# peterhpark/neuroclear

Hardware: AMD Instinct MI355X
Metric: voxels/sec (higher is better)
Workload: dtype f32

## Files before the change

include/nc_hip.h:

```cpp
#ifndef NC_HIP_H
#define NC_HIP_H

#include <stddef.h>
#include <stdint.h>

#ifdef __cplusplus
extern "C" {
#endif

#define NC_OK 0
#define NC_ERR_SHAPE (-1)
#define NC_ERR_WS (-2)
#define NC_ERR_HIP (-3)
#define NC_ERR_ARG (-4)

const char* nc_last_error(void);
int nc_version(void);
int nc_conv_fwd_path(int C, int K, int kd, int kh, int kw, int stride, int pad);
int nc_conv_wgrad_path(int C, int K, int kd, int kh, int kw, int stride, int pad);
void nc_prof_begin(double min_flop);
int nc_prof_end(int max, int* cls, double* flop, float* ms);
int nc_prof_end2(int max, int* cls, double* flop, float* ms, double* abytes);
void nc_set_force_direct(int on);
void nc_sconv_set_cfg(int cfg);
// ... 229 lines not shown
int nc_c8_instnorm_act_bwd(const void* gh, int g_ctot, int g_c0, const void* xh, const float* mean, const float* rstd, float slope,
                           void* dxh, float* dbias , int N, int C, long S, int dtype, void* ws, size_t ws_bytes,
                           void* stream);
int nc_c8_maxpool2_fwd(const void* xh, int x_ctot, int x_c0, void* yh, int N, int C, int D, int H, int W, int dtype, void* stream);
int nc_c8_maxpool2_bwd_add(const void* dph, const void* xh, int x_ctot, int x_c0, const void* skiph, int s_ctot, int s_c0, void* dxh,
                           int N, int C, int D, int H, int W, int dtype, void* stream);
int nc_from_c8(const void* xh, int x_ctot, int x_c0, float* y, int N, int C, long S, int dtype, void* stream);
size_t nc_convT_c8_ws_bytes(int N, int C, int D, int H, int W, int K);
int nc_convT_k2s2_fwd_c8(const void* xh, const float* w, const float* bias, void* yh, int out_ctot, int out_c0, int N, int C, int D,
                         int H, int W, int K, int dtype, void* ws, size_t ws_bytes, void* stream);
int nc_convT_k2s2_dgrad_c8(const void* dyh, int dy_ctot, int dy_c0, const float* w, void* dxh, int N, int C, int D, int H, int W, int K,
                           void* ws, size_t ws_bytes, void* stream);
int nc_convT_k2s2_wgrad_c8(const void* xh, const void* dyh, int dy_ctot, int dy_c0, float* dw, float* dbias , int N,
                           int C, int D, int H, int W, int K, void* ws, size_t ws_bytes, void* stream);

int nc_unet_deconv_lp_supported(int N, int S0, int S1, int S2, int dtype);
size_t nc_unet_deconv_lp_saved_bytes(int N, int S0, int S1, int S2);
size_t nc_unet_deconv_lp_ws_bytes(int N, int S0, int S1, int S2);
int nc_unet_deconv_lp_fwd(const float* params, const float* x, float* y, void* saved, int N, int S0, int S1, int S2, int dtype,
                          void* ws, size_t ws_bytes, void* stream);
int nc_unet_deconv_lp_bwd(const float* params, const float* x, const float* y, const void* saved, const float* dy, float* dx,
                          float* dparams, int N, int S0, int S1, int S2, int dtype, void* ws, size_t ws_bytes, void* stream);
int nc_deep_linear_lp_supported(int N, int S0, int S1, int S2, int dtype);
size_t nc_deep_linear_lp_saved_bytes(int N, int S0, int S1, int S2);
size_t nc_deep_linear_lp_ws_bytes(int N, int S0, int S1, int S2);
int nc_deep_linear_lp_fwd(const float* params, const float* x, float* y, void* saved, int N, int S0, int S1, int S2, int dtype,
                          void* ws, size_t ws_bytes, void* stream, unsigned* kept);
int nc_deep_linear_lp_bwd(const float* params, const float* x, const void* saved, const float* dy, float* dx, float* dparams,
                          int N, int S0, int S1, int S2, int dtype, void* ws, size_t ws_bytes, void* stream, unsigned kept);

void nc_set_conv_split(int on);
int nc_get_conv_split(void);
void nc_set_split_terms(int terms);
int nc_get_split_terms(void);
void nc_set_p2d_terms(int mode);
int nc_get_p2d_terms(void);
void nc_set_h2_guard(int on);
int nc_get_h2_guard(void);
int nc_h2_guard_stats(unsigned long long* out4, int reset);
void nc_set_epi_stats(int on);
int nc_get_epi_stats(void);
void nc_set_s3x_w64(int on);
int nc_get_s3x_w64(void);
int nc_unet_deconv_fwd_terms(int S0, int S1, int S2);
void nc_set_c8x_mode(int mode);
int nc_get_c8x_mode(void);
int nc_conv_lp_uses_c8x(int what , int fp32_out, int N, int C, int D, int H, int W, int K, int ks);
void nc_set_s3_fusion(int on);
int nc_conv_split_supported(int what, int N, int C, int D, int H, int W, int K, int kd, int kh, int kw, int stride, int pad);
size_t nc_conv_split_ws_bytes(int N, int C, int D, int H, int W, int K, int ks);
size_t nc_s3_bytes(int N, int C, long S);
int nc_to_s3(const float* x, void* xs, int N, int C, long S, void* stream);
int nc_conv_fwd_split(const float* x, const void* xs, const float* w, const float* bias, float* y, int N, int C, int D, int H, int W,
                      int K, int ks , void* ws, size_t ws_bytes, void* stream);
int nc_conv_dgrad_split(const float* dy, const void* dys, const float* w, float* dx, int N, int C, int D, int H, int W, int K, int ks,
                        void* ws, size_t ws_bytes, void* stream);
int nc_conv_wgrad_split(const float* x, const void* xs, const float* dy, const void* dys, float* dw, int N, int C, int D, int H, int W,
                        int K, int ks, void* ws, size_t ws_bytes, void* stream);

int nc_conv2d_split_active(int what, int N, int C, int H, int W, int K, int k, int stride, int pad);

int nc_convT_k2s2_split_supported(int N, int C, int D, int H, int W, int K);
int nc_convT_k2s2_split_active(int N, int C, int D, int H, int W, int K);
size_t nc_convT_k2s2_split_ws_bytes(int N, int C, int D, int H, int W, int K);
int nc_convT_k2s2_fwd_split(const float* x, const void* xs, const float* w, const float* bias, float* y, void* ys, int ys_ctot, int ys_c0,
                            int N, int C, int D, int H, int W, int K, void* ws, size_t ws_bytes, void* stream);

size_t nc_h2_bytes(int N, int C, long S);
size_t nc_h2_cells_offset(size_t elems);
int nc_to_h2_debug(const float* x, long xstride, void* xs, int N, int C, long S, int ctot, int c0, unsigned* cell, float bound, unsigned* guard,
                   void* stream);
int nc_act_split2h_debug(const float* x, const float* mean, const float* rstd, float slope, float* y, long ystride, void* ys, int N, int C, long S,
                         int ctot, int c0, float bound, unsigned* cell, unsigned* cell2, void* stream);
int nc_act_split2h_pool_debug(const float* x, const float* mean, const float* rstd, float slope, void* ys, void* pooled, int N, int C, int D, int H,
                              int W, int ctot, int c0, float bound, unsigned* cell, void* stream);
int nc_maxpool2_h2_debug(const void* in, void* out, int N, int C, int ctot, int D, int H, int W, void* stream);
int nc_h2_to_s3_if_debug(const void* xh, void* xs, int N, int C, long S, const unsigned* cells, const unsigned* guard, void* stream);
int nc_instnorm_act_bwd_dbias_h2_debug(const float* dy, const float* w1, const float* x, const float* mean, const float* rstd, float slope, void* dxs,
                                       float* dbias, int N, int C, long S, void* ws, size_t ws_bytes, unsigned* guard, void* stream);
int nc_instnorm_act_bwd_dbias_h2_pool_debug(const float* dy, long dy_stride, const float* gp, const unsigned char* arg, const float* x, const float* mean,
                                            const float* rstd, float slope, void* dxs, float* dbias, int N, int C, int D, int H, int W, void* ws,
                                            size_t ws_bytes, unsigned* guard, void* stream);
int nc_maxpool2_fwd_arg_debug(const float* x, float* y, unsigned char* arg, int NC, int D, int H, int W, void* stream);
size_t nc_convT_k2s2_split_h2_ws_bytes(int N, int C, int D, int H, int W, int K);
int nc_convT_k2s2_fwd_split_h2_debug(const float* x, const float* w, const float* bias, float* y, void* ys, int ys_ctot, int ys_c0, int N, int C,
                                     int D, int H, int W, int K, unsigned* out_cell, void* ws, size_t ws_bytes, void* stream);
int nc_convT_k2s2_fwd_s3_debug(const float* x, const float* w, const float* bias, float* y, void* ys, int ys_ctot, int ys_c0, int N, int C, int D,
                               int H, int W, int K, void* stream);
int nc_instnorm_relu_tail_sigmoid_debug(const float* x, const float* mean, const float* rstd, const float* w1, const float* b1, const float* w2,
                                        const float* b2, float* y, int C, long S, void* stream);

size_t nc_lk_ws_bytes(int N, int D, int H, int W, int k);
int nc_lk_fwd(const float* x, const float* w, float* y, int N, int D, int H, int W, int k, void* ws, size_t ws_bytes, void* stream);
int nc_lk_dgrad(const float* dy, const float* w, float* dx, int N, int D, int H, int W, int k, void* ws, size_t ws_bytes, void* stream);
int nc_lk_wgrad(const float* x, const float* dy, float* dw, int N, int D, int H, int W, int k, void* ws, size_t ws_bytes, void* stream);

size_t nc_kgan_param_floats(int ndf, int nd);
size_t nc_kgan_saved_floats(int B, int D, int H, int W, int ndf, int nd);
size_t nc_kgan_ws_bytes(int B, int D, int H, int W, int ndf, int nd);
int nc_kgan_out_shape(int B, int D, int H, int W, int ndf, int nd, int* oD, int* oH, int* oW);
int nc_kgan_fwd(const float* params, const float* x, float* y, float* saved, int B, int D, int H, int W, int ndf, int nd, void* ws,
                size_t ws_bytes, void* stream);
int nc_kgan_bwd(const float* params, const float* x, const float* saved, const float* dy, float* dx, float* dparams, int B, int D, int H,
                int W, int ndf, int nd, void* ws, size_t ws_bytes, void* stream);

#ifdef __cplusplus
}
#endif
#endif
```

neuroclear_amd/csrc/api.hip:

```cpp
#include <cstring>
#include <vector>

#include <atomic>
#include <mutex>
#include <set>
#include <utility>

#include "common.hpp"

namespace nc {

static thread_local char g_err[512] = "";

void set_error(const char* fmt, ...) {
  va_list ap;
  va_start(ap, fmt);
  vsnprintf(g_err, sizeof(g_err), fmt, ap);
  va_end(ap);
}

int raise_dyn_lds(const void* kernel, int bytes, const char* who) {
  static std::mutex mu;
  static std::set<std::pair<const void*, int>> done;
  int dev = 0;
// ... 403 lines not shown
  if (nc_conv2d_k3_reflect_active(0, N, C, H, W, K)) {
    ProfScope ps(0, 12, d, 0, s);
    return conv_fwd_k3_reflect(x, w, bias, y, d, (char*)ws + pb, ws_bytes - pb, s);
  }
  if (int e = reflect_pad_fwd(x, (float*)ws, (long)N * C, H, W, 1, s)) return e;
  return nc_conv_fwd((const float*)ws, w, bias, y, N, C, 1, H + 2, W + 2, K, 1, 3, 3, 1, 0, (char*)ws + pb, ws_bytes - pb, stream);
}

int nc_conv2d_k3_reflect_dgrad(const float* dy, const float* w, float* dx, int N, int C, int H, int W, int K, void* ws, size_t ws_bytes,
                               void* stream) {
  ConvDims d;
  if (int e = k3r_args("conv2d_k3_reflect_dgrad", d, dy, w, dx, N, C, H, W, K, ws, ws_bytes)) return e;
  hipStream_t s = (hipStream_t)stream;
  const size_t pb = k3r_pad_bytes(N, C, H, W);
  float* dxe = (float*)ws;
  if (nc_conv2d_k3_reflect_active(1, N, C, H, W, K)) {
    ProfScope ps(1, 12, d, 0, s);
    if (int e = conv_dgrad_k3_reflect_ext(dy, w, dxe, d, (char*)ws + pb, ws_bytes - pb, s)) return e;
  } else {
    if (int e = nc_conv_dgrad(dy, w, dxe, N, C, 1, H + 2, W + 2, K, 1, 3, 3, 1, 0, (char*)ws + pb, ws_bytes - pb, stream)) return e;
  }
  return reflect_pad_bwd(dxe, dx, (long)N * C, H, W, 1, s);
}

int nc_conv2d_k3_reflect_wgrad(const float* x, const float* dy, float* dw, float* dbias, int N, int C, int H, int W, int K, void* ws,
                               size_t ws_bytes, void* stream) {
  ConvDims d;
  if (int e = k3r_args("conv2d_k3_reflect_wgrad", d, x, dy, dw, N, C, H, W, K, ws, ws_bytes)) return e;
  const size_t pb = k3r_pad_bytes(N, C, H, W);
  if (int e = reflect_pad_fwd(x, (float*)ws, (long)N * C, H, W, 1, (hipStream_t)stream)) return e;
  return nc_conv_wgrad((const float*)ws, dy, dw, dbias, N, C, 1, H + 2, W + 2, K, 1, 3, 3, 1, 0, (char*)ws + pb, ws_bytes - pb, stream);
}

int nc_conv_bwd(const float* x, const float* dy, const float* w, float* dx, float* dw, float* dbias, int N, int C, int D, int H, int W,
                int K, int kd, int kh, int kw, int stride, int pad, void* ws, size_t ws_bytes, void* stream) {
  ConvDims d;
  if (int e = conv_args("conv_bwd", d, x, dy, dw, N, C, D, H, W, K, kd, kh, kw, stride, pad)) return e;
  if (!w) { set_error("conv_bwd: null pointer"); return NC_ERR_ARG; }
  hipStream_t s = (hipStream_t)stream;
  SwitchScope switches_;
  if (dx && dgrad_path(d) == 9 && wgrad_path(d) == 9 && ws && s3_bwd_ws_bytes(d) && ws_bytes >= s3_bwd_ws_bytes(d)) {
    {
      ProfScope ps(1, 9, d, 0, s);
      if (int e = conv_bwd_s3(x, dy, w, dx, dw, d, ws, ws_bytes, s, 0)) return e;
      if (int e = conv_bwd_s3(x, dy, w, dx, dw, d, ws, ws_bytes, s, 1)) return e;
    }
    {
      ProfScope ps(2, 9, d, 0, s);
      if (int e = conv_bwd_s3(x, dy, w, dx, dw, d, ws, ws_bytes, s, 2)) return e;
    }
    if (dbias) return bias_grad(dy, dbias, d.N, d.K, (long)d.Do * d.Ho * d.Wo, ws, ws_bytes, s);
    return NC_OK;
  }
  if (dx)
    if (int e = nc_conv_dgrad(dy, w, dx, N, C, D, H, W, K, kd, kh, kw, stride, pad, ws, ws_bytes, stream)) return e;
  return nc_conv_wgrad(x, dy, dw, dbias, N, C, D, H, W, K, kd, kh, kw, stride, pad, ws, ws_bytes, stream);
}

}

namespace nc {
int conv_fwd_keep(const float* x, const float* w, const float* bias, float* y, int N, int C, int D, int H, int W, int K, int ks,
                  void* ws, size_t ws_bytes, void* stream, void* xs_keep, bool* kept, const S3xPrepared* prep) {
  ConvDims d;
  *kept = false;
  if (xs_keep && make_dims(d, N, C, D, H, W, K, ks, ks, ks, 1, ks / 2) && fwd_path(d) == 9 && wgrad_path(d) == 9) {
    if (!x || !w || !y) { set_error("conv_fwd: null pointer"); return NC_ERR_ARG; }
    ProfScope ps(0, 9, d, 0, (hipStream_t)stream);
    *kept = true;
    return conv_fwd_s3(x, nullptr, w, bias, y, d, ws, ws_bytes, (hipStream_t)stream, xs_keep, nullptr, prep);
  }
  return nc_conv_fwd(x, w, bias, y, N, C, D, H, W, K, ks, ks, ks, 1, ks / 2, ws, ws_bytes, stream);
}

bool conv_keep_supported(int N, int C, int D, int H, int W, int K, int ks) {
  ConvDims d;
  return make_dims(d, N, C, D, H, W, K, ks, ks, ks, 1, ks / 2) && fwd_path(d) == 9 && wgrad_path(d) == 9;
}
bool conv_fwd_on_split(int N, int C, int D, int H, int W, int K, int ks) {
  ConvDims d;
  return make_dims(d, N, C, D, H, W, K, ks, ks, ks, 1, ks / 2) && fwd_path(d) == 9;
}

int conv_fwd_pre(const void* xs, const float* w, const float* bias, float* y, int N, int C, int D, int H, int W, int K, int ks, void* ws,
                 size_t ws_bytes, void* stream, float* stats_part, const S3xPrepared* prep) {
  ConvDims d;
  if (!xs || !w || !y) { set_error("conv_fwd_pre: null pointer"); return NC_ERR_ARG; }
  if (!make_dims(d, N, C, D, H, W, K, ks, ks, ks, 1, ks / 2) || fwd_path(d) != 9) { set_error("conv_fwd_pre: layer not on the split-operand kernels"); return NC_ERR_SHAPE; }
  ProfScope ps(0, 9, d, 0, (hipStream_t)stream);
  if (stats_part && !(conv_layer_h2(d) && ks == 3)) { set_error("conv_fwd_pre: epilogue statistics exist for the two-term 3^3 layers only"); return NC_ERR_ARG; }
  return conv_fwd_s3(nullptr, xs, w, bias, y, d, ws, ws_bytes, (hipStream_t)stream, nullptr, stats_part, prep);
}

bool conv_bwd_pre_supported(int N, int C, int D, int H, int W, int K, int ks, bool want_dx, size_t ws_bytes) {
  ConvDims d;
  return make_dims(d, N, C, D, H, W, K, ks, ks, ks, 1, ks / 2) && wgrad_path(d) == 9 && s3_bwd_ws_bytes(d) && ws_bytes >= s3_bwd_ws_bytes(d) &&
         (!want_dx || dgrad_path(d) == 9);
}
int conv_bwd_pre(const float* x, const void* xs, const float* w, float* dx, float* dw, int N, int C, int D, int H, int W, int K, int ks,
                 void* ws, size_t ws_bytes, void* stream, bool dy_guarded, const S3xPrepared* prep) {
  ConvDims d;
  hipStream_t s = (hipStream_t)stream;
  if (!conv_bwd_pre_supported(N, C, D, H, W, K, ks, dx != nullptr, ws_bytes) || !make_dims(d, N, C, D, H, W, K, ks, ks, ks, 1, ks / 2)) {
    set_error("conv_bwd_pre: layer not on the split-operand kernels");
    return NC_ERR_SHAPE;
  }
  if ((!x && !xs) || !w || !dw || !ws) { set_error("conv_bwd_pre: null pointer"); return NC_ERR_ARG; }
  if (dx) {
    ProfScope ps(1, 9, d, 0, s);
    if (int e = conv_bwd_s3(x, nullptr, w, dx, dw, d, ws, ws_bytes, s, 1, nullptr, dy_guarded, prep)) return e;
  }
  ProfScope ps(2, 9, d, 0, s);
  return conv_bwd_s3(x, nullptr, w, dx, dw, d, ws, ws_bytes, s, 2, xs, dy_guarded);
}

int conv_bwd_keep(const float* x, const void* xs, const float* dy, const float* w, float* dx, float* dw, int N, int C, int D, int H,
                  int W, int K, int ks, void* ws, size_t ws_bytes, void* stream) {
  ConvDims d;
  hipStream_t s = (hipStream_t)stream;
  if (xs && make_dims(d, N, C, D, H, W, K, ks, ks, ks, 1, ks / 2) && wgrad_path(d) == 9 && ws && s3_bwd_ws_bytes(d) &&
      ws_bytes >= s3_bwd_ws_bytes(d) &&
      (!dx || dgrad_path(d) == 9)) {
    if (!x || !dy || !w || !dw) { set_error("conv_bwd: null pointer"); return NC_ERR_ARG; }
    {
      ProfScope ps(1, 9, d, 0, s);
      if (int e = conv_bwd_s3(x, dy, w, dx, dw, d, ws, ws_bytes, s, 0)) return e;
      if (dx)
        if (int e = conv_bwd_s3(x, dy, w, dx, dw, d, ws, ws_bytes, s, 1)) return e;
    }
    ProfScope ps(2, 9, d, 0, s);
    return conv_bwd_s3(x, dy, w, dx, dw, d, ws, ws_bytes, s, 2, xs);
  }
  return nc_conv_bwd(x, dy, w, dx, dw, nullptr, N, C, D, H, W, K, ks, ks, ks, 1, ks / 2, ws, ws_bytes, stream);
}
}
```

neuroclear_amd/csrc/c8_api.hip:

```cpp
#include "common.hpp"

namespace nc {
size_t c8_stats_ws_bytes(int N, int C, long S);
int c8_instnorm_stats(const void* x, int N, int C, long S, float eps, float* mean, float* rstd, int dt, void* ws, size_t wsb, hipStream_t s);
int c8_instnorm_apply(const void* x, const float* mean, const float* rstd, float slope, void* y, int ctot, int c0, int N, int C, long S, int dt, hipStream_t s);
int c8_instnorm_bwd(const void* g, int gctot, int gc0, const void* x, const float* mean, const float* rstd, float slope, void* dx, float* dbias, int N, int C, long S, int dt, void* ws, size_t wsb, hipStream_t s);
int c8_maxpool_fwd(const void* x, int ctot, int c0, void* y, int N, int C, int D, int H, int W, int dt, hipStream_t s);
int c8_maxpool_bwd_add(const void* dp, const void* x, int ctot, int c0, const void* skip, int sctot, int sc0, void* dx, int N, int C, int D, int H, int W, int dt, hipStream_t s);
int c8_to_f32(const void* x, int ctot, int c0, float* y, int N, int C, long S, int dt, hipStream_t s);
bool convT_h_supported(int C, int K);
size_t convT_h_ws_bytes(int N, int C, int D, int H, int W, int K);
int convT_fwd_h(const void* x, const float* w, const float* bias, void* out, int octot, int oc0, int N, int C, int D, int H, int W, int K, int dt, void* ws, size_t wsb, hipStream_t s);
int convT_dgrad_h(const void* dy, int dctot, int dc0, const float* w, void* dx, int N, int C, int D, int H, int W, int K, void* ws, size_t wsb, hipStream_t s);
int convT_wgrad_h(const void* x, const void* dy, int dctot, int dc0, float* dw, float* dbias, int N, int C, int D, int H, int W, int K, void* ws, size_t wsb, hipStream_t s);
}

using namespace nc;

static bool dt_ok(int dt) { return dt == NC_DT_F16 || dt == NC_DT_BF16; }

extern "C" {

int nc_conv_fwd_c8(const void* xh, const float* w, const float* bias, void* yh, int out_ctot, int out_c0, int N, int C, int D, int H,
                   int W, int K, int kd, int kh, int kw, int stride, int pad, int dtype, void* ws, size_t ws_bytes, void* stream) {
// ... 109 lines not shown
int nc_conv_split_supported(int what, int N, int C, int D, int H, int W, int K, int kd, int kh, int kw, int stride, int pad) {
  ConvDims d;
  if (!make_dims(d, N, C, D, H, W, K, kd, kh, kw, stride, pad)) return 0;
  return what == 0 ? s3_fwd_supported(d) : what == 1 ? s3_dgrad_supported(d) : what == 2 ? s3_wgrad_supported(d) : 0;
}

size_t nc_conv_split_ws_bytes(int N, int C, int D, int H, int W, int K, int ks) {
  ConvDims d;
  if (!make_dims(d, N, C, D, H, W, K, ks, ks, ks, 1, ks / 2)) return 0;
  const size_t a = s3_ws_bytes(d), b = s3_wgrad_ws_bytes(d);
  return a > b ? a : b;
}

size_t nc_s3_bytes(int N, int C, long S) { return (C % 8 || N < 1 || S < 1) ? 0 : s3_tensor_bytes(N, C, S); }

int nc_to_s3(const float* x, void* xs, int N, int C, long S, void* stream) {
  if (!x || !xs) { set_error("to_s3: null pointer"); return NC_ERR_ARG; }
  if (N < 1 || C < 8 || C % 8 || S < 1) { set_error("to_s3: channels must be a multiple of 8"); return NC_ERR_SHAPE; }
  return split3_to(x, xs, N, C, S, (hipStream_t)stream);
}

int nc_conv_fwd_split(const float* x, const void* xs, const float* w, const float* bias, float* y, int N, int C, int D, int H, int W,
                      int K, int ks, void* ws, size_t ws_bytes, void* stream) {
  ConvDims d;
  if ((!x && !xs) || !w || !y) { set_error("conv_fwd_split: null pointer"); return NC_ERR_ARG; }
  if (!make_dims(d, N, C, D, H, W, K, ks, ks, ks, 1, ks / 2) || !s3_fwd_supported(d)) { set_error("conv_fwd_split: shape not covered"); return NC_ERR_SHAPE; }
  ProfScope ps(0, 1, d, 1, (hipStream_t)stream);
  ForceThreeTerm f3;
  return conv_fwd_s3(x, xs, w, bias, y, d, ws, ws_bytes, (hipStream_t)stream);
}

int nc_conv_dgrad_split(const float* dy, const void* dys, const float* w, float* dx, int N, int C, int D, int H, int W, int K, int ks,
                        void* ws, size_t ws_bytes, void* stream) {
  ConvDims d;
  if ((!dy && !dys) || !w || !dx) { set_error("conv_dgrad_split: null pointer"); return NC_ERR_ARG; }
  if (!make_dims(d, N, C, D, H, W, K, ks, ks, ks, 1, ks / 2) || !s3_dgrad_supported(d)) { set_error("conv_dgrad_split: shape not covered"); return NC_ERR_SHAPE; }
  ProfScope ps(1, 1, d, 1, (hipStream_t)stream);
  ForceThreeTerm f3;
  return conv_dgrad_s3(dy, dys, w, dx, d, ws, ws_bytes, (hipStream_t)stream);
}

int nc_conv_wgrad_split(const float* x, const void* xs, const float* dy, const void* dys, float* dw, int N, int C, int D, int H, int W,
                        int K, int ks, void* ws, size_t ws_bytes, void* stream) {
  ConvDims d;
  if ((!x && !xs) || (!dy && !dys) || !dw) { set_error("conv_wgrad_split: null pointer"); return NC_ERR_ARG; }
  if (!make_dims(d, N, C, D, H, W, K, ks, ks, ks, 1, ks / 2) || !s3_wgrad_supported(d)) { set_error("conv_wgrad_split: shape not covered"); return NC_ERR_SHAPE; }
  ProfScope ps(2, 9, d, 0, (hipStream_t)stream);
  ForceThreeTerm f3;
  return conv_wgrad_s3(x, xs, dy, dys, dw, d, ws, ws_bytes, (hipStream_t)stream);
}

static size_t al256(size_t b) { return (b + 255) & ~(size_t)255; }
int nc_convT_k2s2_split_supported(int N, int C, int D, int H, int W, int K) { return convT_s3x_supported(N, C, D, H, W, K) ? 1 : 0; }
int nc_conv_lp_uses_c8x(int what, int fp32_out, int N, int C, int D, int H, int W, int K, int ks) {
  if (what == 0) return c8x_supported(N, C, D, H, W, K, ks, fp32_out != 0) ? 1 : 0;
  if (what == 1) return c8x_supported(N, K, D, H, W, C, ks, fp32_out != 0) ? 1 : 0;
  return 0;
}
int nc_convT_k2s2_split_active(int N, int C, int D, int H, int W, int K) { return nc_get_conv_split() && convT_s3x_supported(N, C, D, H, W, K) ? 1 : 0; }
size_t nc_convT_k2s2_split_ws_bytes(int N, int C, int D, int H, int W, int K) {
  if (!convT_s3x_supported(N, C, D, H, W, K)) return 0;
  return al256(convT_s3x_ws_bytes(C, K)) + al256(s3_tensor_bytes(N, C, (long)D * H * W)) + 256;
}
int nc_convT_k2s2_fwd_split(const float* x, const void* xs, const float* w, const float* bias, float* y, void* ys, int ys_ctot, int ys_c0,
                            int N, int C, int D, int H, int W, int K, void* ws, size_t ws_bytes, void* stream) {
  if ((!x && !xs) || !w || (!y && !ys) || !ws) { set_error("convT_k2s2_fwd_split: null pointer"); return NC_ERR_ARG; }
  if (!convT_s3x_supported(N, C, D, H, W, K)) { set_error("convT_k2s2_fwd_split: shape not covered"); return NC_ERR_SHAPE; }
  const size_t wb = al256(convT_s3x_ws_bytes(C, K));
  const long S = (long)D * H * W;
  if (ws_bytes < wb + (xs ? 0 : al256(s3_tensor_bytes(N, C, S)))) { set_error("convT_k2s2_fwd_split: workspace too small"); return NC_ERR_WS; }
  if (!xs) {
    void* t = (char*)ws + wb;
    if (int e = split3_to(x, t, N, C, S, (hipStream_t)stream)) return e;
    xs = t;
  }
  return convT_fwd_s3x(xs, w, bias, y, ys, ys ? ys_ctot : 8, ys ? ys_c0 : 0, N, C, D, H, W, K, ws, wb, (hipStream_t)stream);
}

}

namespace nc {
int convT_fwd_split_h2(const float* x, const float* w, const float* bias, float* y, void* ys, int ys_ctot, int ys_c0, int N, int C, int D, int H,
                       int W, int K, const unsigned* out_cell, void* ws, size_t ws_bytes, hipStream_t s) {
  if (!x || !w || !ys || !out_cell || !ws) { set_error("convT_fwd_split_h2: null pointer"); return NC_ERR_ARG; }
  if (!convT_s3x_supported(N, C, D, H, W, K)) { set_error("convT_fwd_split_h2: shape not covered"); return NC_ERR_SHAPE; }
  const size_t wb = al256(convT_s3x_ws_bytes(C, K));
  const long S = (long)D * H * W;
  const size_t ex = (size_t)N * C * S;
  if (ws_bytes < wb + h2_cells_offset(ex) + 256) { set_error("convT_fwd_split_h2: workspace too small"); return NC_ERR_WS; }
  void* t = (char*)ws + wb;
  unsigned* xc = h2_cells_of(t, ex);
  if (int e = h2_set_cell(xc, sqrtf((float)S), s)) return e;
  if (int e = split2h_into(x, (long)C * S, t, N, C, S, C, 0, xc, s)) return e;
  return convT_fwd_s3x(t, w, bias, y, ys, ys_ctot, ys_c0, N, C, D, H, W, K, ws, wb, s, out_cell, xc);
}
}
```

neuroclear_amd/csrc/common.hpp:

```cpp
#pragma once
#include <hip/hip_runtime.h>

#include <cstdarg>
#include <cstdio>

#include "../../include/nc_hip.h"
#include "switches.hpp"

namespace nc {

void set_error(const char* fmt, ...);

inline int check_launch(const char* what) {
  hipError_t e = hipGetLastError();
  if (e != hipSuccess) {
    set_error("%s: %s", what, hipGetErrorString(e));
    return NC_ERR_HIP;
  }
  return NC_OK;
}

inline long cdiv(long a, long b) { return (a + b - 1) / b; }
inline size_t align256(size_t b) { return (b + 255) & ~(size_t)255; }
inline size_t up64(size_t n) { return (n + 63) & ~(size_t)63; }
// ... 46 lines not shown
    return false;
  d.Do = (D + 2 * d.pd - kd) / d.sd + 1;
  d.Ho = (H + 2 * d.ph - kh) / d.sh + 1;
  d.Wo = (W + 2 * d.pw - kw) / d.sw + 1;
  return d.Do >= 1 && d.Ho >= 1 && d.Wo >= 1 && (D + 2 * d.pd >= kd) && (H + 2 * d.ph >= kh) && (W + 2 * d.pw >= kw);
}

int conv_fwd_direct(const float* x, const float* w, const float* b, float* y, const ConvDims& d, hipStream_t s);
int conv_dgrad_direct(const float* dy, const float* w, float* dx, const ConvDims& d, hipStream_t s);
int conv_wgrad_direct(const float* x, const float* dy, float* dw, const ConvDims& d, hipStream_t s);
int bias_grad(const float* dy, float* db, int N, int K, long S, void* ws, size_t wsb, hipStream_t s);
static constexpr size_t kBiasGradWsBytes = 64 * 1024 * sizeof(double);

bool mfma_fwd_supported(const ConvDims& d);
bool c1k3_fwd_supported(const ConvDims& d);
int conv_fwd_c1k3(const float* x, const float* w, const float* bias, float* y, const ConvDims& d, hipStream_t s, float* stats_part = nullptr);
size_t c1k3_stats_bytes(const ConvDims& d);
int c1k3_stats_finalize(const float* stats_part, const float* bias, const ConvDims& d, float eps, float* mean, float* rstd, hipStream_t s);
bool mfma_dgrad_supported(const ConvDims& d);
bool mfma_wgrad_supported(const ConvDims& d);
size_t mfma_ws_bytes(const ConvDims& d);
size_t mfma_fwd_ws_bytes(const ConvDims& d);
int conv_fwd_mfma(const float* x, const float* w, const float* b, float* y, const ConvDims& d, void* ws, size_t wsb,
                  hipStream_t s);
int conv_dgrad_mfma(const float* dy, const float* w, float* dx, const ConvDims& d, void* ws, size_t wsb,
                    hipStream_t s);
int conv_wgrad_mfma(const float* x, const float* dy, float* dw, const ConvDims& d, void* ws, size_t wsb,
                    hipStream_t s);

bool gemm_fwd_supported(const ConvDims& d);
bool gemm_dgrad_supported(const ConvDims& d);
bool gemm_wgrad_supported(const ConvDims& d);
size_t gemm_ws_bytes(const ConvDims& d);
int conv_fwd_gemm(const float* x, const float* w, const float* b, float* y, const ConvDims& d, void* ws, size_t wsb,
                  hipStream_t s);
int conv_dgrad_gemm(const float* dy, const float* w, float* dx, const ConvDims& d, void* ws, size_t wsb,
                    hipStream_t s);
int conv_wgrad_gemm(const float* x, const float* dy, float* dw, const ConvDims& d, void* ws, size_t wsb,
                    hipStream_t s);

bool sconv_fwd_supported(const ConvDims& d);
bool sconv_dgrad_supported(const ConvDims& d);
size_t sconv_ws_bytes(const ConvDims& d);
bool p2d_fwd_supported(const ConvDims& d);
bool p2d_dgrad_supported(const ConvDims& d);
size_t p2d_ws_bytes(const ConvDims& d);
int conv_fwd_p2d(const float* x, const float* w, const float* bias, float* y, const ConvDims& d, void* ws, size_t wsb, hipStream_t s);
int conv_dgrad_p2d(const float* dy, const float* w, float* dx, const ConvDims& d, void* ws, size_t wsb, hipStream_t s);
bool p2d_wgrad_supported(const ConvDims& d);
size_t p2d_wgrad_ws_bytes(const ConvDims& d);
int conv_wgrad_p2d(const float* x, const float* dy, float* dw, const ConvDims& d, void* ws, size_t wsb, hipStream_t s);
int conv_fwd_sconv(const float* x, const float* w, const float* bias, float* y, const ConvDims& d, void* ws, size_t wsb, hipStream_t s);
int conv_dgrad_sconv(const float* dy, const float* w, float* dx, const ConvDims& d, void* ws, size_t wsb, hipStream_t s);
int conv2d_k3_num_cfgs();
bool conv2d_k3_fwd_supported(const ConvDims& d);
bool conv2d_k3_dgrad_supported(const ConvDims& d);
size_t conv2d_k3_ws_bytes(const ConvDims& d);
int conv_fwd_k3(const float* x, const float* w, const float* bias, float* y, const ConvDims& d, void* ws, size_t wsb, hipStream_t s);
int conv_dgrad_k3(const float* dy, const float* w, float* dx, const ConvDims& d, void* ws, size_t wsb, hipStream_t s);
bool conv2d_k3_reflect_ok(const ConvDims& d);
int conv_fwd_k3_reflect(const float* x, const float* w, const float* bias, float* y, const ConvDims& d, void* ws, size_t wsb, hipStream_t s);
int conv_dgrad_k3_reflect_ext(const float* dy, const float* w, float* dxe, const ConvDims& d, void* ws, size_t wsb, hipStream_t s);
int reflect_pad_fwd(const float* x, float* y, long NC, int H, int W, int p, hipStream_t s);
int reflect_pad_bwd(const float* g, float* dx, long NC, int H, int W, int p, hipStream_t s);
bool sconv_wgrad_supported(const ConvDims& d);
size_t sconv_wgrad_ws_bytes(const ConvDims& d);
int conv_wgrad_sconv(const float* x, const float* dy, float* dw, const ConvDims& d, void* ws, size_t wsb, hipStream_t s);

bool pg1_supported(const ConvDims& d);
size_t pg1_ws_bytes(const ConvDims& d);
int conv_fwd_pg1(const float* x, const float* w, const float* bias, float* y, const ConvDims& d, float slope, hipStream_t s);
int conv_wgrad_pg1(const float* x, const float* g, const float* act, float slope, float* dw, float* db, const ConvDims& d,
                   void* ws, size_t wsb, hipStream_t s);
int conv_dgrad_pg1(const float* g, const float* act, float slope, const float* w, float* dx, const ConvDims& d, hipStream_t s);

bool wgrad_1x1_supported(const ConvDims& d);
size_t wgrad_1x1_ws_bytes(const ConvDims& d);
int conv_wgrad_1x1(const float* x, const float* dy, float* dw, const ConvDims& d, void* ws, size_t wsb, hipStream_t s);
bool flat_1x1_supported(const ConvDims& d);
int conv_fwd_1x1(const float* x, const float* w, const float* b, float* y, const ConvDims& d, void* ws, size_t wsb,
                 hipStream_t s);
int conv_dgrad_1x1(const float* dy, const float* w, float* dx, const ConvDims& d, void* ws, size_t wsb,
                   hipStream_t s);

size_t conv_fwd_to1_k3_ws_bytes(int N, int D, int H, int W);
int conv_fwd_to1_k3(const float* x, const float* w, float* y, int N, int C, int D, int H, int W, void* ws, size_t wsb, hipStream_t s);
bool to1_dgrad_supported(const ConvDims& d);
int conv_dgrad_to1(const float* dy, const float* w, float* dx, const ConvDims& d, hipStream_t s);
bool to1_mfma_supported(const ConvDims& d);
size_t to1_mfma_ws_bytes(const ConvDims& d);
int conv_dgrad_to1_mfma(const float* dy, const float* w, float* dx, const ConvDims& d, void* ws, size_t wsb,
                        hipStream_t s);
bool k1_fwd_supported(const ConvDims& d);
bool k1_wgrad_supported(const ConvDims& d);
int conv_fwd_k1(const float* x, const float* w, const float* b, float* y, const ConvDims& d, hipStream_t s);
int conv_wgrad_k1(const float* x, const float* dy, float* dw, const ConvDims& d, hipStream_t s);
bool c1_wgrad_supported(const ConvDims& d);
size_t c1_wgrad_ws_bytes(const ConvDims& d);
int conv_wgrad_c1(const float* x, const float* dy, float* dw, const ConvDims& d, void* ws, size_t wsb, hipStream_t s);

bool s3_fwd_supported(const ConvDims& d);
bool s3_dgrad_supported(const ConvDims& d);
size_t s3_ws_bytes(const ConvDims& d);
size_t s3_tensor_bytes(int N, int C, long S);
int split3_to(const float* x, void* xs, int N, int C, long S, hipStream_t s);
int split3_into(const float* x, long xstride, void* xs, int N, int C, long S, int ctot, int c0, hipStream_t s, const unsigned* guard = nullptr);
bool conv_layer_h2(const ConvDims& d);
void count_in_bwd_launches(int n, int which = 0);
int operand_into(const ConvDims& d, const float* x, long xstride, void* xs, int N, int C, long S, int ctot, int c0, hipStream_t s);
int act_operand(const ConvDims& d, const float* x, const float* mean, const float* rstd, float slope, float* y, long ystride, void* ys, int N, int C,
                long S, int ctot, int c0, hipStream_t s);
int act_split3(const float* x, const float* mean, const float* rstd, float slope, float* y, long ystride, void* ys, int N, int C, long S,
               int ctot, int c0, hipStream_t s);
struct S3xPrepared { const void* wp; const unsigned* wcell; };
int conv_fwd_s3(const float* x, const void* xs, const float* w, const float* b, float* y, const ConvDims& d, void* ws, size_t wsb,
                hipStream_t s, void* xs_keep = nullptr, float* stats_part = nullptr, const S3xPrepared* prep = nullptr);
int conv_dgrad_s3(const float* dy, const void* dys, const float* w, float* dx, const ConvDims& d, void* ws, size_t wsb, hipStream_t s);
size_t s3_bwd_ws_bytes(const ConvDims& d);
int conv_bwd_s3(const float* x, const float* dy, const float* w, float* dx, float* dw, const ConvDims& d, void* ws, size_t wsb,
                hipStream_t s, int phase, const void* xs = nullptr, bool dy_guarded = false, const S3xPrepared* prep = nullptr);
int conv_fwd_keep(const float* x, const float* w, const float* bias, float* y, int N, int C, int D, int H, int W, int K, int ks,
                  void* ws, size_t ws_bytes, void* stream, void* xs_keep, bool* kept, const S3xPrepared* prep = nullptr);
int conv_bwd_keep(const float* x, const void* xs, const float* dy, const float* w, float* dx, float* dw, int N, int C, int D, int H,
                  int W, int K, int ks, void* ws, size_t ws_bytes, void* stream);
bool s3x_supported(int N, int Cin, int D, int H, int W, int Kout, int KS);
size_t s3x_packed_bytes(int Cin, int Kout, int KS, int NT = 3);
int s3x_ksteps(int Cin, int KS);
constexpr int kWPrepMaxSegs = 18, kWPrepMaxBounds = 2, kWPrepBoundCell0 = kWPrepMaxSegs, kWPrepCellBytes = 256;
struct WPrepSeg { const float* w; int Cin, Kout, flip; unsigned a_bits; int b_cell; unsigned* ext_cell; };
struct WPrepBound { const float* w; const float* bias; int C, K; float in_bound; int cell; };
size_t wprep_bytes(const WPrepSeg* segs, int n);
int wprep_run(const WPrepSeg* segs, int n, const WPrepBound* bounds, int nb, void* region, S3xPrepared* out, hipStream_t s);
int s3x_pack_h2(const float* w, int Cin, int Kout, int KS, long so, long si, int flip, int split_c, const unsigned* cell_a, const unsigned* cell_b,
                unsigned* wcell, void* wp_ws, hipStream_t s);
int conv_s3x_h2(const void* xs, const unsigned* cell_a, const unsigned* cell_b, int split_c, const float* w, const float* bias, float* y, int N,
                int Cin, int D, int H, int W, int Kout, int KS, long so, long si, int flip, unsigned* wcell, void* wp_ws, hipStream_t s,
                const unsigned* guard = nullptr, float* stats_part = nullptr, const S3xPrepared* prep = nullptr);
size_t s3x_stats_bytes(int N, int D, int H, int W, int Kout, int KS);
int s3x_stats_finalize(const float* stats_part, const float* bias, int N, int D, int H, int W, int Kout, int KS, float eps, float* mean, float* rstd,
                       hipStream_t s);
bool c1k7_h2_supported(const ConvDims& d);
size_t c1k7_h2_ws_bytes(const ConvDims& d);
int conv_c1k7_h2(const float* x, const float* w, const float* bias, float* y, const ConvDims& d, void* ws, size_t wsb, hipStream_t s);
size_t c1k7_h2_dgrad_ws_bytes(const ConvDims& d);
bool dl_typed_supported(int N, int D, int H, int W);
size_t dl_typed_bytes(int N, int D, int H, int W);
const float* dl_typed_wp(const char* scratch, int N, int D, int H, int W);
float* dl_typed_dwsw(char* scratch, int N, int D, int H, int W);
int dl_typed_compose(const float* F, char* scratch, int N, int D, int H, int W, hipStream_t s);
int dl_typed_fwd_boundary(const float* act0, float* y, char* scratch, int N, int D, int H, int W, hipStream_t s);
int dl_typed_dgrad_boundary(const float* act0, const float* dy, float* g, char* scratch, int N, int D, int H, int W, hipStream_t s);
int dl_typed_p(const float* act0, const float* dy, float* Pq, char* scratch, int N, int D, int H, int W, hipStream_t s);
int conv_c1k7_h2_dgrad(const float* dy, const float* w, float* dx, const ConvDims& d, void* ws, size_t wsb, hipStream_t s);
inline size_t h2_cells_offset(size_t elems) { return (elems * 4 + 255) & ~(size_t)255; }
inline unsigned* h2_cells_of(const void* t, size_t elems) { return (unsigned*)((char*)const_cast<void*>(t) + h2_cells_offset(elems)); }
int instnorm_relu_tail_sigmoid(const float* x, const float* mean, const float* rstd, const float* w1, const float* b1, const float* w2,
                               const float* b2, float* y, int C, long S, hipStream_t s);
int instnorm_act_bwd_dbias_h2(const float* dy, const float* x, const float* mean, const float* rstd, float slope, void* dxs,
                              float* dbias, int N, int C, long S, void* ws, size_t ws_bytes, void* stream, unsigned* guard = nullptr);
int instnorm_act_bwd_dbias_h2_rank1(const float* dy1, const float* w1, const float* x, const float* mean, const float* rstd, float slope, void* dxs,
                                    float* dbias, int C, long S, void* ws, size_t ws_bytes, void* stream, unsigned* guard);
unsigned* conv_bwd_guard_words(void* ws, int N, int K, long S);
int maxpool2_h2(const void* in, void* out, int N, int C, int ctot, int D, int H, int W, hipStream_t s);
int h2_zero_cells(unsigned* cells, int n, hipStream_t s);
int h2_set_cell(unsigned* cell, float bound, hipStream_t s);
int h2_absmax(const float* x, long n, unsigned* cell, hipStream_t s, unsigned* cell2 = nullptr);
int split2h_into(const float* x, long xstride, void* xs, int N, int C, long S, int ctot, int c0, const unsigned* cell, hipStream_t s,
                 unsigned* guard = nullptr);
constexpr int kGuardLow = 0, kGuardAll = 1, kGuardFlag = 2;
constexpr unsigned kGuardDrop = 17u << 23;
constexpr unsigned long long kGuardShare = 64;
#if defined(__HIP_DEVICE_COMPILE__)
__device__ __forceinline__ bool guard_skip(const unsigned* guard, int want) {
  return guard && (int)(__builtin_nontemporal_load(guard + kGuardFlag) != 0) != want;
}
#else
__device__ bool guard_skip(const unsigned* guard, int want);
#endif
#if defined(__HIPCC__)
__device__ __forceinline__ void h2_guard_decide_one(unsigned* ga, unsigned* gb, unsigned* prior, unsigned* flag, int can_flip,
                                                    unsigned long long* stats, unsigned long long total_a) {
  unsigned f = 0;
  unsigned long long worst = 0;
  int n = 0;
  for (unsigned* g : {ga, gb}) {
    if (!g) continue;
    ++n;
    const unsigned long long lo = g[kGuardLow], all = (g == ga && total_a) ? total_a - g[kGuardAll] : g[kGuardAll];
    if (all && lo * kGuardShare > all) f = 1;
    const unsigned long long ppm = all ? lo * 1000000ull / all : 0;
    worst = ppm > worst ? ppm : worst;
  }
  unsigned F = f && can_flip ? 1u : 0u;
  if (prior && prior[kGuardFlag]) F = 1u;
  *flag = F;
  if (prior) prior[kGuardFlag] = F;
  if (stats && n) {
    __hip_atomic_fetch_add(stats + 0, (unsigned long long)n, __ATOMIC_RELAXED, __HIP_MEMORY_SCOPE_SYSTEM);
    if (f) __hip_atomic_fetch_add(stats + (can_flip ? 1 : 2), 1ull, __ATOMIC_RELAXED, __HIP_MEMORY_SCOPE_SYSTEM);
    __hip_atomic_fetch_max(stats + 3, worst, __ATOMIC_RELAXED, __HIP_MEMORY_SCOPE_SYSTEM);
  }
}
#endif
unsigned long long* h2_guard_stats_dev();
int h2_guard_read(unsigned long long* out4, int reset);
int h2_guard_zero(unsigned* g, hipStream_t s, int nwords = 8);
int h2_guard_decide(unsigned* ga, unsigned* gb, unsigned* prior, unsigned* flag, bool can_flip, hipStream_t s, unsigned long long total_a = 0);
int h2_to_s3_if(const void* xh, void* xs, int N, int C, long S, const unsigned* cells, const unsigned* guard, hipStream_t s);
int act_split2h(const float* x, const float* mean, const float* rstd, float slope, float* y, long ystride, void* ys, int N, int C, long S, int ctot,
                int c0, float bound, unsigned* cell, unsigned* cell2, hipStream_t s);
int act_split2h_pool(const float* x, const float* mean, const float* rstd, float slope, void* ys, void* pooled, int N, int C, int D, int H, int W,
                     int ctot, int c0, float bound, unsigned* cell, hipStream_t s);
int conv_s3x(const void* xs, const float* w, const float* bias, float* y, int N, int Cin, int D, int H, int W, int Kout, int KS, long so,
             long si, int flip, void* wp_ws, hipStream_t s, const unsigned* guard = nullptr);
bool conv_keep_supported(int N, int C, int D, int H, int W, int K, int ks);
bool conv_fwd_on_split(int N, int C, int D, int H, int W, int K, int ks);
int conv_fwd_pre(const void* xs, const float* w, const float* bias, float* y, int N, int C, int D, int H, int W, int K, int ks, void* ws,
                 size_t ws_bytes, void* stream, float* stats_part = nullptr, const S3xPrepared* prep = nullptr);
bool conv_bwd_pre_supported(int N, int C, int D, int H, int W, int K, int ks, bool want_dx, size_t ws_bytes);
int conv_bwd_pre(const float* x, const void* xs, const float* w, float* dx, float* dw, int N, int C, int D, int H, int W, int K, int ks,
                 void* ws, size_t ws_bytes, void* stream, bool dy_guarded = false, const S3xPrepared* prep = nullptr);
bool instnorm_bwd_h2_pool_supported(int N, int C, int D, int H, int W, unsigned* guard);
int instnorm_act_bwd_dbias_h2_pool(const float* skip, long skip_stride, const float* gp, const unsigned char* arg, const float* x, const float* mean,
                                   const float* rstd, float slope, void* dxs, float* dbias, int N, int C, int D, int H, int W, void* ws,
                                   size_t ws_bytes, void* stream, unsigned* guard);
int maxpool2_fwd_arg(const float* x, float* y, unsigned char* arg, int NC, int D, int H, int W, hipStream_t s);
bool instnorm_bwd_s3_supported(int N, int C, long S);
int instnorm_act_bwd_dbias_s3(const float* dy, const float* x, const float* mean, const float* rstd, float slope, void* dxs,
                              float* dbias, int N, int C, long S, void* ws, size_t ws_bytes, void* stream);
bool convT_fwd_s3_supported(int N, int C, int D, int H, int W, int K);
size_t c8x_packed_bytes(int Cin, int Kout, int KS);
bool c8x_supported(int N, int Cin, int D, int H, int W, int Kout, int KS, bool fp32_out);
int conv_c8x(const void* xh, const float* w, const float* bias, float* y, void* yh, int ctot, int c0, int N, int Cin, int D, int H, int W,
             int Kout, int KS, long so, long si, int flip, int diffuse, int dt, void* wp_ws, hipStream_t s);
bool convT_s3x_supported(int N, int C, int D, int H, int W, int K);
size_t convT_s3x_ws_bytes(int C, int K);
int convT_fwd_s3x(const void* xs, const float* w, const float* bias, float* y, void* ys, int ctot, int c0, int N, int C, int D, int H, int W,
                  int K, void* ws, size_t wsb, hipStream_t s, const unsigned* h2cell = nullptr, const unsigned* xcell = nullptr);
int convT_h2_bound(const float* w, const float* bias, int C, int K, float in_bound, unsigned* cell, hipStream_t s);
int convT_fwd_split_h2(const float* x, const float* w, const float* bias, float* y, void* ys, int ys_ctot, int ys_c0, int N, int C, int D, int H,
                       int W, int K, const unsigned* out_cell, void* ws, size_t ws_bytes, hipStream_t s);
int convT_fwd_s3(const float* x, const float* w, const float* bias, float* y, void* ys, int ctot, int c0, int N, int C, int D, int H,
                 int W, int K, void* stream);
bool s3_wgrad_supported(const ConvDims& d);
bool c8x_wgrad_supported(const ConvDims& d);
size_t c8x_wgrad_part_bytes(const ConvDims& d);
int conv_wgrad_c8x(const void* xh, const void* dyh, float* dw, const ConvDims& d, int dtype, void* ws, size_t wsb, hipStream_t s);
size_t s3_wgrad_ws_bytes(const ConvDims& d);
int conv_wgrad_s3(const float* x, const void* xs, const float* dy, const void* dys, float* dw, const ConvDims& d, void* ws, size_t wsb,
                  hipStream_t s);
bool s3x_k32_supported(int N, int D, int H, int W);
bool conv_fwd_h2_k32_supported(const ConvDims& d);
int conv_fwd_h2_k32_keep(const float* x, const float* w, float* y, const ConvDims& d, void* ws, size_t wsb, hipStream_t s, void* xs_keep);
bool conv_fwd_h2_c32_supported(const ConvDims& d);
size_t conv_fwd_h2_c32_ws_bytes(const ConvDims& d);
int conv_fwd_h2_c32(const float* x, const float* w, float* y, const ConvDims& d, void* ws, size_t wsb, hipStream_t s);
bool wgrad_h2_supported(const ConvDims& d);
int conv_wgrad_h2(const float* x, const void* xs, const float* dy, const void* dys, float* dw, const ConvDims& d, void* ws, size_t wsb, hipStream_t s);
bool h_fwd_supported(const ConvDims& d);
bool h_dgrad_supported(const ConvDims& d);
bool h_wgrad_supported(const ConvDims& d);
size_t h_ws_bytes(const ConvDims& d);
int to_c8(const float* x, void* xh, int N, int C, long S, int dt, hipStream_t s);
int conv_fwd_h(const float* x, const void* xh, const float* w, const float* b, float* y, const ConvDims& d, int dt,
               void* ws, size_t wsb, hipStream_t s);
int conv_dgrad_h(const float* dy, const void* dyh, const float* w, float* dx, const ConvDims& d, int dt, void* ws,
                 size_t wsb, hipStream_t s);
int conv_wgrad_h(const float* x, const void* xh, const float* dy, const void* dyh, float* dw, const ConvDims& d, int dt,
                 void* ws, size_t wsb, hipStream_t s);
int conv_fwd_h_c8(const void* xh, const float* w, const float* b, void* yh, int ctot, int c0, const ConvDims& d, int dt,
                  void* ws, size_t wsb, hipStream_t s);
int conv_fwd_h_na1(const void* xh, const float* w, float* y, const ConvDims& d, int dt, void* ws, size_t wsb, hipStream_t s);
int conv_dgrad_h_c8(const void* dyh, const float* w, void* dxh, int ctot, int c0, const ConvDims& d, int dt, void* ws,
                    size_t wsb, hipStream_t s);
size_t dl_tail_bytes();
const float* dl_tail_E(const char* tail);
const float* dl_tail_Ef(const char* tail);
float* dl_tail_q(char* tail);
int dl_tail_compose(const float* w2, const float* w3, const float* w4, const float* w5, char* tail, hipStream_t s);
int dl_tail_grads(const float* w2, const float* w3, const float* w4, const float* w5, char* tail, float* dw2, float* dw3, float* dw4, float* dw5,
                  hipStream_t s);
float* dl_tail_P(char* tail);
const float* dl_w1_fold(char* tail, const float* w1, hipStream_t s);
int dl_w1_contract(const char* tail, float* dw1, hipStream_t s);
int dl_q_from_p(char* tail, const float* w1, hipStream_t s);
const float* dl_fold_fwd64(char* tail, const float* w1, hipStream_t s);
int dl_combine27(const float* Z, float* y, int N, int D, int H, int W, int zch, hipStream_t s);
bool c1_h_supported(int D, int H, int W, int KS);
size_t c1_h_ws_bytes(int N, int D, int H, int W, int KS);
int conv_c1_fwd_h(const float* x, const float* w, const float* bias, void* yh, int ctot, int c0, int N, int D, int H, int W, int KS,
                  int dt, void* ws, size_t wsb, hipStream_t s);
int conv_c1_dgrad_h(const void* dyh, const float* w, float* dx, int N, int D, int H, int W, int KS, void* ws, size_t wsb,
                    hipStream_t s);

void h_set_weight_diffusion(int on);

bool c1_wgrad_h_supported(int N, int D, int H, int W, int KS);
size_t c1_wgrad_h_ws_bytes(int N, int D, int H, int W, int KS);
int conv_c1_wgrad_h(const float* x, const void* dyh, float* dw, int N, int D, int H, int W, int KS, void* ws, size_t wsb,
                    hipStream_t s);

static constexpr size_t kPackSlackBytes = 128 * 1024;

struct ProfScope {
  int idx;
  hipStream_t s;
  ProfScope(int op, int path, const ConvDims& d, int lp, hipStream_t stream);
  ~ProfScope();
};

}
```

neuroclear_amd/csrc/conv_1x1.hip:

```cpp
#include "common.hpp"

namespace nc {
NC_ZERO_PAGE()


typedef float f32x4 __attribute__((ext_vector_type(4)));

static constexpr int kVC = 128;
static constexpr int kPitch = 136;
static constexpr int kMaxP1 = 9;

struct W1Params {
  const float* x;
  const float* dy;
  float* slab;
  const float* zeros;
  int C, K, N;
  long S;
  int Kp, Cp;
  int npd, npx;
  long nchunks;
  long cps;
};

__global__ __launch_bounds__(512) void k_wgrad_1x1(W1Params p) {
  extern __shared__ __attribute__((aligned(16))) float lds[];
  typedef const __attribute__((address_space(1))) void* gptr_t;
  typedef __attribute__((address_space(3))) void* lptr_t;
  const int tid = threadIdx.x, lane = tid & 63;
  const int wave = __builtin_amdgcn_readfirstlane(tid >> 6);
  const int l15 = lane & 15, kq = lane >> 4;
  const int MB = p.Kp / 16, NB = p.Cp / 16, nblk = MB * NB;
  const int bufsz = (p.npd + p.npx) * 256;
  const long c0 = p.nchunks * blockIdx.x / gridDim.x, c1 = p.nchunks * (blockIdx.x + 1) / gridDim.x;

  int goff[kMaxP1], gcol[kMaxP1];
#pragma unroll
  for (int i = 0; i < kMaxP1; ++i) {
    const int j = wave + 8 * i;
    const bool isx = j >= p.npd;
    const int f = ((isx ? j - p.npd : j) * 64 + lane) * 4;
    const int row = f / kPitch, col = f - row * kPitch;
    const bool ok = col < kVC && row < (isx ? p.C : p.K);
    goff[i] = ok ? (int)(row * p.S + col) : -1;
    gcol[i] = col;
  }
  auto issue = [&](long chunk, float* buf) {
    const long n = chunk / p.cps;
    const long v0 = (chunk - n * p.cps) * kVC;
    const float* db = p.dy + n * p.K * p.S + v0;
    const float* xb = p.x + n * p.C * p.S + v0;
    const int vleft = (int)min((long)kVC, p.S - v0);
#pragma unroll
    for (int i = 0; i < kMaxP1; ++i) {
      const int j = wave + 8 * i;
      if (j < p.npd + p.npx) {
        const float* base = j >= p.npd ? xb : db;
        const float* src = (goff[i] >= 0 && gcol[i] < vleft) ? base + goff[i] : p.zeros;
        nc_dma_lds16(src, nc_lds_addr((buf + j * 256)));
      }
    }
  };

  f32x4 acc[2] = {f32x4{0.f, 0.f, 0.f, 0.f}, f32x4{0.f, 0.f, 0.f, 0.f}};
  int aoff[2], boff[2];
#pragma unroll
  for (int t = 0; t < 2; ++t) {
    const int b = wave + 8 * t;
    const int mb = b < nblk ? b / NB : 0, nb = b < nblk ? b % NB : 0;
    aoff[t] = (mb * 16 + l15) * kPitch + 4 * kq;
    boff[t] = p.npd * 256 + (nb * 16 + l15) * kPitch + 4 * kq;
  }

  if (c0 < c1) issue(c0, lds);
  for (long c = c0; c < c1; ++c) {
    const int par = (int)((c - c0) & 1);
    asm volatile("s_waitcnt vmcnt(0)" ::: "memory");
    __syncthreads();
    if (c + 1 < c1) issue(c + 1, lds + (par ^ 1) * bufsz);
    const float* buf = lds + par * bufsz;
#pragma unroll
    for (int t = 0; t < 2; ++t) {
      if (wave + 8 * t < nblk) {
#pragma unroll
        for (int q = 0; q < kVC; q += 16) {
          const f32x4 a = *reinterpret_cast<const f32x4*>(__builtin_assume_aligned(buf + aoff[t] + q, 16));
          const f32x4 b = *reinterpret_cast<const f32x4*>(__builtin_assume_aligned(buf + boff[t] + q, 16));
#pragma unroll
          for (int m = 0; m < 4; ++m) acc[t] = __builtin_amdgcn_mfma_f32_16x16x4f32(a[m], b[m], acc[t], 0, 0, 0);
        }
      }
    }
  }
  float* sl = p.slab + (long)blockIdx.x * p.Kp * p.Cp;
#pragma unroll
  for (int t = 0; t < 2; ++t) {
    const int b = wave + 8 * t;
    if (b < nblk) {
      const int mb = b / NB, nb = b % NB;
#pragma unroll
      for (int r = 0; r < 4; ++r) sl[(mb * 16 + 4 * kq + r) * p.Cp + nb * 16 + l15] = acc[t][r];
    }
  }
}

__global__ void k_wgrad_1x1_reduce(const float* __restrict__ slab, float* __restrict__ dw, int nwg, int K, int C,
                                   int Kp, int Cp) {
  const int i = blockIdx.x * (blockDim.x >> 6) + (threadIdx.x >> 6);
  if (i >= K * C) return;
  const int lane = threadIdx.x & 63;
  const int k = i / C, c = i - k * C;
  float s = 0.f;
  for (int w = lane; w < nwg; w += 64) s += slab[((long)w * Kp + k) * Cp + c];
#pragma unroll
  for (int o = 32; o > 0; o >>= 1) s += __shfl_xor(s, o, 64);
  if (lane == 0) dw[i] = s;
}

bool wgrad_1x1_supported(const ConvDims& d) {
  if (d.kd != 1 || d.kh != 1 || d.kw != 1 || d.sh != 1 || d.sw != 1 || d.ph != 0 || d.pw != 0) return false;
  if (d.K > 64 || d.C > 64) return false;
  const long S = (long)d.D * d.H * d.W;
  if (S % 4 || S < 16384 || S * 64 >= (1L << 31)) return false;
  return true;
}

static int wg1_nwg(const ConvDims& d) {
  const long S = (long)d.D * d.H * d.W;
  const long chunks = (long)d.N * ((S + kVC - 1) / kVC);
  return (int)(chunks < 256 ? chunks : 256);
}

size_t wgrad_1x1_ws_bytes(const ConvDims& d) {
  if (!wgrad_1x1_supported(d)) return 0;
  const int Kp = (d.K + 15) & ~15, Cp = (d.C + 15) & ~15;
  return (size_t)wg1_nwg(d) * Kp * Cp * sizeof(float) + 256;
}

int conv_wgrad_1x1(const float* x, const float* dy, float* dw, const ConvDims& d, void* ws, size_t wsb, hipStream_t s) {
  const size_t need = wgrad_1x1_ws_bytes(d);
  if (!need) {
    set_error("wgrad_1x1: unsupported shape");
    return NC_ERR_SHAPE;
  }
  if (!ws || wsb < need) {
    set_error("wgrad_1x1: workspace too small (%zu < %zu)", wsb, need);
    return NC_ERR_WS;
  }
  W1Params p{};
  p.x = x; p.dy = dy; p.slab = (float*)ws;
  p.zeros = nc_zero_page();
  if (!p.zeros) { set_error("wgrad_1x1: no zero page"); return NC_ERR_HIP; }
  p.C = d.C; p.K = d.K; p.N = d.N;
  p.S = (long)d.D * d.H * d.W;
  p.Kp = (d.K + 15) & ~15; p.Cp = (d.C + 15) & ~15;
  p.npd = (p.Kp * kPitch + 255) / 256; p.npx = (p.Cp * kPitch + 255) / 256;
  p.cps = (p.S + kVC - 1) / kVC;
  p.nchunks = (long)d.N * p.cps;
  const int nwg = wg1_nwg(d);
  const int lds_bytes = 2 * (p.npd + p.npx) * 256 * (int)sizeof(float);
  if (int e = raise_dyn_lds(k_wgrad_1x1, 160 * 1024, "wgrad_1x1")) return e;
  hipLaunchKernelGGL(k_wgrad_1x1, dim3(nwg), dim3(512), lds_bytes, s, p);
  if (int e = check_launch("wgrad_1x1")) return e;
  hipLaunchKernelGGL(k_wgrad_1x1_reduce, dim3((d.K * d.C + 3) / 4), dim3(256), 0, s, (const float*)ws, dw, nwg, d.K,
                     d.C, p.Kp, p.Cp);
  return check_launch("wgrad_1x1_reduce");
}

static constexpr int kPitchF = 144;
static constexpr int kPitchO = 132;
struct F1Params {
  const float* in;
  const float* w;
  const float* bias;
  float* out;
  const float* zeros;
  int M, R, N;
  int sm, sr;
  long S;
  int Rp;
  int npi;
  long nchunks, cps;
};

__global__ __launch_bounds__(512) void k_flat_1x1(F1Params p) {
  extern __shared__ __attribute__((aligned(16))) float lds[];
  typedef const __attribute__((address_space(1))) void* gptr_t;
  typedef __attribute__((address_space(3))) void* lptr_t;
  const int tid = threadIdx.x, lane = tid & 63;
  const int wave = __builtin_amdgcn_readfirstlane(tid >> 6);
  const int l15 = lane & 15, kq = lane >> 4;
  const int MB = (p.M + 15) / 16;
  const int bufsz = p.npi * 256;
  float* ost = lds + 2 * bufsz;
  const long c0 = p.nchunks * blockIdx.x / gridDim.x, c1 = p.nchunks * (blockIdx.x + 1) / gridDim.x;

  int goff[5], gcol[5];
#pragma unroll
  for (int i = 0; i < 5; ++i) {
    const int f = ((wave + 8 * i) * 64 + lane) * 4;
    const int row = f / kPitchF, col = f - row * kPitchF;
    goff[i] = (col < kVC && row < p.R) ? (int)(row * p.S + col) : -1;
    gcol[i] = col;
  }
  auto issue = [&](long chunk, float* buf) {
    const long n = chunk / p.cps;
    const long v0 = (chunk - n * p.cps) * kVC;
    const float* xb = p.in + n * p.R * p.S + v0;
    const int vleft = (int)min((long)kVC, p.S - v0);
#pragma unroll
    for (int i = 0; i < 5; ++i) {
      const int j = wave + 8 * i;
      if (j < p.npi) {
        const float* src = (goff[i] >= 0 && gcol[i] < vleft) ? xb + goff[i] : p.zeros;
        nc_dma_lds16(src, nc_lds_addr((buf + j * 256)));
      }
    }
  };
  const int wpm = MB >= 4 ? 2 : MB == 2 ? 4 : 8;
  const int mb = wave / wpm;
  const bool mb_on = mb < MB;
  float aw[16];
#pragma unroll
  for (int ks = 0; ks < 16; ++ks) {
    const int m = mb * 16 + l15, r = 4 * ks + kq;
    aw[ks] = (mb_on && m < p.M && r < p.R) ? p.w[(long)m * p.sm + (long)r * p.sr] : 0.f;
  }
  const int nks = p.Rp / 4;
  const int b_off = kq * kPitchF + l15;

  if (c0 < c1) issue(c0, lds);
  for (long c = c0; c < c1; ++c) {
    const int par = (int)((c - c0) & 1);
    asm volatile("s_waitcnt vmcnt(0)" ::: "memory");
    __syncthreads();
    if (c + 1 < c1) issue(c + 1, lds + (par ^ 1) * bufsz);
    const float* buf = lds + par * bufsz + b_off;
    if (mb_on) {
      for (int nb = wave % wpm; nb < 8; nb += wpm) {
        f32x4 acc = f32x4{0.f, 0.f, 0.f, 0.f};
#pragma unroll
        for (int ks = 0; ks < 16; ++ks)
          if (ks < nks) acc = __builtin_amdgcn_mfma_f32_16x16x4f32(aw[ks], buf[4 * ks * kPitchF + nb * 16], acc, 0, 0, 0);
#pragma unroll
        for (int rr = 0; rr < 4; ++rr) ost[(mb * 16 + 4 * kq + rr) * kPitchO + nb * 16 + l15] = acc[rr];
      }
    }
    __syncthreads();
    const long n = c / p.cps;
    const long v0 = (c - n * p.cps) * kVC;
    const int vleft = (int)min((long)kVC, p.S - v0);
    for (int m = 2 * wave + (lane >> 5); m < p.M; m += 16) {
      const int col = (lane & 31) * 4;
      if (col < vleft) {
        f32x4 v = *reinterpret_cast<const f32x4*>(__builtin_assume_aligned(ost + m * kPitchO + col, 16));
        if (p.bias) {
          const float b = p.bias[m];
          v += f32x4{b, b, b, b};
        }
        *reinterpret_cast<f32x4*>(p.out + (n * p.M + m) * p.S + v0 + col) = v;
      }
    }
  }
}

static bool flat_1x1_shape(const ConvDims& d) {
  if (d.kd != 1 || d.kh != 1 || d.kw != 1 || d.sh != 1 || d.sw != 1 || d.ph != 0 || d.pw != 0) return false;
  if (d.K > 64 || d.C > 64) return false;
  const long S = (long)d.D * d.H * d.W;
  return S % 4 == 0 && S >= 16384 && S * 64 < (1L << 31);
}
bool flat_1x1_supported(const ConvDims& d) { return flat_1x1_shape(d); }

static int launch_flat(const float* in, const float* w, const float* bias, float* out, int M, int R, int sm, int sr,
                       const ConvDims& d, void* ws, size_t wsb, hipStream_t s) {
  if (!ws || wsb < 256) {
    set_error("flat_1x1: workspace too small");
    return NC_ERR_WS;
  }
  F1Params p{};
  p.in = in; p.w = w; p.bias = bias; p.out = out; p.zeros = nc_zero_page();
  if (!p.zeros) { set_error("flat_1x1: no zero page"); return NC_ERR_HIP; }
  p.M = M; p.R = R; p.N = d.N; p.sm = sm; p.sr = sr;
  p.S = (long)d.D * d.H * d.W;
  p.Rp = (R + 3) & ~3;
  p.npi = (p.Rp * kPitchF + 255) / 256;
  p.cps = (p.S + kVC - 1) / kVC;
  p.nchunks = (long)d.N * p.cps;
  const int nwg = (int)(p.nchunks < 512 ? p.nchunks : 512);
  const int MB = (M + 15) / 16;
  const int lds_bytes = (2 * p.npi * 256 + MB * 16 * kPitchO) * (int)sizeof(float);
  if (int e = raise_dyn_lds(k_flat_1x1, 160 * 1024, "flat_1x1")) return e;
  hipLaunchKernelGGL(k_flat_1x1, dim3(nwg), dim3(512), lds_bytes, s, p);
  return check_launch("flat_1x1");
}

int conv_fwd_1x1(const float* x, const float* w, const float* b, float* y, const ConvDims& d, void* ws, size_t wsb,
                 hipStream_t s) {
  return launch_flat(x, w, b, y, d.K, d.C, d.C, 1, d, ws, wsb, s);
}
int conv_dgrad_1x1(const float* dy, const float* w, float* dx, const ConvDims& d, void* ws, size_t wsb,
                   hipStream_t s) {
  return launch_flat(dy, w, nullptr, dx, d.C, d.K, 1, d.C, d, ws, wsb, s);
}

}
```

neuroclear_amd/csrc/convt_s3.hip:

```cpp

#include "common.hpp"
#include "s3_common.hpp"
#include "w_prep.hpp"

namespace nc {
namespace {

typedef float f32x4 __attribute__((ext_vector_type(4)));
typedef __bf16 bf16x8 __attribute__((ext_vector_type(8)));
typedef _Float16 f16x8 __attribute__((ext_vector_type(8)));
typedef int i32x4 __attribute__((ext_vector_type(4)));

constexpr int kTWaves = 8;
constexpr int kTThreads = kTWaves * 64;
constexpr int kTCB = 4;

template <int NT>
__global__ void __launch_bounds__(256) k_pack_wT_s3(const float* __restrict__ w, unsigned short* __restrict__ wp, int C, int K, int QN, long total,
                                                    const unsigned* __restrict__ wcell) {
  const long i = (long)blockIdx.x * 256 + threadIdx.x;
  if (i >= total) return;
  const int j = (int)(i & 7);
  long r = i >> 3;
  const int lane = (int)(r & 63); r >>= 6;
// ... 84 lines not shown
    };
    load_b(0);
#pragma unroll 1
    for (int s = 0; s < NS; ++s) {
      i32x4 Bc[kTCB][NT];
#pragma unroll
      for (int cb = 0; cb < kTCB; ++cb)
#pragma unroll
        for (int t = 0; t < NT; ++t) Bc[cb][t] = B[cb][t];
      if (s + 1 < NS) load_b(s + 1);
      const i32x4* ws = wl + (long)s * QN * NT * 64;
#pragma unroll
      for (int q = 0; q < QN; ++q) {
        i32x4 A[NT];
#pragma unroll
        for (int t = 0; t < NT; ++t) A[t] = ws[(q * NT + t) * 64];
        constexpr int NP = NT == 3 ? 6 : 3;
        constexpr int TA[6] = {NT - 1, NT == 3 ? 1 : 0, 0, 1, 0, 0};
        constexpr int TB[6] = {0, 1, NT == 3 ? 2 : 0, 0, 1, 0};
#pragma unroll
        for (int m = 0; m < NP; ++m)
#pragma unroll
          for (int cb = 0; cb < kTCB; ++cb) {
            if constexpr (NT == 3)
              acc[q][cb] = __builtin_amdgcn_mfma_f32_16x16x32_bf16(__builtin_bit_cast(bf16x8, A[TA[m]]), __builtin_bit_cast(bf16x8, Bc[cb][TB[m]]),
                                                                   acc[q][cb], 0, 0, 0);
            else
              acc[q][cb] = __builtin_amdgcn_mfma_f32_16x16x32_f16(__builtin_bit_cast(f16x8, A[TA[m]]), __builtin_bit_cast(f16x8, Bc[cb][TB[m]]),
                                                                  acc[q][cb], 0, 0, 0);
          }
      }
    }
#pragma unroll
    for (int cb = 0; cb < kTCB; ++cb) {
      const long v = v0 + cb * 16 + m16;
      if (v >= S) continue;
      const int ix = (int)(v % p.W), iy = (int)((v / p.W) % p.H), iz = (int)(v / ((long)p.W * p.H));
#pragma unroll
      for (int q = 0; q < QN; ++q) {
        const int qq = qg * QN + q;
        const long o = ((long)(2 * iz + (qq >> 2)) * H2 + (2 * iy + ((qq >> 1) & 1))) * W2 + 2 * ix + (qq & 1);
        float val[4];
#pragma unroll
        for (int e = 0; e < 4; ++e) val[e] = NT == 2 ? acc[q][cb][e] * oscx * oscw + bb[e] : acc[q][cb][e] + bb[e];
        if (p.y) {
          float* yk = p.y + ((long)n * p.K + kg * 16 + 4 * g) * S2 + o;
#pragma unroll
          for (int e = 0; e < 4; ++e) yk[(long)e * S2] = val[e];
        }
        if (p.ys && p.h2cell) {
          unsigned short t3[4][3];
          const float sc = h2_scale(*p.h2cell);
#pragma unroll
          for (int e = 0; e < 4; ++e) h2_split(val[e] * sc, t3[e]);
          const long blk = ((long)n * p.oblocks + p.ob0 + kg * 2 + (g >> 1)) * 2;
#pragma unroll
          for (int t = 0; t < 2; ++t)
            p.ys[((blk + t) * S2 + o) * 2 + (g & 1)] = make_uint2(t3[0][t] | ((unsigned)t3[1][t] << 16), t3[2][t] | ((unsigned)t3[3][t] << 16));
        } else if (p.ys) {
          unsigned short t3[4][3];
#pragma unroll
          for (int e = 0; e < 4; ++e) s3_split(val[e], t3[e]);
          const long blk = ((long)n * p.oblocks + p.ob0 + kg * 2 + (g >> 1)) * 3;
#pragma unroll
          for (int t = 0; t < 3; ++t)
            p.ys[((blk + t) * S2 + o) * 2 + (g & 1)] = make_uint2(t3[0][t] | ((unsigned)t3[1][t] << 16), t3[2][t] | ((unsigned)t3[3][t] << 16));
        }
      }
    }
  }
}

__global__ void __launch_bounds__(256) k_convT_bound(const float* __restrict__ w, const float* __restrict__ bias, int C, int K, float in_bound,
                                                     unsigned* __restrict__ cell) {
  __shared__ float part[4][64];
  __shared__ float red[64];
  convT_bound_block(w, bias, C, K, in_bound, cell, (int)blockIdx.x, part, red);
}

int qn_for(int C) { return (C / 32) * 8 * 3 * 1024 <= 128 * 1024 ? 8 : 4; }

}

bool convT_s3x_supported(int N, int C, int D, int H, int W, int K) {
  const bool on = sw::raw(sw::CONVT_S3X) != 0;
  const long S = (long)D * H * W;
  if (!on || C % 32 || K % 16 || C > 256 || N < 1) return false;
  if ((C / 32) * qn_for(C) * 3 * 1024 > 128 * 1024) return false;
  return (long)N * K * 8 * S < (1L << 40) && S * 16 * 3 * (C / 8) < (1L << 40);
}
size_t convT_s3x_ws_bytes(int C, int K) { return (size_t)C * K * 8 * 3 * 2 + 256; }

int convT_h2_bound(const float* w, const float* bias, int C, int K, float in_bound, unsigned* cell, hipStream_t s) {
  hipLaunchKernelGGL(k_convT_bound, dim3((unsigned)cdiv((long)K * 8, 64)), dim3(256), 0, s, w, bias, C, K, in_bound, cell);
  return check_launch("convT_h2_bound");
}

int convT_fwd_s3x(const void* xs, const float* w, const float* bias, float* y, void* ys, int ctot, int c0, int N, int C, int D, int H, int W,
                  int K, void* ws, size_t wsb, hipStream_t s, const unsigned* h2cell, const unsigned* xcell) {
  if (!xs || !w || (!y && !ys) || !ws) { set_error("convT_fwd_s3x: null pointer"); return NC_ERR_ARG; }
  if (!convT_s3x_supported(N, C, D, H, W, K) || ctot % 8 || c0 % 8) { set_error("convT_fwd_s3x: shape not covered"); return NC_ERR_SHAPE; }
  if (wsb < convT_s3x_ws_bytes(C, K)) { set_error("convT_fwd_s3x: workspace too small"); return NC_ERR_WS; }
  const int QN = qn_for(C);
  const int NT = xcell ? 2 : 3;
  const long total = (long)C * K * 8 * NT;
  unsigned* wcell = (unsigned*)((char*)ws + (size_t)C * K * 8 * 3 * 2);
  if (NT == 2) {
    if (int e = h2_zero_cells(wcell, 1, s)) return e;
    if (int e = h2_absmax(w, (long)C * K * 8, wcell, s)) return e;
    hipLaunchKernelGGL(k_pack_wT_s3<2>, dim3((unsigned)cdiv(total, 256)), dim3(256), 0, s, w, (unsigned short*)ws, C, K, QN, total, (const unsigned*)wcell);
  } else {
    hipLaunchKernelGGL(k_pack_wT_s3<3>, dim3((unsigned)cdiv(total, 256)), dim3(256), 0, s, w, (unsigned short*)ws, C, K, QN, total, (const unsigned*)nullptr);
  }
  if (int e = check_launch("pack_wT_s3")) return e;
  const long S = (long)D * H * W;
  TParams3 p{};
  p.xs = (const uint4*)xs; p.wp = (const uint4*)ws; p.bias = bias; p.y = y; p.ys = (uint2*)ys;
  p.N = N; p.C = C; p.K = K; p.D = D; p.H = H; p.W = W;
  p.oblocks = ctot / 8; p.ob0 = c0 / 8; p.h2cell = ys ? h2cell : nullptr; p.xcell = xcell; p.wcell = wcell;
  p.ngroups = (K / 16) * (8 / QN);
  p.ntiles = (long)N * cdiv(S, 512);
  int per_xcd = 32 / p.ngroups;
  if (per_xcd < 1) per_xcd = 1;
  const unsigned grid = (unsigned)(8 * p.ngroups * per_xcd);
  const size_t lds = (size_t)(C / 32) * QN * NT * 1024;
  auto launch = [&](auto kern) -> int {
    if (int e = raise_dyn_lds(kern, 160 * 1024, "convT_fwd_s3x")) return e;
    hipLaunchKernelGGL(kern, dim3(grid), dim3(kTThreads), lds, s, p);
    return check_launch("convT_s3");
  };
  if (NT == 2) return QN == 8 ? launch(k_convT_s3<8, 2>) : launch(k_convT_s3<4, 2>);
  return QN == 8 ? launch(k_convT_s3<8, 3>) : launch(k_convT_s3<4, 3>);
}

}
```

neuroclear_amd/csrc/gen_nets.hip:

```cpp


#include "common.hpp"
#include "unet_desc.hpp"

using namespace nc;

namespace {

size_t s3_floats(size_t elems) { return up64((elems * 6 + 3) / 4); }

constexpr int kLeanBit0 = 10;
constexpr int kLeanBlocks[5] = {1, 3, 5, 6, 8};
int lean_index(int consumer) {
  for (int j = 0; j < 5; ++j) if (kLeanBlocks[j] == consumer) return j;
  return -1;
}

constexpr unsigned kKeptWPrep = 1u << 15;
constexpr unsigned kKeptPoolArg = 1u << 26;
void wprep_segs(WPrepSeg (&sg)[18]) {
  for (int i = 1; i < 10; ++i) {
    sg[2 * (i - 1)] = WPrepSeg{nullptr, kUB[i].C, kUB[i].K, 0, 0u, -1, nullptr};
    sg[2 * (i - 1) + 1] = WPrepSeg{nullptr, kUB[i].K, kUB[i].C, 1, 0u, -1, nullptr};
  }
}
unsigned f32_bits(float f) { unsigned b; __builtin_memcpy(&b, &f, 4); return b; }


struct UPlan {
  int N, d[3][3];
  long S[3];
  size_t a1, cat1, p1, a2, cat2, p2, b1, b2, b3, e2a, e2b, e1, t1, raw[10], mean[10], rstd[10], saved;
  size_t xs3[10];
  size_t wprep;
  size_t parg[2];
  size_t G1, G2, G3, H1, H2, H3, Q1, Q2, s1, s2, T, grads;
  size_t conv_ws, in_ws, convT_ws;
};

bool u_plan(UPlan& p, int N, int S0, int S1, int S2) {
  if (N < 1 || !u_edges_ok(S0, S1, S2)) return false;
  p = UPlan{};
  p.N = N;
  u_level_dims(S0, S1, S2, p.d, p.S);
  const size_t n = (size_t)N, S = (size_t)p.S[0], Sh = (size_t)p.S[1], Sq = (size_t)p.S[2];
  size_t off = 0;
  auto take = [&](size_t k) { size_t r = off; off += up64(k); return r; };
  p.a1 = take(n * 64 * S); p.cat1 = take(n * 128 * S); p.p1 = take(n * 64 * Sh); p.a2 = take(n * 128 * Sh);
  p.cat2 = take(n * 256 * Sh); p.p2 = take(n * 128 * Sq); p.b1 = take(n * 256 * Sq); p.b2 = take(n * 256 * Sq);
  p.b3 = take(n * 256 * Sq); p.e2a = take(n * 128 * Sh); p.e2b = take(n * 128 * Sh); p.e1 = take(n * 64 * S);
  p.t1 = take(n * S);
  for (int i = 0; i < 10; ++i) {
    p.raw[i] = take(n * kUB[i].K * (size_t)p.S[kUB[i].lvl]);
    p.mean[i] = take(n * kUB[i].K);
    p.rstd[i] = take(n * kUB[i].K);
  }
  for (int i = 1; i < 10; ++i) { p.xs3[i] = off; off += s3_floats(n * kUB[i].C * (size_t)p.S[kUB[i].lvl]); }
  {
    WPrepSeg sg[18];
    wprep_segs(sg);
    p.wprep = off;
    off += up64((wprep_bytes(sg, 18) + 3) / 4);
  }
  p.parg[0] = off; off += up64((n * 64 * Sh + 3) / 4);
  p.parg[1] = off; off += up64((n * 128 * Sq + 3) / 4);
  p.saved = off;
  off = 0;
  p.G1 = take(n * 64 * S); p.G2 = take(n * 64 * S); p.G3 = take(n * 128 * S);
  p.H1 = take(n * 128 * Sh); p.H2 = take(n * 128 * Sh); p.H3 = take(n * 256 * Sh);
  p.Q1 = take(n * 256 * Sq); p.Q2 = take(n * 256 * Sq); p.s1 = take(n * S); p.s2 = take(n * S);
  p.T = take(n * 64 * S);
  p.grads = off;
  auto upd = [&](int C, int K, int l, int k) {
    const size_t b = nc_conv_ws_bytes(N, C, p.d[l][0], p.d[l][1], p.d[l][2], K, k, k, k, 1, k / 2);
    if (b > p.conv_ws) p.conv_ws = b;
  };
  for (int i = 0; i < 10; ++i) upd(kUB[i].C, kUB[i].K, kUB[i].lvl, 3);
  upd(64, 1, 0, 1); upd(1, 1, 0, 1);
  p.in_ws = nc_instnorm_bwd_dbias_ws_bytes(N * 256, (long)S);
  for (int i = 1; i < 10; ++i) {
    const size_t b = s3x_stats_bytes(N, p.d[kUB[i].lvl][0], p.d[kUB[i].lvl][1], p.d[kUB[i].lvl][2], kUB[i].K, 3);
    if (b > p.in_ws) p.in_ws = b;
  }
  p.convT_ws = nc_convT_ws_bytes(N, 256, p.d[2][0], p.d[2][1], p.d[2][2], 128);
  const size_t c2 = nc_convT_ws_bytes(N, 128, p.d[1][0], p.d[1][1], p.d[1][2], 64);
  if (c2 > p.convT_ws) p.convT_ws = c2;
  return true;
}

int gather_half(const float* src, float* dst, int N, int Ctot, int c0, int C, long S, hipStream_t s) {
  if (hipMemcpy2DAsync(dst, (size_t)C * S * 4, src + (size_t)c0 * S, (size_t)Ctot * S * 4, (size_t)C * S * 4, N,
                       hipMemcpyDeviceToDevice, s) != hipSuccess) {
    set_error("gather_half: hipMemcpy2DAsync failed");
// ... 9 lines not shown
}

extern "C" {

size_t nc_unet_deconv_param_floats(void) { return u_offsets().total; }

int nc_unet_wprep_layout(int N, int S0, int S1, int S2, int block, int form, size_t* pack_off, size_t* pack_bytes, size_t* cell_off,
                         size_t* bound_off) {
  UPlan p;
  if (!u_plan(p, N, S0, S1, S2) || block < 1 || block > 9 || form < 0 || form > 1) { set_error("unet_wprep_layout: bad argument"); return NC_ERR_ARG; }
  WPrepSeg sg[18];
  wprep_segs(sg);
  const int k = 2 * (block - 1) + form;
  size_t off = kWPrepCellBytes;
  for (int j = 0; j < k; ++j) off += s3x_packed_bytes(sg[j].Cin, sg[j].Kout, 3, 2);
  if (pack_off) *pack_off = p.wprep * 4 + off;
  if (pack_bytes) *pack_bytes = s3x_packed_bytes(sg[k].Cin, sg[k].Kout, 3, 2);
  if (cell_off) *cell_off = p.wprep * 4 + (size_t)k * 4;
  if (bound_off) *bound_off = block == 7 ? p.wprep * 4 + (size_t)kWPrepBoundCell0 * 4 : block == 9 ? p.wprep * 4 + (size_t)(kWPrepBoundCell0 + 1) * 4 : 0;
  return NC_OK;
}
int nc_s3x_pack_h2_debug(const float* w, int C, int K, int form, const unsigned* cell_a, const unsigned* cell_b, void* wp, unsigned* wcell,
                         void* stream) {
  if (!w || !cell_a || !cell_b || !wp || !wcell || C % 64 || K % 64) { set_error("s3x_pack_h2_debug: bad argument"); return NC_ERR_ARG; }
  if (form) return s3x_pack_h2(w, K, C, 3, 27, (long)C * 27, 1, K, cell_a, cell_a, wcell, wp, (hipStream_t)stream);
  return s3x_pack_h2(w, C, K, 3, (long)C * 27, 27, 0, C / 2, cell_a, cell_b, wcell, wp, (hipStream_t)stream);
}
int nc_convT_h2_bound_debug(const float* w, const float* bias, int C, int K, float in_bound, unsigned* cell, void* stream) {
  if (!w || !cell) { set_error("convT_h2_bound_debug: null pointer"); return NC_ERR_ARG; }
  NC_TRY(h2_zero_cells(cell, 1, (hipStream_t)stream));
  return convT_h2_bound(w, bias, C, K, in_bound, cell, (hipStream_t)stream);
}

size_t nc_unet_deconv_saved_floats(int N, int S0, int S1, int S2) {
  UPlan p;
  return u_plan(p, N, S0, S1, S2) ? p.saved : 0;
}

size_t nc_unet_deconv_train_ws_bytes(int N, int S0, int S1, int S2) {
  UPlan p;
  return u_plan(p, N, S0, S1, S2) ? u_ws_bytes(p, true) : 0;
}

int nc_unet_deconv_train_fwd(const float* params, const float* x, float* y, float* saved, int N, int S0, int S1, int S2,
                             void* ws, size_t ws_bytes, void* stream, unsigned* kept) {
  NetworkScope net_scope;
  if (!params || !x || !y || !saved) { set_error("unet_deconv_train_fwd: null pointer"); return NC_ERR_ARG; }
  UPlan p;
  if (!u_plan(p, N, S0, S1, S2)) {
    set_error("unet_deconv_train_fwd: every edge must be a positive multiple of 4 (got %d,%d,%d)", S0, S1, S2);
    return NC_ERR_SHAPE;
  }
  if (!ws || ws_bytes < u_ws_bytes(p, false)) { set_error("unet_deconv_train_fwd: workspace too small"); return NC_ERR_WS; }
  const UOff o = u_offsets();
  void* cws = ws;
  void* iws = (char*)ws + align256(p.conv_ws);
  float* V = saved;
  const float* P = params;
  if (kept) *kept = 0;
  hipStream_t hs = (hipStream_t)stream;
  const bool fuse_on = sw::raw(sw::S3_TRAIN_FUSE) != 0;
  const bool lean = sw::raw(sw::UNET_LEAN) != 0;
  bool use[10], pre[10], h2l[10];
  ConvDims cd[10];
  for (int i = 0; i < 10; ++i) {
    const UBlock& b = kUB[i];
    const int* d = p.d[b.lvl];
    use[i] = fuse_on && i >= 1 && conv_keep_supported(N, b.C, d[0], d[1], d[2], b.K, 3);
    pre[i] = false;
    h2l[i] = make_dims(cd[i], N, b.C, d[0], d[1], d[2], b.K, 3, 3, 3, 1, 1) && use[i] && conv_layer_h2(cd[i]);
  }
  const long S = p.S[0], Sh = p.S[1], Sq = p.S[2];
  const int *d0 = p.d[0], *d1 = p.d[1], *d2 = p.d[2];
  const bool ct2 = nc_convT_k2s2_split_active(1, 256, d2[0], d2[1], d2[2], 128) &&
                   p.conv_ws >= nc_convT_k2s2_split_ws_bytes(1, 256, d2[0], d2[1], d2[2], 128);
  const bool ct_h2 = sw::raw(sw::CONVT_H2) != 0;
  const bool ct2h = ct2 && h2l[7] && ct_h2;
  const bool ct1 = nc_convT_k2s2_split_active(1, 128, d1[0], d1[1], d1[2], 64) &&
                   p.conv_ws >= nc_convT_k2s2_split_ws_bytes(1, 128, d1[0], d1[1], d1[2], 64);
  const bool ct1h = ct1 && h2l[9] && ct_h2;
  unsigned* cell7 = h2_cells_of(V + p.xs3[7], (size_t)N * 256 * Sh) + 1;
  unsigned* cell9 = h2_cells_of(V + p.xs3[9], (size_t)N * 128 * S) + 1;
  unsigned kept_mask = 0;
  S3xPrepared prep[18] = {};
  bool bound7 = false, bound9 = false;
  if (sw::raw(sw::UNET_WPREP)) {
    WPrepSeg sg[18];
    wprep_segs(sg);
    WPrepBound wb[2];
    int nb = 0, any = 0;
    for (int i = 1; i < 10; ++i) {
      if (!h2l[i]) continue;
      WPrepSeg& f = sg[2 * (i - 1)];
      f.a_bits = f32_bits(sqrtf((float)p.S[kUB[i].lvl]));
      f.w = P + o.w[i];
      if (i == 7 || i == 9) {
        if (i == 7 ? ct2h : ct1h) {
          f.b_cell = kWPrepBoundCell0 + nb;
          f.ext_cell = i == 7 ? cell7 : cell9;
          wb[nb++] = i == 7 ? WPrepBound{P + o.w[10], P + o.b[10], 256, 128, sqrtf((float)Sq), 0}
                            : WPrepBound{P + o.w[11], P + o.b[11], 128, 64, sqrtf((float)Sh), 0};
          (i == 7 ? bound7 : bound9) = true;
        } else {
          f.w = nullptr;
        }
      }
      sg[2 * (i - 1) + 1].w = P + o.w[i];
      any = 1;
    }
    if (any) {
      NC_TRY(wprep_run(sg, 18, wb, nb, V + p.wprep, prep, hs));
      kept_mask |= kKeptWPrep;
    }
  }
  auto prep_of = [&](int seg) -> const S3xPrepared* { return prep[seg].wp ? &prep[seg] : nullptr; };
  auto block = [&](int i, const float* in, float* out, size_t out_stride, int to, int to_ctot) -> int {
    const UBlock& b = kUB[i];
    const int* d = p.d[b.lvl];
    const long S = p.S[b.lvl];
    const bool epi = pre[i] && h2l[i] && sw::raw(sw::EPI_STATS) == 2 && s3x_stats_bytes(N, d[0], d[1], d[2], b.K, 3) && s3x_stats_bytes(N, d[0], d[1], d[2], b.K, 3) <= p.in_ws;
    if (pre[i]) {
      NC_TRY(conv_fwd_pre(V + p.xs3[i], P + o.w[i], P + o.b[i], V + p.raw[i], N, b.C, d[0], d[1], d[2], b.K, 3, cws, p.conv_ws, stream,
                          epi ? (float*)iws : nullptr, i >= 1 ? prep_of(2 * (i - 1)) : nullptr));
      kept_mask |= 1u << i;
      if (h2l[i]) kept_mask |= 1u << (16 + i);
    } else {
      bool kept1 = false;
      NC_TRY(conv_fwd_keep(in, P + o.w[i], P + o.b[i], V + p.raw[i], N, b.C, d[0], d[1], d[2], b.K, 3, cws, p.conv_ws, stream,
                           i >= 1 ? (void*)(V + p.xs3[i]) : nullptr, &kept1, i >= 1 ? prep_of(2 * (i - 1)) : nullptr));
      if (kept1) kept_mask |= 1u << i;
      if (kept1 && i >= 1 && conv_layer_h2(cd[i])) kept_mask |= 1u << (16 + i);
    }
    if (epi) NC_TRY(s3x_stats_finalize((const float*)iws, P + o.b[i], N, d[0], d[1], d[2], b.K, 3, 1e-5f, V + p.mean[i], V + p.rstd[i], hs));
    else NC_TRY(nc_instnorm_stats(V + p.raw[i], N * b.K, S, 1e-5f, V + p.mean[i], V + p.rstd[i], iws, p.in_ws, stream));
    if (to >= 0 && use[to]) {
      const int lj = lean && h2l[to] && to_ctot == b.K ? lean_index(to) : -1;
      if (lj >= 0) { out = nullptr; kept_mask |= 1u << (kLeanBit0 + lj); }
      NC_TRY(act_operand(cd[to], V + p.raw[i], V + p.mean[i], V + p.rstd[i], 0.f, out, (long)out_stride, V + p.xs3[to], N, b.K, S, to_ctot, 0, hs));
      if (to_ctot == b.K) pre[to] = true;
      return NC_OK;
    }
    if (out_stride == (size_t)b.K * S || N == 1)
      return nc_instnorm_act_fwd(V + p.raw[i], V + p.mean[i], V + p.rstd[i], 0.f, out, N * b.K, S, stream);
    for (int n = 0; n < N; ++n)
      NC_TRY(nc_instnorm_act_fwd(V + p.raw[i] + (size_t)n * b.K * S, V + p.mean[i] + n * b.K, V + p.rstd[i] + n * b.K, 0.f,
                                 out + n * out_stride, b.K, S, stream));
    return NC_OK;
  };
  NC_TRY(block(0, x, V + p.a1, (size_t)64 * S, 1, 64));
  NC_TRY(block(1, V + p.a1, V + p.cat1, (size_t)128 * S, 9, 128));
  const bool pool_arg = sw::get(sw::IN_BWD_FOLD) != 0;
  if (pool_arg) kept_mask |= kKeptPoolArg;
  for (int n = 0; n < N; ++n) {
    if (pool_arg)
      NC_TRY(maxpool2_fwd_arg(V + p.cat1 + (size_t)n * 128 * S, V + p.p1 + (size_t)n * 64 * Sh, (unsigned char*)(V + p.parg[0]) + (size_t)n * 64 * Sh, 64,
                              d0[0], d0[1], d0[2], hs));
    else
      NC_TRY(nc_maxpool2_fwd(V + p.cat1 + (size_t)n * 128 * S, V + p.p1 + (size_t)n * 64 * Sh, 64, d0[0], d0[1], d0[2], stream));
  }
  NC_TRY(block(2, V + p.p1, V + p.a2, (size_t)128 * Sh, 3, 128));
  NC_TRY(block(3, V + p.a2, V + p.cat2, (size_t)256 * Sh, 7, 256));
  for (int n = 0; n < N; ++n) {
    if (pool_arg)
      NC_TRY(maxpool2_fwd_arg(V + p.cat2 + (size_t)n * 256 * Sh, V + p.p2 + (size_t)n * 128 * Sq, (unsigned char*)(V + p.parg[1]) + (size_t)n * 128 * Sq,
                              128, d1[0], d1[1], d1[2], hs));
    else
      NC_TRY(nc_maxpool2_fwd(V + p.cat2 + (size_t)n * 256 * Sh, V + p.p2 + (size_t)n * 128 * Sq, 128, d1[0], d1[1], d1[2], stream));
  }
  NC_TRY(block(4, V + p.p2, V + p.b1, (size_t)256 * Sq, 5, 256));
  NC_TRY(block(5, V + p.b1, V + p.b2, (size_t)256 * Sq, 6, 256));
  NC_TRY(block(6, V + p.b2, V + p.b3, (size_t)256 * Sq, -1, 0));
  if (ct2h && !bound7) {
    NC_TRY(h2_zero_cells(cell7, 1, hs));
    NC_TRY(convT_h2_bound(P + o.w[10], P + o.b[10], 256, 128, sqrtf((float)Sq), cell7, hs));
  }
  for (int n = 0; n < N; ++n) {
    if (ct2h)
      NC_TRY(convT_fwd_split_h2(V + p.b3 + (size_t)n * 256 * Sq, P + o.w[10], P + o.b[10], V + p.cat2 + ((size_t)n * 256 + 128) * Sh,
                                (char*)(V + p.xs3[7]) + (size_t)n * 256 * Sh * 4, 256, 128, 1, 256, d2[0], d2[1], d2[2], 128, cell7, cws, p.conv_ws, hs));
    else if (ct2)
      NC_TRY(nc_convT_k2s2_fwd_split(V + p.b3 + (size_t)n * 256 * Sq, nullptr, P + o.w[10], P + o.b[10], V + p.cat2 + ((size_t)n * 256 + 128) * Sh,
                                     use[7] && !h2l[7] ? (char*)(V + p.xs3[7]) + (size_t)n * 256 * Sh * 6 : nullptr, 256, 128, 1, 256, d2[0], d2[1], d2[2], 128, cws,
                                     p.conv_ws, stream));
    else
      NC_TRY(nc_convT_k2s2_fwd(V + p.b3 + (size_t)n * 256 * Sq, P + o.w[10], P + o.b[10], V + p.cat2 + ((size_t)n * 256 + 128) * Sh,
                               1, 256, d2[0], d2[1], d2[2], 128, stream));
  }
  if (use[7]) {
    if (!ct2 || (h2l[7] && !ct2h)) NC_TRY(operand_into(cd[7], V + p.cat2 + (size_t)128 * Sh, (long)256 * Sh, V + p.xs3[7], N, 128, Sh, 256, 128, hs));
    pre[7] = true;
  }
  NC_TRY(block(7, V + p.cat2, V + p.e2a, (size_t)128 * Sh, 8, 128));
  NC_TRY(block(8, V + p.e2a, V + p.e2b, (size_t)128 * Sh, -1, 0));
  const bool ct_s3 = use[9] && !h2l[9] && (ct1 || convT_fwd_s3_supported(1, 128, d1[0], d1[1], d1[2], 64));
  if (ct1h && !bound9) {
    NC_TRY(h2_zero_cells(cell9, 1, hs));
    NC_TRY(convT_h2_bound(P + o.w[11], P + o.b[11], 128, 64, sqrtf((float)Sh), cell9, hs));
  }
  for (int n = 0; n < N; ++n) {
    if (ct1h)
      NC_TRY(convT_fwd_split_h2(V + p.e2b + (size_t)n * 128 * Sh, P + o.w[11], P + o.b[11], V + p.cat1 + ((size_t)n * 128 + 64) * S,
                                (char*)(V + p.xs3[9]) + (size_t)n * 128 * S * 4, 128, 64, 1, 128, d1[0], d1[1], d1[2], 64, cell9, cws, p.conv_ws, hs));
    else if (ct1)
      NC_TRY(nc_convT_k2s2_fwd_split(V + p.e2b + (size_t)n * 128 * Sh, nullptr, P + o.w[11], P + o.b[11], V + p.cat1 + ((size_t)n * 128 + 64) * S,
                                     use[9] && !h2l[9] ? (char*)(V + p.xs3[9]) + (size_t)n * 128 * S * 6 : nullptr, 128, 64, 1, 128, d1[0], d1[1], d1[2], 64, cws,
                                     p.conv_ws, stream));
    else if (ct_s3)
      NC_TRY(convT_fwd_s3(V + p.e2b + (size_t)n * 128 * Sh, P + o.w[11], P + o.b[11], V + p.cat1 + ((size_t)n * 128 + 64) * S,
                          (char*)(V + p.xs3[9]) + (size_t)n * 128 * S * 6, 128, 64, 1, 128, d1[0], d1[1], d1[2], 64, stream));
    else
      NC_TRY(nc_convT_k2s2_fwd(V + p.e2b + (size_t)n * 128 * Sh, P + o.w[11], P + o.b[11], V + p.cat1 + ((size_t)n * 128 + 64) * S,
                               1, 128, d1[0], d1[1], d1[2], 64, stream));
  }
  if (use[9]) {
    if (!ct_s3 && !ct1h) NC_TRY(operand_into(cd[9], V + p.cat1 + (size_t)64 * S, (long)128 * S, V + p.xs3[9], N, 64, S, 128, 64, hs));
    pre[9] = true;
  }
  NC_TRY(block(9, V + p.cat1, V + p.e1, (size_t)64 * S, -1, 0));
  NC_TRY(nc_conv_fwd(V + p.e1, P + o.w[12], P + o.b[12], V + p.t1, N, 64, d0[0], d0[1], d0[2], 1, 1, 1, 1, 1, 0, cws, p.conv_ws, stream));
  NC_TRY(nc_conv_fwd(V + p.t1, P + o.w[13], P + o.b[13], y, N, 1, d0[0], d0[1], d0[2], 1, 1, 1, 1, 1, 0, cws, p.conv_ws, stream));
  if (kept) *kept = kept_mask;
  return nc_sigmoid_fwd(y, y, (long)N * S, stream);
}

int nc_unet_deconv_bwd(const float* params, const float* x, const float* y, const float* saved, const float* dy, float* dx,
                       float* dparams, int N, int S0, int S1, int S2, void* ws, size_t ws_bytes, void* stream, unsigned kept) {
  NetworkScope net_scope;
  if (!params || !x || !y || !saved || !dy || !dparams) { set_error("unet_deconv_bwd: null pointer"); return NC_ERR_ARG; }
  UPlan p;
  if (!u_plan(p, N, S0, S1, S2)) { set_error("unet_deconv_bwd: bad shape"); return NC_ERR_SHAPE; }
  if (!ws || ws_bytes < u_ws_bytes(p, true)) { set_error("unet_deconv_bwd: workspace too small"); return NC_ERR_WS; }
  const UOff o = u_offsets();
  hipStream_t hs = (hipStream_t)stream;
  void* cws = ws;
  void* iws = (char*)ws + align256(p.conv_ws);
  void* tws = (char*)iws + align256(p.in_ws);
  float* G = (float*)((char*)tws + align256(p.convT_ws));
  const float* V = saved;
  const float* P = params;
  float* DP = dparams;
  const long S = p.S[0], Sh = p.S[1], Sq = p.S[2];
  const int *d0 = p.d[0], *d1 = p.d[1], *d2 = p.d[2];
  const unsigned kept_mask = kept;
  const bool fuse_bwd = sw::raw(sw::S3_TRAIN_FUSE) != 0;
  const bool wprep_now = sw::raw(sw::UNET_WPREP) != 0;
  S3xPrepared prepd[10] = {};
  {
    WPrepSeg sg[18];
    wprep_segs(sg);
    const char* region = (const char*)(V + p.wprep);
    size_t off = kWPrepCellBytes;
    for (int k = 0; k < 18; ++k) {
      if (k & 1) prepd[k / 2 + 1] = S3xPrepared{region + off, (const unsigned*)region + k};
      off += s3x_packed_bytes(sg[k].Cin, sg[k].Kout, 3, 2);
    }
  }
  auto block_bwd = [&](int i, const float* g, const float* in, float* draw, float* gin, bool r1 = false, const float* pool = nullptr) -> int {
    const UBlock& b = kUB[i];
    const int* d = p.d[b.lvl];
    const long Sl = p.S[b.lvl];
    ConvDims cdk;
    const bool now_h2 = make_dims(cdk, N, b.C, d[0], d[1], d[2], b.K, 3, 3, 3, 1, 1) && conv_layer_h2(cdk);
    const void* xs = ((kept_mask >> i) & 1) && (((kept_mask >> (16 + i)) & 1) != 0) == now_h2 ? (const void*)(V + p.xs3[i]) : nullptr;
    const S3xPrepared* pd = i >= 1 && gin && now_h2 && (kept_mask & kKeptWPrep) && ((kept_mask >> (16 + i)) & 1) && wprep_now ? &prepd[i] : nullptr;
    const int lj = lean_index(i);
    if (lj >= 0 && ((kept_mask >> (kLeanBit0 + lj)) & 1) &&
        !(xs && !h2_guard_can_flip() && conv_bwd_pre_supported(N, b.C, d[0], d[1], d[2], b.K, 3, gin != nullptr, p.conv_ws))) {
      NC_TRY(nc_instnorm_act_fwd(V + p.raw[i - 1], V + p.mean[i - 1], V + p.rstd[i - 1], 0.f, G + p.T, N * b.C, Sl, stream));
      in = G + p.T;
    }
    if (r1) {
      NC_TRY(instnorm_act_bwd_dbias_h2_rank1(g, P + o.w[12], V + p.raw[i], V + p.mean[i], V + p.rstd[i], 0.f, cws, DP + o.b[i], b.K, Sl, iws, p.in_ws,
                                             stream, conv_bwd_guard_words(cws, N, b.K, Sl)));
      return conv_bwd_pre(in, xs, P + o.w[i], gin, DP + o.w[i], N, b.C, d[0], d[1], d[2], b.K, 3, cws, p.conv_ws, stream, h2_guard_can_flip(), pd);
    }
    if (fuse_bwd && i >= 1 && conv_bwd_pre_supported(N, b.C, d[0], d[1], d[2], b.K, 3, gin != nullptr, p.conv_ws) &&
        instnorm_bwd_s3_supported(N, b.K, Sl)) {
      if (now_h2 && pool)
        NC_TRY(instnorm_act_bwd_dbias_h2_pool(g, (long)2 * b.K * Sl, pool, (const unsigned char*)(V + p.parg[i == 1 ? 0 : 1]), V + p.raw[i], V + p.mean[i],
                                              V + p.rstd[i], 0.f, cws, DP + o.b[i], N, b.K, d[0], d[1], d[2], iws, p.in_ws, stream,
                                              conv_bwd_guard_words(cws, N, b.K, Sl)));
      else if (now_h2)
        NC_TRY(instnorm_act_bwd_dbias_h2(g, V + p.raw[i], V + p.mean[i], V + p.rstd[i], 0.f, cws, DP + o.b[i], N, b.K, Sl, iws, p.in_ws, stream,
                                         conv_bwd_guard_words(cws, N, b.K, Sl)));
      else
        NC_TRY(instnorm_act_bwd_dbias_s3(g, V + p.raw[i], V + p.mean[i], V + p.rstd[i], 0.f, cws, DP + o.b[i], N, b.K, Sl, iws, p.in_ws, stream));
      return conv_bwd_pre(in, xs, P + o.w[i], gin, DP + o.w[i], N, b.C, d[0], d[1], d[2], b.K, 3, cws, p.conv_ws, stream, now_h2 && h2_guard_can_flip(), pd);
    }
    if (pool) { set_error("unet_deconv_bwd: block %d left the path its pooled gradient was planned for", i); return NC_ERR_ARG; }
    NC_TRY(nc_instnorm_act_bwd_dbias(g, V + p.raw[i], V + p.mean[i], V + p.rstd[i], 0.f, draw, DP + o.b[i], N, b.K, Sl, iws,
                                     p.in_ws, stream));
    return conv_bwd_keep(in, xs, draw, P + o.w[i], gin, DP + o.w[i], N, b.C, d[0], d[1], d[2], b.K, 3, cws, p.conv_ws, stream);
  };
  auto pool_folds = [&](int i) -> bool {
    const UBlock& b = kUB[i];
    const int* d = p.d[b.lvl];
    ConvDims cdk;
    return (kept_mask & kKeptPoolArg) && fuse_bwd && make_dims(cdk, N, b.C, d[0], d[1], d[2], b.K, 3, 3, 3, 1, 1) && conv_layer_h2(cdk) &&
           conv_bwd_pre_supported(N, b.C, d[0], d[1], d[2], b.K, 3, true, p.conv_ws) &&
           instnorm_bwd_h2_pool_supported(N, b.K, d[0], d[1], d[2], conv_bwd_guard_words(cws, N, b.K, p.S[b.lvl]));
  };
  auto upper_half = [&](const float* dcat, int Ctot, long Sl, const float** out) -> int {
    const int C = Ctot / 2;
    if (N == 1) { *out = dcat + (size_t)C * Sl; return NC_OK; }
    NC_TRY(gather_half(dcat, G + p.T, N, Ctot, C, C, Sl, hs));
    *out = G + p.T;
    return NC_OK;
  };
  NC_TRY(nc_sigmoid_bwd(dy, y, G + p.s1, (long)N * S, stream));
  NC_TRY(nc_conv_wgrad(V + p.t1, G + p.s1, DP + o.w[13], DP + o.b[13], N, 1, d0[0], d0[1], d0[2], 1, 1, 1, 1, 1, 0, cws, p.conv_ws, stream));
  NC_TRY(nc_conv_dgrad(G + p.s1, P + o.w[13], G + p.s2, N, 1, d0[0], d0[1], d0[2], 1, 1, 1, 1, 1, 0, cws, p.conv_ws, stream));
  ConvDims cd9;
  const bool r1 = sw::raw(sw::UNET_LEAN) != 0 && N == 1 && fuse_bwd &&
                  make_dims(cd9, N, 128, d0[0], d0[1], d0[2], 64, 3, 3, 3, 1, 1) && conv_layer_h2(cd9) &&
                  conv_bwd_pre_supported(N, 128, d0[0], d0[1], d0[2], 64, 3, true, p.conv_ws) && instnorm_bwd_s3_supported(N, 64, S);
  NC_TRY(nc_conv_wgrad(V + p.e1, G + p.s2, DP + o.w[12], DP + o.b[12], N, 64, d0[0], d0[1], d0[2], 1, 1, 1, 1, 1, 0, cws, p.conv_ws, stream));
  if (!r1) {
    NC_TRY(nc_conv_dgrad(G + p.s2, P + o.w[12], G + p.G1, N, 64, d0[0], d0[1], d0[2], 1, 1, 1, 1, 1, 0, cws, p.conv_ws, stream));
  }
  NC_TRY(block_bwd(9, r1 ? G + p.s2 : G + p.G1, V + p.cat1, G + p.G2, G + p.G3, r1));
  const float* g;
  NC_TRY(upper_half(G + p.G3, 128, S, &g));
  NC_TRY(nc_convT_k2s2_dgrad(g, P + o.w[11], G + p.H1, N, 128, d1[0], d1[1], d1[2], 64, tws, p.convT_ws, stream));
  NC_TRY(nc_convT_k2s2_wgrad(V + p.e2b, g, DP + o.w[11], DP + o.b[11], N, 128, d1[0], d1[1], d1[2], 64, tws, p.convT_ws, stream));
  NC_TRY(block_bwd(8, G + p.H1, V + p.e2a, G + p.H2, G + p.H1));
  NC_TRY(block_bwd(7, G + p.H1, V + p.cat2, G + p.H2, G + p.H3));
  NC_TRY(upper_half(G + p.H3, 256, Sh, &g));
  NC_TRY(nc_convT_k2s2_dgrad(g, P + o.w[10], G + p.Q1, N, 256, d2[0], d2[1], d2[2], 128, tws, p.convT_ws, stream));
  NC_TRY(nc_convT_k2s2_wgrad(V + p.b3, g, DP + o.w[10], DP + o.b[10], N, 256, d2[0], d2[1], d2[2], 128, tws, p.convT_ws, stream));
  NC_TRY(block_bwd(6, G + p.Q1, V + p.b2, G + p.Q2, G + p.Q1));
  NC_TRY(block_bwd(5, G + p.Q1, V + p.b1, G + p.Q2, G + p.Q1));
  NC_TRY(block_bwd(4, G + p.Q1, V + p.p2, G + p.Q2, G + p.Q1));
  if (pool_folds(3)) {
    NC_TRY(block_bwd(3, G + p.H3, V + p.a2, G + p.H2, G + p.H1, false, G + p.Q1));
  } else {
    for (int n = 0; n < N; ++n)
      NC_TRY(nc_maxpool2_bwd_add(G + p.Q1 + (size_t)n * 128 * Sq, V + p.cat2 + (size_t)n * 256 * Sh, G + p.H3 + (size_t)n * 256 * Sh,
                                 G + p.H1 + (size_t)n * 128 * Sh, 128, d1[0], d1[1], d1[2], stream));
    NC_TRY(block_bwd(3, G + p.H1, V + p.a2, G + p.H2, G + p.H1));
  }
  NC_TRY(block_bwd(2, G + p.H1, V + p.p1, G + p.H2, G + p.H1));
  if (pool_folds(1)) {
    NC_TRY(block_bwd(1, G + p.G3, V + p.a1, G + p.G2, G + p.G1, false, G + p.H1));
  } else {
    for (int n = 0; n < N; ++n)
      NC_TRY(nc_maxpool2_bwd_add(G + p.H1 + (size_t)n * 64 * Sh, V + p.cat1 + (size_t)n * 128 * S, G + p.G3 + (size_t)n * 128 * S,
                                 G + p.G1 + (size_t)n * 64 * S, 64, d0[0], d0[1], d0[2], stream));
    NC_TRY(block_bwd(1, G + p.G1, V + p.a1, G + p.G2, G + p.G1));
  }
  return block_bwd(0, G + p.G1, x, G + p.G2, dx);
}

}

namespace {

struct LLayer { int C, K, k; };
const LLayer kLL[6] = {{1, 64, 7}, {64, 64, 5}, {64, 64, 3}, {64, 32, 1}, {32, 16, 1}, {16, 1, 1}};

struct LPlan {
  int N, d[3];
  long S;
  size_t w[6], params;
  size_t act[5], saved;
  size_t xs3[6];
  size_t g[2], grads;
  size_t conv_ws;
};

struct LTail {
  static constexpr size_t a = 0, e = 32 * 8, r = e + 64 * 8, E = r + 64 * 8, Ef = E + 1728 * 4, q = Ef + 1728 * 4, P = q + 1728 * 4 + 256,
                          Wf = P + (size_t)64 * 32 * 125 * 4 + 256, bytes = Wf + (size_t)64 * 32 * 125 * 4 + 256;
};

__global__ void __launch_bounds__(256) k_dl_shift27(const float* __restrict__ dy, float* __restrict__ dsh, int D, int H, int W) {
  const long S = (long)D * H * W;
  const int a = blockIdx.y, n = blockIdx.z;
  float* out = dsh + ((long)n * 32 + a) * S;
  const float* in = dy + (long)n * S;
  const int az = a / 9 - 1, ay = (a / 3) % 3 - 1, ax = a % 3 - 1;
  for (long v = (long)blockIdx.x * 256 + threadIdx.x; v < S; v += (long)gridDim.x * 256) {
    float r = 0.f;
    if (a < 27) {
      const int x = (int)(v % W), y = (int)((v / W) % H), z = (int)(v / ((long)W * H));
      const int sx = x - ax, sy = y - ay, sz = z - az;
      if ((unsigned)sx < (unsigned)W && (unsigned)sy < (unsigned)H && (unsigned)sz < (unsigned)D) r = in[((long)sz * H + sy) * W + sx];
    }
    out[v] = r;
  }
}
__global__ void __launch_bounds__(128) k_dl_w1_fold(const float* __restrict__ E, const float* __restrict__ w1, float* __restrict__ wf) {
  const int c = blockIdx.x, a = blockIdx.y, sidx = threadIdx.x;
  if (sidx >= 125) return;
  double v = 0.0;
  if (a < 27)
    for (int k = 0; k < 64; ++k) v += (double)w1[((long)k * 64 + c) * 125 + 124 - sidx] * (double)E[k * 27 + a];
  wf[((long)c * 32 + a) * 125 + sidx] = (float)v;
}
__global__ void __launch_bounds__(128) k_dl_fold_fwd(const float* __restrict__ E, const float* __restrict__ w1, float* __restrict__ F) {
// ... 402 lines not shown
```

neuroclear_amd/csrc/h2.hip:

```cpp
#include <mutex>

#include "common.hpp"
#include "s3_common.hpp"

namespace nc {
namespace {

__global__ void __launch_bounds__(256) k_absmax(const float* __restrict__ x, long n, unsigned* __restrict__ cell, unsigned* __restrict__ cell2) {
  unsigned m = 0;
  const int head = (int)((4 - (((unsigned long long)x >> 2) & 3)) & 3) < n ? (int)((4 - (((unsigned long long)x >> 2) & 3)) & 3) : (int)n;
  if (blockIdx.x == 0 && (int)threadIdx.x < head) {
    const unsigned b = __float_as_uint(x[threadIdx.x]) & 0x7fffffffu;
    if (b < 0x7f800000u && b > m) m = b;
  }
  x += head;
  n -= head;
  const long n4 = n >> 2;
  const float4* x4 = reinterpret_cast<const float4*>(x);
  auto take = [&](const float4& v) __attribute__((always_inline)) {
    const unsigned b[4] = {__float_as_uint(v.x) & 0x7fffffffu, __float_as_uint(v.y) & 0x7fffffffu, __float_as_uint(v.z) & 0x7fffffffu,
                           __float_as_uint(v.w) & 0x7fffffffu};
#pragma unroll
    for (int j = 0; j < 4; ++j)
      if (b[j] < 0x7f800000u && b[j] > m) m = b[j];
// ... 51 lines not shown
        if (b < 0x7f800000u && b > m) m = b;
        h2_split(f * sc, e[j]);
      }
#pragma unroll
      for (int t = 0; t < 2; ++t) out[(ob * 2 + t) * S + v] = s3_unit(e, t);
    }
    if (guard) {
      const unsigned thr = cb_bits > kGuardDrop ? cb_bits - kGuardDrop : 0u;
      const bool any_hi = __builtin_amdgcn_ballot_w64(m >= thr && m != 0) != 0;
      const bool any_nz = __builtin_amdgcn_ballot_w64(m != 0) != 0;
      if (any_nz) {
        ++n_all;
        if (!any_hi) ++n_low;
      }
    }
  }
  if (!guard) return;
  __shared__ unsigned cnt[2];
  if (threadIdx.x < 2) cnt[threadIdx.x] = 0;
  __syncthreads();
  if ((threadIdx.x & 63) == 0) {
    if (n_all) atomicAdd(&cnt[kGuardAll], n_all);
    if (n_low) atomicAdd(&cnt[kGuardLow], n_low);
  }
  __syncthreads();
  if (threadIdx.x < 2 && cnt[threadIdx.x]) atomicAdd(guard + threadIdx.x, cnt[threadIdx.x]);
}

__global__ void k_h2_guard_decide(unsigned* ga, unsigned* gb, unsigned* prior, unsigned* flag, int can_flip, unsigned long long* stats,
                                  unsigned long long total_a) {
  if (threadIdx.x || blockIdx.x) return;
  h2_guard_decide_one(ga, gb, prior, flag, can_flip, stats, total_a);
}

__global__ void __launch_bounds__(256) k_h2_to_s3_if(const uint4* __restrict__ in, uint4* __restrict__ out, long S, int cblocks,
                                                      const unsigned* __restrict__ cells, const unsigned* __restrict__ guard) {
  if (guard_skip(guard, 1)) return;
  const long v = (long)blockIdx.x * 256 + threadIdx.x;
  if (v >= S) return;
  const int cb = blockIdx.y % cblocks;
  const float inv = h2_inv_scale(cells[cb >= cblocks / 2 ? 1 : 0]);
  const long b = blockIdx.y;
  const uint4 a = in[(b * 2 + 0) * S + v], r = in[(b * 2 + 1) * S + v];
  const unsigned aw[4] = {a.x, a.y, a.z, a.w}, rw[4] = {r.x, r.y, r.z, r.w};
  unsigned short e[8][3];
#pragma unroll
  for (int j = 0; j < 8; ++j) {
    const unsigned short h0 = (unsigned short)(aw[j >> 1] >> ((j & 1) * 16)), h1 = (unsigned short)(rw[j >> 1] >> ((j & 1) * 16));
    const float val = ((float)__builtin_bit_cast(_Float16, h0) + (float)__builtin_bit_cast(_Float16, h1)) * inv;
    s3_split(val, e[j]);
  }
#pragma unroll
  for (int t = 0; t < 3; ++t) out[(b * 3 + t) * S + v] = s3_unit(e, t);
}

__global__ void __launch_bounds__(256) k_act_split2h(const float* __restrict__ x, const float* __restrict__ mean, const float* __restrict__ rstd,
                                                     float slope, float* __restrict__ y, long ystride, uint4* __restrict__ out, long S, int cblocks,
                                                     int oblocks, int ob0, unsigned bound_bits, unsigned* __restrict__ cell, unsigned* __restrict__ cell2) {
  if (blockIdx.x == 0 && blockIdx.y == 0 && threadIdx.x == 0) {
    if (cell) *cell = bound_bits;
    if (cell2) *cell2 = bound_bits;
  }
  const long v = (long)blockIdx.x * 256 + threadIdx.x;
  if (v >= S) return;
  const float sc = h2_scale(bound_bits);
  const int n = blockIdx.y / cblocks, cb = blockIdx.y % cblocks;
  const long c0 = (long)blockIdx.y * 8;
  const float* xs = x + c0 * S + v;
  float* ys = y ? y + (long)n * ystride + (long)cb * 8 * S + v : nullptr;
  unsigned short e[8][3];
#pragma unroll
  for (int j = 0; j < 8; ++j) {
    float t = (xs[j * S] - mean[c0 + j]) * rstd[c0 + j];
    t = t > 0.f ? t : t * slope;
    if (ys) ys[j * S] = t;
    asm("" : "+v"(t));
    h2_split(t * sc, e[j]);
  }
  const long ob = (long)n * oblocks + ob0 + cb;
#pragma unroll
  for (int t = 0; t < 2; ++t) out[(ob * 2 + t) * S + v] = s3_unit(e, t);
}

__global__ void __launch_bounds__(256) k_act_split2h_pool(const float* __restrict__ x, const float* __restrict__ mean, const float* __restrict__ rstd,
                                                          float slope, uint4* __restrict__ out, uint4* __restrict__ pooled, int D, int H, int W,
                                                          int cblocks, int oblocks, int ob0, unsigned bound_bits, unsigned* __restrict__ cell) {
  if (blockIdx.x == 0 && blockIdx.y == 0 && threadIdx.x == 0 && cell) *cell = bound_bits;
  const int Do = D / 2, Ho = H / 2, Wo = W / 2;
  const long So = (long)Do * Ho * Wo, S = (long)D * H * W;
  const long v = (long)blockIdx.x * 256 + threadIdx.x;
  if (v >= So) return;
  const int xo = (int)(v % Wo), yo = (int)((v / Wo) % Ho), zo = (int)(v / ((long)Wo * Ho));
  const float sc = h2_scale(bound_bits);
  const int n = blockIdx.y / cblocks, cb = blockIdx.y % cblocks;
  const long c0 = (long)blockIdx.y * 8;
  const long ob = (long)n * oblocks + ob0 + cb;
  float m[8], r[8];
#pragma unroll
  for (int j = 0; j < 8; ++j) { m[j] = mean[c0 + j]; r[j] = rstd[c0 + j]; }
  float best[8];
  unsigned short w0[8], w1[8];
#pragma unroll
  for (int kp = 0; kp < 4; ++kp) {
    const long u = ((long)(2 * zo + (kp >> 1)) * H + (2 * yo + (kp & 1))) * W + 2 * xo;
    unsigned short e[2][8][3];
#pragma unroll
    for (int j = 0; j < 8; ++j) {
      const float2 xv = *reinterpret_cast<const float2*>(x + (c0 + j) * S + u);
      float t0 = (xv.x - m[j]) * r[j], t1 = (xv.y - m[j]) * r[j];
      t0 = t0 > 0.f ? t0 : t0 * slope;
      t1 = t1 > 0.f ? t1 : t1 * slope;
      asm("" : "+v"(t0), "+v"(t1));
      h2_split(t0 * sc, e[0][j]);
      h2_split(t1 * sc, e[1][j]);
    }
#pragma unroll
    for (int h = 0; h < 2; ++h) {
#pragma unroll
      for (int t = 0; t < 2; ++t) out[(ob * 2 + t) * S + u + h] = s3_unit(e[h], t);
      const int k = (kp >> 1) * 4 + (kp & 1) * 2 + h;
#pragma unroll
      for (int j = 0; j < 8; ++j) {
        const float val = (float)__builtin_bit_cast(_Float16, e[h][j][0]) + (float)__builtin_bit_cast(_Float16, e[h][j][1]);
        if (val > best[j] || k == 0) { best[j] = val; w0[j] = e[h][j][0]; w1[j] = e[h][j][1]; }
      }
    }
  }
  uint4 o0, o1;
  o0.x = w0[0] | ((unsigned)w0[1] << 16); o0.y = w0[2] | ((unsigned)w0[3] << 16); o0.z = w0[4] | ((unsigned)w0[5] << 16); o0.w = w0[6] | ((unsigned)w0[7] << 16);
  o1.x = w1[0] | ((unsigned)w1[1] << 16); o1.y = w1[2] | ((unsigned)w1[3] << 16); o1.z = w1[4] | ((unsigned)w1[5] << 16); o1.w = w1[6] | ((unsigned)w1[7] << 16);
  uint4* o = pooled + ((long)n * cblocks + cb) * 2 * So;
  o[v] = o0;
  o[So + v] = o1;
}

__global__ void __launch_bounds__(256) k_maxpool2_h2(const uint4* __restrict__ in, uint4* __restrict__ out, int cblocks, int iblocks, int D, int H,
                                                     int W) {
  const int Do = D / 2, Ho = H / 2, Wo = W / 2;
  const long So = (long)Do * Ho * Wo, S = (long)D * H * W;
  const long v = (long)blockIdx.x * 256 + threadIdx.x;
  if (v >= So) return;
  const int n = blockIdx.y / cblocks, cb = blockIdx.y % cblocks;
  const int xo = (int)(v % Wo), yo = (int)((v / Wo) % Ho), zo = (int)(v / ((long)Wo * Ho));
  const uint4* i0 = in + ((long)n * iblocks + cb) * 2 * S;
  float best[8];
  unsigned short t0[8], t1[8];
#pragma unroll
  for (int j = 0; j < 8; ++j) { best[j] = -3.0e38f; t0[j] = 0; t1[j] = 0; }
#pragma unroll
  for (int k = 0; k < 8; ++k) {
    const long u = ((long)(2 * zo + (k >> 2)) * H + (2 * yo + ((k >> 1) & 1))) * W + 2 * xo + (k & 1);
    const uint4 a = i0[u], b = i0[S + u];
    const unsigned aw[4] = {a.x, a.y, a.z, a.w}, bw[4] = {b.x, b.y, b.z, b.w};
#pragma unroll
    for (int j = 0; j < 8; ++j) {
      const unsigned short h0 = (unsigned short)(aw[j >> 1] >> ((j & 1) * 16)), h1 = (unsigned short)(bw[j >> 1] >> ((j & 1) * 16));
      const float val = (float)__builtin_bit_cast(_Float16, h0) + (float)__builtin_bit_cast(_Float16, h1);
      if (val > best[j] || k == 0) { best[j] = val; t0[j] = h0; t1[j] = h1; }
    }
  }
  uint4 o0, o1;
  o0.x = t0[0] | ((unsigned)t0[1] << 16); o0.y = t0[2] | ((unsigned)t0[3] << 16); o0.z = t0[4] | ((unsigned)t0[5] << 16); o0.w = t0[6] | ((unsigned)t0[7] << 16);
  o1.x = t1[0] | ((unsigned)t1[1] << 16); o1.y = t1[2] | ((unsigned)t1[3] << 16); o1.z = t1[4] | ((unsigned)t1[5] << 16); o1.w = t1[6] | ((unsigned)t1[7] << 16);
  uint4* o = out + ((long)n * cblocks + cb) * 2 * So;
  o[v] = o0;
  o[So + v] = o1;
}

}

int maxpool2_h2(const void* in, void* out, int N, int C, int ctot, int D, int H, int W, hipStream_t s) {
  if (C % 8 || ctot % 8 || (D | H | W) & 1) { set_error("maxpool2_h2: channels % 8, even extents"); return NC_ERR_SHAPE; }
  const long So = (long)(D / 2) * (H / 2) * (W / 2);
  hipLaunchKernelGGL(k_maxpool2_h2, dim3((unsigned)cdiv(So, 256), (unsigned)(N * C / 8)), dim3(256), 0, s, (const uint4*)in, (uint4*)out, C / 8, ctot / 8, D, H,
                     W);
  return check_launch("maxpool2_h2");
}

int h2_zero_cells(unsigned* cells, int n, hipStream_t s) {
  hipLaunchKernelGGL(k_set_cells, dim3(1), dim3(64), 0, s, cells, n, 0u);
  return check_launch("h2_zero_cells");
}
int h2_set_cell(unsigned* cell, float bound, hipStream_t s) {
  unsigned bits;
  static_assert(sizeof(bits) == sizeof(bound), "");
  __builtin_memcpy(&bits, &bound, 4);
  hipLaunchKernelGGL(k_set_cells, dim3(1), dim3(64), 0, s, cell, 1, bits);
  return check_launch("h2_set_cell");
}
int h2_absmax(const float* x, long n, unsigned* cell, hipStream_t s, unsigned* cell2) {
  if ((unsigned long long)x & 3) { set_error("h2_absmax: the tensor must be 4-byte aligned"); return NC_ERR_ARG; }
  long blocks = cdiv(n, 256 * 4 * 8);
  if (blocks > 1024) blocks = 1024;
  if (blocks < 1) blocks = 1;
  hipLaunchKernelGGL(k_absmax, dim3((unsigned)blocks), dim3(256), 0, s, x, n, cell, cell2);
  return check_launch("h2_absmax");
}
int split2h_into(const float* x, long xstride, void* xs, int N, int C, long S, int ctot, int c0, const unsigned* cell, hipStream_t s, unsigned* guard) {
  if (C % 8 || ctot % 8 || c0 % 8) { set_error("split2h: channels must be multiples of 8"); return NC_ERR_SHAPE; }
  long bx = cdiv(S, 256);
  const long ny = (long)N * C / 8;
  if (guard && sw::get(sw::H2_GUARD) && bx * ny > 4096) bx = cdiv(4096, ny) < bx ? cdiv(4096, ny) : bx;
  hipLaunchKernelGGL(k_split2h, dim3((unsigned)bx, (unsigned)ny), dim3(256), 0, s, x, (uint4*)xs, S, C / 8, ctot / 8, c0 / 8, xstride,
                     cell, sw::get(sw::H2_GUARD) ? guard : nullptr);
  return check_launch("split2h");
}

namespace {
std::mutex g_stats_mu;
unsigned long long* g_stats_host = nullptr;
unsigned long long* g_stats_dev = nullptr;
unsigned long long* guard_stats_dev() {
  std::lock_guard<std::mutex> lk(g_stats_mu);
  if (!g_stats_host) {
    void* h = nullptr;
    if (hipHostMalloc(&h, 64, hipHostMallocMapped | hipHostMallocPortable) != hipSuccess) { (void)hipGetLastError(); return nullptr; }
    __builtin_memset(h, 0, 64);
    void* d = nullptr;
    if (hipHostGetDevicePointer(&d, h, 0) != hipSuccess) { (void)hipGetLastError(); (void)hipHostFree(h); return nullptr; }
    g_stats_host = (unsigned long long*)h;
    g_stats_dev = (unsigned long long*)d;
  }
  return g_stats_dev;
}
}
int h2_guard_read(unsigned long long* out4, int reset) {
  std::lock_guard<std::mutex> lk(g_stats_mu);
  for (int i = 0; i < 4; ++i) {
    if (!g_stats_host) out4[i] = 0;
    else out4[i] = reset ? __atomic_exchange_n(g_stats_host + i, 0ull, __ATOMIC_RELAXED) : __atomic_load_n(g_stats_host + i, __ATOMIC_RELAXED);
  }
  return NC_OK;
}
unsigned long long* h2_guard_stats_dev() { return guard_stats_dev(); }
int h2_guard_zero(unsigned* g, hipStream_t s, int nwords) {
  hipLaunchKernelGGL(k_set_cells, dim3(1), dim3(64), 0, s, g, nwords, 0u);
  return check_launch("h2_guard_zero");
}
int h2_guard_decide(unsigned* ga, unsigned* gb, unsigned* prior, unsigned* flag, bool can_flip, hipStream_t s, unsigned long long total_a) {
  if (!sw::get(sw::H2_GUARD) && !prior) return NC_OK;
  hipLaunchKernelGGL(k_h2_guard_decide, dim3(1), dim3(64), 0, s, ga, gb, prior, flag, can_flip ? 1 : 0, guard_stats_dev(), total_a);
  return check_launch("h2_guard_decide");
}
int h2_to_s3_if(const void* xh, void* xs, int N, int C, long S, const unsigned* cells, const unsigned* guard, hipStream_t s) {
  if (C % 8) { set_error("h2_to_s3: channels must be a multiple of 8"); return NC_ERR_SHAPE; }
  hipLaunchKernelGGL(k_h2_to_s3_if, dim3((unsigned)cdiv(S, 256), (unsigned)(N * C / 8)), dim3(256), 0, s, (const uint4*)xh, (uint4*)xs, S, C / 8, cells, guard);
  return check_launch("h2_to_s3_if");
}
int act_split2h(const float* x, const float* mean, const float* rstd, float slope, float* y, long ystride, void* ys, int N, int C, long S, int ctot,
                int c0, float bound, unsigned* cell, unsigned* cell2, hipStream_t s) {
  if (C % 8 || ctot % 8 || c0 % 8) { set_error("act_split2h: channels must be multiples of 8"); return NC_ERR_SHAPE; }
  unsigned bits;
  __builtin_memcpy(&bits, &bound, 4);
  hipLaunchKernelGGL(k_act_split2h, dim3((unsigned)cdiv(S, 256), (unsigned)(N * C / 8)), dim3(256), 0, s, x, mean, rstd, slope, y, ystride,
                     (uint4*)ys, S, C / 8, ctot / 8, c0 / 8, bits, cell, cell2);
  return check_launch("act_split2h");
}

int act_split2h_pool(const float* x, const float* mean, const float* rstd, float slope, void* ys, void* pooled, int N, int C, int D, int H, int W,
                     int ctot, int c0, float bound, unsigned* cell, hipStream_t s) {
  if (C % 8 || ctot % 8 || c0 % 8 || ((D | H | W) & 1)) { set_error("act_split2h_pool: channels % 8, even extents"); return NC_ERR_SHAPE; }
  if ((((uintptr_t)x) & 7) != 0) { set_error("act_split2h_pool: input not 8-byte aligned"); return NC_ERR_ARG; }
  unsigned bits;
  __builtin_memcpy(&bits, &bound, 4);
  const long So = (long)(D / 2) * (H / 2) * (W / 2);
  hipLaunchKernelGGL(k_act_split2h_pool, dim3((unsigned)cdiv(So, 256), (unsigned)(N * C / 8)), dim3(256), 0, s, x, mean, rstd, slope, (uint4*)ys,
                     (uint4*)pooled, D, H, W, C / 8, ctot / 8, c0 / 8, bits, cell);
  return check_launch("act_split2h_pool");
}

}
```

neuroclear_amd/csrc/h2_debug.hip:

```cpp
#include <cmath>

#include "common.hpp"

using namespace nc;

extern "C" {

size_t nc_h2_bytes(int N, int C, long S) {
  if (N < 1 || C < 1 || S < 1) return 0;
  return h2_cells_offset((size_t)N * C * S) + 256;
}
size_t nc_h2_cells_offset(size_t elems) { return h2_cells_offset(elems); }

static bool h2_part_ok(int N, int C, long S, int ctot, int c0) {
  return N >= 1 && C >= 8 && S >= 1 && C % 8 == 0 && ctot % 8 == 0 && c0 % 8 == 0 && c0 >= 0 && c0 + C <= ctot && (long)N * C / 8 <= 65535;
}

int nc_to_h2_debug(const float* x, long xstride, void* xs, int N, int C, long S, int ctot, int c0, unsigned* cell, float bound, unsigned* guard,
                   void* stream) {
  if (!x || !xs || !cell) { set_error("to_h2_debug: null pointer"); return NC_ERR_ARG; }
  if (!h2_part_ok(N, C, S, ctot, c0) || xstride < (long)C * S) { set_error("to_h2_debug: bad shape"); return NC_ERR_SHAPE; }
  hipStream_t s = (hipStream_t)stream;
  if (bound > 0.f) {
    if (int e = h2_set_cell(cell, bound, s)) return e;
  } else {
    if (int e = h2_zero_cells(cell, 1, s)) return e;
    for (int n = 0; n < N; ++n)
      if (int e = h2_absmax(x + (long)n * xstride, (long)C * S, cell, s)) return e;
  }
  if (guard)
    if (int e = h2_guard_zero(guard, s)) return e;
  return split2h_into(x, xstride, xs, N, C, S, ctot, c0, cell, s, guard);
}

int nc_act_split2h_debug(const float* x, const float* mean, const float* rstd, float slope, float* y, long ystride, void* ys, int N, int C, long S,
                         int ctot, int c0, float bound, unsigned* cell, unsigned* cell2, void* stream) {
  if (!x || !mean || !rstd || !ys) { set_error("act_split2h_debug: null pointer"); return NC_ERR_ARG; }
  if (!h2_part_ok(N, C, S, ctot, c0) || (y && ystride < (long)C * S) || !(bound > 0.f)) { set_error("act_split2h_debug: bad shape"); return NC_ERR_SHAPE; }
  return act_split2h(x, mean, rstd, slope, y, ystride, ys, N, C, S, ctot, c0, bound, cell, cell2, (hipStream_t)stream);
}

int nc_act_split2h_pool_debug(const float* x, const float* mean, const float* rstd, float slope, void* ys, void* pooled, int N, int C, int D, int H,
                              int W, int ctot, int c0, float bound, unsigned* cell, void* stream) {
  if (!x || !mean || !rstd || !ys || !pooled) { set_error("act_split2h_pool_debug: null pointer"); return NC_ERR_ARG; }
  if (D < 2 || H < 2 || W < 2 || !h2_part_ok(N, C, (long)D * H * W, ctot, c0) || !(bound > 0.f)) { set_error("act_split2h_pool_debug: bad shape"); return NC_ERR_SHAPE; }
  return act_split2h_pool(x, mean, rstd, slope, ys, pooled, N, C, D, H, W, ctot, c0, bound, cell, (hipStream_t)stream);
}

int nc_maxpool2_h2_debug(const void* in, void* out, int N, int C, int ctot, int D, int H, int W, void* stream) {
  if (!in || !out) { set_error("maxpool2_h2_debug: null pointer"); return NC_ERR_ARG; }
  if (D < 2 || H < 2 || W < 2 || !h2_part_ok(N, C, (long)D * H * W, ctot, 0)) { set_error("maxpool2_h2_debug: bad shape"); return NC_ERR_SHAPE; }
  return maxpool2_h2(in, out, N, C, ctot, D, H, W, (hipStream_t)stream);
}

int nc_h2_to_s3_if_debug(const void* xh, void* xs, int N, int C, long S, const unsigned* cells, const unsigned* guard, void* stream) {
  if (!xh || !xs || !cells) { set_error("h2_to_s3_if_debug: null pointer"); return NC_ERR_ARG; }
  if (!h2_part_ok(N, C, S, C, 0)) { set_error("h2_to_s3_if_debug: bad shape"); return NC_ERR_SHAPE; }
  return h2_to_s3_if(xh, xs, N, C, S, cells, guard, (hipStream_t)stream);
}

int nc_instnorm_act_bwd_dbias_h2_debug(const float* dy, const float* w1, const float* x, const float* mean, const float* rstd, float slope, void* dxs,
                                       float* dbias, int N, int C, long S, void* ws, size_t ws_bytes, unsigned* guard, void* stream) {
  if (w1) {
    if (N != 1) { set_error("instnorm_act_bwd_dbias_h2_debug: the rank-one form takes one sample"); return NC_ERR_ARG; }
    return instnorm_act_bwd_dbias_h2_rank1(dy, w1, x, mean, rstd, slope, dxs, dbias, C, S, ws, ws_bytes, stream, guard);
  }
  return instnorm_act_bwd_dbias_h2(dy, x, mean, rstd, slope, dxs, dbias, N, C, S, ws, ws_bytes, stream, guard);
}

int nc_instnorm_act_bwd_dbias_h2_pool_debug(const float* dy, long dy_stride, const float* gp, const unsigned char* arg, const float* x, const float* mean,
                                            const float* rstd, float slope, void* dxs, float* dbias, int N, int C, int D, int H, int W, void* ws,
                                            size_t ws_bytes, unsigned* guard, void* stream) {
  NetworkScope net_scope;
  if (D < 1 || H < 1 || W < 1) { set_error("instnorm_act_bwd_dbias_h2_pool_debug: bad shape"); return NC_ERR_SHAPE; }
  if (!gp && !arg) {
    if (dy_stride != (long)C * D * H * W) { set_error("instnorm_act_bwd_dbias_h2_pool_debug: the plain form takes a dense gradient"); return NC_ERR_ARG; }
    return instnorm_act_bwd_dbias_h2(dy, x, mean, rstd, slope, dxs, dbias, N, C, (long)D * H * W, ws, ws_bytes, stream, guard);
  }
  return instnorm_act_bwd_dbias_h2_pool(dy, dy_stride, gp, arg, x, mean, rstd, slope, dxs, dbias, N, C, D, H, W, ws, ws_bytes, stream, guard);
}
int nc_maxpool2_fwd_arg_debug(const float* x, float* y, unsigned char* arg, int NC, int D, int H, int W, void* stream) {
  return maxpool2_fwd_arg(x, y, arg, NC, D, H, W, (hipStream_t)stream);
}

static size_t al256(size_t b) { return (b + 255) & ~(size_t)255; }
size_t nc_convT_k2s2_split_h2_ws_bytes(int N, int C, int D, int H, int W, int K) {
  if (!convT_s3x_supported(N, C, D, H, W, K)) return 0;
  return al256(convT_s3x_ws_bytes(C, K)) + h2_cells_offset((size_t)N * C * D * H * W) + 256;
}
int nc_convT_k2s2_fwd_split_h2_debug(const float* x, const float* w, const float* bias, float* y, void* ys, int ys_ctot, int ys_c0, int N, int C,
                                     int D, int H, int W, int K, unsigned* out_cell, void* ws, size_t ws_bytes, void* stream) {
  if (!x || !w || !ys || !out_cell || !ws) { set_error("convT_k2s2_fwd_split_h2_debug: null pointer"); return NC_ERR_ARG; }
  if (!convT_s3x_supported(N, C, D, H, W, K) || ys_ctot % 8 || ys_c0 % 8 || ys_c0 < 0 || ys_c0 + K > ys_ctot) {
    set_error("convT_k2s2_fwd_split_h2_debug: shape not covered");
    return NC_ERR_SHAPE;
  }
  hipStream_t s = (hipStream_t)stream;
  if (int e = h2_zero_cells(out_cell, 1, s)) return e;
  if (int e = convT_h2_bound(w, bias, C, K, sqrtf((float)((long)D * H * W)), out_cell, s)) return e;
  return convT_fwd_split_h2(x, w, bias, y, ys, ys_ctot, ys_c0, N, C, D, H, W, K, out_cell, ws, ws_bytes, s);
}

int nc_convT_k2s2_fwd_s3_debug(const float* x, const float* w, const float* bias, float* y, void* ys, int ys_ctot, int ys_c0, int N, int C, int D,
                               int H, int W, int K, void* stream) {
  if (N < 1 || C < 1 || D < 1 || H < 1 || W < 1 || K < 1 || ys_ctot < 8 || ys_ctot % 8 || ys_c0 % 8 || ys_c0 < 0 || (long)ys_c0 + K > ys_ctot) {
    set_error("convT_k2s2_fwd_s3_debug: shape not covered");
    return NC_ERR_SHAPE;
  }
  return convT_fwd_s3(x, w, bias, y, ys, ys_ctot, ys_c0, N, C, D, H, W, K, stream);
}

int nc_instnorm_relu_tail_sigmoid_debug(const float* x, const float* mean, const float* rstd, const float* w1, const float* b1, const float* w2,
                                        const float* b2, float* y, int C, long S, void* stream) {
  if (!x || !mean || !rstd || !w1 || !b1 || !w2 || !b2 || !y) { set_error("instnorm_relu_tail_sigmoid_debug: null pointer"); return NC_ERR_ARG; }
  if (C < 1 || S < 1) { set_error("instnorm_relu_tail_sigmoid_debug: bad shape"); return NC_ERR_SHAPE; }
  return instnorm_relu_tail_sigmoid(x, mean, rstd, w1, b1, w2, b2, y, C, S, (hipStream_t)stream);
}

}
```

neuroclear_amd/csrc/norm_act.hip:

```cpp
#include <atomic>

#include "common.hpp"
#include "s3_common.hpp"

namespace nc {

static constexpr int kMaxSplits = 64;

static int pick_splits(int NC, long S) {
  long want = cdiv(2048, NC);
  long cap = cdiv(S, 8192);
  long s = want < cap ? want : cap;
  if (s < 1) s = 1;
  if (s > kMaxSplits) s = kMaxSplits;
  return (int)s;
}

__device__ __forceinline__ void block_reduce2(double& a, double& b, double* out2) {
  __shared__ double red[2][4];
  for (int o = 32; o > 0; o >>= 1) {
    a += __shfl_down(a, o);
    b += __shfl_down(b, o);
  }
  const int lane = threadIdx.x & 63, wv = threadIdx.x >> 6;
  if (lane == 0) {
    red[0][wv] = a;
    red[1][wv] = b;
  }
  __syncthreads();
  if (threadIdx.x == 0) {
    out2[0] = (red[0][0] + red[0][1]) + (red[0][2] + red[0][3]);
    out2[1] = (red[1][0] + red[1][1]) + (red[1][2] + red[1][3]);
  }
}

__device__ __forceinline__ void chunk_range(long S, int splits, int sp, long& b, long& e) {
  long chunk = (S + splits - 1) / splits;
  chunk = (chunk + 3) & ~3L;
  b = (long)sp * chunk;
  e = b + chunk < S ? b + chunk : S;
  if (b > S) b = S;
}

__global__ __launch_bounds__(256) void k_in_stats(const float* __restrict__ x, long S, int splits,
                                                  double* __restrict__ part) {
  const int inst = blockIdx.y, sp = blockIdx.x;
  long b, e;
  chunk_range(S, splits, sp, b, e);
  const float* p = x + (long)inst * S;
  double s = 0.0, q = 0.0;
  if ((S & 3) == 0 && ((uintptr_t)x & 15) == 0) {
    const float4* p4 = reinterpret_cast<const float4*>(p);
    for (long i = b / 4 + threadIdx.x; i < e / 4; i += 256) {
      const float4 v = p4[i];
      const double a0 = v.x, a1 = v.y, a2 = v.z, a3 = v.w;
      s += (a0 + a1) + (a2 + a3);
      q = fma(a0, a0, q); q = fma(a1, a1, q); q = fma(a2, a2, q); q = fma(a3, a3, q);
    }
  } else {
    for (long i = b + threadIdx.x; i < e; i += 256) {
      const double a = p[i];
      s += a;
      q = fma(a, a, q);
    }
  }
  block_reduce2(s, q, part + ((long)inst * splits + sp) * 2);
}

__global__ void k_in_finalize(const double* __restrict__ part, int NC, int splits, long S, float eps,
                              float* __restrict__ mean, float* __restrict__ rstd) {
  const int i = blockIdx.x * blockDim.x + threadIdx.x;
  if (i >= NC) return;
  double s = 0.0, q = 0.0;
  for (int k = 0; k < splits; ++k) {
    s += part[((long)i * splits + k) * 2];
    q += part[((long)i * splits + k) * 2 + 1];
  }
  const double m = s / (double)S;
  double var = q / (double)S - m * m;
  if (var < 0.0) var = 0.0;
  mean[i] = (float)m;
  rstd[i] = (float)(1.0 / sqrt(var + (double)eps));
}

__global__ __launch_bounds__(256) void k_in_act_fwd(const float* __restrict__ x, const float* __restrict__ mean,
                                                    const float* __restrict__ rstd, float slope,
                                                    float* __restrict__ y, long S) {
  const int inst = blockIdx.y;
  const float m = mean[inst], r = rstd[inst];
  const float* p = x + (long)inst * S;
  float* o = y + (long)inst * S;
  if ((S & 3) == 0 && (((uintptr_t)x | (uintptr_t)y) & 15) == 0) {
    const float4* p4 = reinterpret_cast<const float4*>(p);
    float4* o4 = reinterpret_cast<float4*>(o);
    for (long i = (long)blockIdx.x * 256 + threadIdx.x; i < S / 4; i += (long)gridDim.x * 256) {
      float4 v = p4[i];
      v.x = (v.x - m) * r; v.y = (v.y - m) * r; v.z = (v.z - m) * r; v.w = (v.w - m) * r;
      v.x = v.x > 0.f ? v.x : v.x * slope; v.y = v.y > 0.f ? v.y : v.y * slope;
      v.z = v.z > 0.f ? v.z : v.z * slope; v.w = v.w > 0.f ? v.w : v.w * slope;
      o4[i] = v;
    }
  } else {
    for (long i = (long)blockIdx.x * 256 + threadIdx.x; i < S; i += (long)gridDim.x * 256) {
      const float v = (p[i] - m) * r;
      o[i] = v > 0.f ? v : v * slope;
    }
  }
}

template <int U = 1>
__global__ __launch_bounds__(256) void k_in_bwd_sums(const float* __restrict__ dy, const float* __restrict__ x,
                                                     const float* __restrict__ mean, const float* __restrict__ rstd,
                                                     float slope, long S, int splits, double* __restrict__ part) {
  const int inst = blockIdx.y, sp = blockIdx.x;
  long b, e;
  chunk_range(S, splits, sp, b, e);
  const float m = mean[inst], r = rstd[inst];
  const float* px = x + (long)inst * S;
  const float* pg = dy + (long)inst * S;
  double s1 = 0.0, s2 = 0.0;
  auto add = [&](float xv, float gy) {
    const float xh = (xv - m) * r;
    const float g = xh > 0.f ? gy : gy * slope;
    s1 += (double)g;
    s2 = fma((double)g, (double)xh, s2);
  };
  long i = b + threadIdx.x;
  if constexpr (U > 1) {
    for (; i + (long)(U - 1) * 256 < e; i += (long)U * 256) {
      float xv[U], gv[U];
#pragma unroll
      for (int k = 0; k < U; ++k) xv[k] = px[i + k * 256];
#pragma unroll
      for (int k = 0; k < U; ++k) gv[k] = pg[i + k * 256];
#pragma unroll
      for (int k = 0; k < U; ++k) add(xv[k], gv[k]);
    }
  }
  for (; i < e; i += 256) add(px[i], pg[i]);
  block_reduce2(s1, s2, part + ((long)inst * splits + sp) * 2);
}

__device__ __forceinline__ float in_bwd_value(float xv, float gy, float m, float r, float m1, float m2, float slope) {
  const float xh = (xv - m) * r;
  const float g = xh > 0.f ? gy : gy * slope;
  float p = xh * m2;
  asm("" : "+v"(p));
  return r * ((g - m1) - p);
}

template <int U = 1>
__global__ __launch_bounds__(256) void k_in_bwd_apply(const float* __restrict__ dy, const float* __restrict__ x,
                                                      const float* __restrict__ mean, const float* __restrict__ rstd,
                                                      float slope, long S, int splits,
                                                      const double* __restrict__ part, float* __restrict__ dx,
                                                      double* __restrict__ rowpart) {
  const int inst = blockIdx.y;
  const float* px = x + (long)inst * S;
  const float* pg = dy + (long)inst * S;
  float* o = dx + (long)inst * S;
  const long st = (long)gridDim.x * 256;
  long i = (long)blockIdx.x * 256 + threadIdx.x;
  float xv[U], gv[U];
  bool round = U > 1 && i + (U - 1) * st < S;
  if constexpr (U > 1) {
    if (round) {
#pragma unroll
      for (int k = 0; k < U; ++k) xv[k] = px[i + k * st];
#pragma unroll
      for (int k = 0; k < U; ++k) gv[k] = pg[i + k * st];
    }
  }
  double s1 = 0.0, s2 = 0.0;
  int k0 = 0;
  if constexpr (U > 1) {
    for (; k0 + 8 <= splits; k0 += 8) {
      double a[8], b[8];
#pragma unroll
      for (int j = 0; j < 8; ++j) { a[j] = part[((long)inst * splits + k0 + j) * 2]; b[j] = part[((long)inst * splits + k0 + j) * 2 + 1]; }
#pragma unroll
      for (int j = 0; j < 8; ++j) { s1 += a[j]; s2 += b[j]; }
    }
  }
  for (int k = k0; k < splits; ++k) {
    s1 += part[((long)inst * splits + k) * 2];
    s2 += part[((long)inst * splits + k) * 2 + 1];
  }
  const float m1 = (float)(s1 / (double)S), m2 = (float)(s2 / (double)S);
  const float m = mean[inst], r = rstd[inst];
// ... 518 lines not shown
      rs[j] += (double)t;
      asm("" : "+v"(t));
      const unsigned b = __float_as_uint(t) & 0x7fffffffu;
      if (b < 0x7f800000u && b > mx) mx = b;
      h2_split(t * sc, e[j]);
    }
#pragma unroll
    for (int t = 0; t < 2; ++t) dxs[(ncb * 2 + t) * S + v] = s3_unit(e, t);
    if (guard) {
      const unsigned thr = cbits > kGuardDrop ? cbits - kGuardDrop : 0u;
      const bool any_hi = __builtin_amdgcn_ballot_w64(mx >= thr && mx != 0) != 0;
      const bool any_nz = __builtin_amdgcn_ballot_w64(mx != 0) != 0;
      if (!any_nz) ++n_zero;
      else if (!any_hi) ++n_low;
    }
  }
  if (guard && (threadIdx.x & 63) == 0) {
    if (n_low) atomicAdd(guard + kGuardLow, n_low);
    if (n_zero) atomicAdd(guard + kGuardAll, n_zero);
  }
  if (rowpart) {
    const int lane = threadIdx.x & 63, wv = threadIdx.x >> 6;
#pragma unroll
    for (int j = 0; j < 8; ++j) {
      double a = rs[j];
      for (int of = 32; of > 0; of >>= 1) a += __shfl_down(a, of);
      if (lane == 0) red[j][wv] = a;
    }
    __syncthreads();
    if (threadIdx.x < 8)
      rowpart[(ncb * 8 + threadIdx.x) * gridDim.x + blockIdx.x] =
          (red[threadIdx.x][0] + red[threadIdx.x][1]) + (red[threadIdx.x][2] + red[threadIdx.x][3]);
  }
}


__global__ void k_lrelu_fwd(const float* __restrict__ x, float slope, float* __restrict__ y, long n) {
  for (long i = (long)blockIdx.x * blockDim.x + threadIdx.x; i < n; i += (long)gridDim.x * blockDim.x) {
    const float v = x[i];
    y[i] = v > 0.f ? v : v * slope;
  }
}
__global__ void k_lrelu_bwd(const float* __restrict__ dy, const float* __restrict__ x, float slope,
                            float* __restrict__ dx, long n) {
  for (long i = (long)blockIdx.x * blockDim.x + threadIdx.x; i < n; i += (long)gridDim.x * blockDim.x)
    dx[i] = x[i] > 0.f ? dy[i] : dy[i] * slope;
}
__global__ void __launch_bounds__(256) k_in_act_tail(const float* __restrict__ x, const float* __restrict__ mean, const float* __restrict__ rstd,
                                                     const float* __restrict__ w1, const float* __restrict__ b1, const float* __restrict__ w2,
                                                     const float* __restrict__ b2, float* __restrict__ y, long S, int C) {
  __shared__ float sm[3][256];
  for (int c = threadIdx.x; c < C; c += 256) { sm[0][c] = mean[c]; sm[1][c] = rstd[c]; sm[2][c] = w1[c]; }
  __syncthreads();
  const long v = (long)blockIdx.x * 256 + threadIdx.x;
  if (v >= S) return;
  float acc = 0.f;
  for (int c = 0; c < C; ++c) {
    float t = (x[(long)c * S + v] - sm[0][c]) * sm[1][c];
    t = t > 0.f ? t : 0.f;
    acc = fmaf(sm[2][c], t, acc);
  }
  const float t1 = acc + b1[0];
  const float t2 = fmaf(w2[0], t1, b2[0]);
  y[v] = 1.f / (1.f + expf(-t2));
}

__global__ void k_sigmoid_fwd(const float* __restrict__ x, float* __restrict__ y, long n) {
  for (long i = (long)blockIdx.x * blockDim.x + threadIdx.x; i < n; i += (long)gridDim.x * blockDim.x)
    y[i] = 1.f / (1.f + expf(-x[i]));
}
__global__ void k_sigmoid_bwd(const float* __restrict__ dy, const float* __restrict__ y, float* __restrict__ dx,
                              long n) {
  for (long i = (long)blockIdx.x * blockDim.x + threadIdx.x; i < n; i += (long)gridDim.x * blockDim.x) {
    const float s = y[i];
    dx[i] = dy[i] * s * (1.f - s);
  }
}

__device__ __forceinline__ int pool_winner(const float* __restrict__ p, int od, int oh, int ow, int H, int W, int wd, float& best) {
  best = -INFINITY;
  int arg = 0;
  for (int a = 0; a < wd; ++a)
    for (int b = 0; b < 2; ++b)
      for (int c = 0; c < 2; ++c) {
        const float v = p[((long)(od * wd + a) * H + (oh * 2 + b)) * W + ow * 2 + c];
        if (v > best || v != v) {
          best = v;
          arg = (a * 2 + b) * 2 + c;
        }
      }
  return arg;
}

template <bool ARG>
__global__ void k_maxpool2_fwd(const float* __restrict__ x, float* __restrict__ y, unsigned char* __restrict__ arg, int NC, int D, int H, int W,
                               int Do, int Ho, int Wo, int wd) {
  const long total = (long)NC * Do * Ho * Wo;
  for (long i = (long)blockIdx.x * blockDim.x + threadIdx.x; i < total; i += (long)gridDim.x * blockDim.x) {
    const int ow = (int)(i % Wo), oh = (int)((i / Wo) % Ho), od = (int)((i / ((long)Wo * Ho)) % Do);
    const long nc = i / ((long)Wo * Ho * Do);
    float best;
    const int a = pool_winner(x + nc * D * H * W, od, oh, ow, H, W, wd, best);
    y[i] = best;
    if (ARG) arg[i] = (unsigned char)a;
  }
}

template <bool SKIP>
__global__ void k_maxpool2_bwd(const float* __restrict__ dy, const float* __restrict__ x, const float* __restrict__ skip,
                               float* __restrict__ dx, int NC, int D, int H, int W, int Do, int Ho, int Wo, int wd) {
  const long total = (long)NC * Do * Ho * Wo;
  for (long i = (long)blockIdx.x * blockDim.x + threadIdx.x; i < total; i += (long)gridDim.x * blockDim.x) {
    const int ow = (int)(i % Wo), oh = (int)((i / Wo) % Ho), od = (int)((i / ((long)Wo * Ho)) % Do);
    const long nc = i / ((long)Wo * Ho * Do);
    float* q = dx + nc * D * H * W;
    float best;
    const int arg = pool_winner(x + nc * D * H * W, od, oh, ow, H, W, wd, best);
    const float g = dy[i];
    for (int a = 0; a < wd; ++a)
      for (int b = 0; b < 2; ++b)
        for (int c = 0; c < 2; ++c) {
          const long o = ((long)(od * wd + a) * H + (oh * 2 + b)) * W + ow * 2 + c;
          const float v = ((a * 2 + b) * 2 + c) == arg ? g : 0.f;
          q[o] = SKIP ? skip[nc * D * H * W + o] + v : v;
        }
  }
}

static void launch_in_bwd_sums(const float* dy, const float* x, const float* mean, const float* rstd, float slope, long S, int splits, int NC,
                               double* part, hipStream_t s) {
  if (sw::get(sw::STREAM_PASSES)) hipLaunchKernelGGL(k_in_bwd_sums<8>, dim3(splits, NC), dim3(256), 0, s, dy, x, mean, rstd, slope, S, splits, part);
  else hipLaunchKernelGGL(k_in_bwd_sums<1>, dim3(splits, NC), dim3(256), 0, s, dy, x, mean, rstd, slope, S, splits, part);
}
static void launch_in_bwd_apply(const float* dy, const float* x, const float* mean, const float* rstd, float slope, long S, int splits, int NC,
                                long bx, const double* part, float* dx, double* rowpart, hipStream_t s) {
  if (sw::get(sw::STREAM_PASSES))
    hipLaunchKernelGGL(k_in_bwd_apply<4>, dim3((unsigned)bx, NC), dim3(256), 0, s, dy, x, mean, rstd, slope, S, splits, part, dx, rowpart);
  else
    hipLaunchKernelGGL(k_in_bwd_apply<1>, dim3((unsigned)bx, NC), dim3(256), 0, s, dy, x, mean, rstd, slope, S, splits, part, dx, rowpart);
}

static unsigned flat_grid(long n, int per_block = 256) {
  long b = cdiv(n, per_block);
  if (b > 16384) b = 16384;
  if (b < 1) b = 1;
  return (unsigned)b;
}

}

using namespace nc;

__global__ void k_bn_finalize(const double* __restrict__ part, int N, int C, int splits, long S, float eps, float momentum,
                              float* __restrict__ mean, float* __restrict__ rstd, float* __restrict__ running_mean,
                              float* __restrict__ running_var) {
  const int c = blockIdx.x * blockDim.x + threadIdx.x;
  if (c >= C) return;
  double s = 0.0, q = 0.0;
  for (int n = 0; n < N; ++n)
    for (int k = 0; k < splits; ++k) {
      s += part[(((long)n * C + c) * splits + k) * 2];
      q += part[(((long)n * C + c) * splits + k) * 2 + 1];
    }
  const double M = (double)N * (double)S;
  const double m = s / M;
  double var = q / M - m * m;
  if (var < 0.0) var = 0.0;
  mean[c] = (float)m;
  rstd[c] = (float)(1.0 / sqrt(var + (double)eps));
  if (running_mean) running_mean[c] = (float)((1.0 - (double)momentum) * (double)running_mean[c] + (double)momentum * m);
  if (running_var) {
    const double unb = M > 1.0 ? var * M / (M - 1.0) : var;
    running_var[c] = (float)((1.0 - (double)momentum) * (double)running_var[c] + (double)momentum * unb);
// ... 518 lines not shown
```

Measured before the change: 56.01 million.

## Fuse instance-norm activation into 1x1 conv operand loads and pool-arg split kernel

Adds NORM template variants of the flat 1x1 forward and 1x1 wgrad kernels that apply instance-norm plus leaky-ReLU to the raw input as it is read from LDS. This avoids materialising the activated tensor. The lean-E1 path in the network backward calls the fused wgrad directly, and falls back to an explicit instnorm_act pass otherwise. It also adds an ARG variant of the split-h2 pooling kernel that emits float pooled values and argmax indices, so a separate maxpool pass is not needed. The trade-off is extra ALU work inside the MFMA loops and extra per-instance mean and rstd loads.

Result: faster. 56.77 million, median of 6 (+1.4%).

```diff
diff --git a/include/nc_hip.h b/include/nc_hip.h
--- a/include/nc_hip.h
+++ b/include/nc_hip.h
@@ -335,6 +335,12 @@
                                             const float* rstd, float slope, void* dxs, float* dbias, int N, int C, int D, int H, int W, void* ws,
                                             size_t ws_bytes, unsigned* guard, void* stream);
 int nc_maxpool2_fwd_arg_debug(const float* x, float* y, unsigned char* arg, int NC, int D, int H, int W, void* stream);
+int nc_act_split2h_pool_arg_debug(const float* x, const float* mean, const float* rstd, float slope, void* ys, float* pooled, unsigned char* arg, int N,
+                                  int C, int D, int H, int W, int ctot, int c0, float bound, unsigned* cell, void* stream);
+int nc_conv_fwd_norm_1x1_debug(const float* raw, const float* mean, const float* rstd, float slope, const float* w, const float* bias, float* y, int N,
+                               int C, int D, int H, int W, int K, void* ws, size_t ws_bytes, void* stream);
+int nc_conv_wgrad_norm_1x1_debug(const float* raw, const float* mean, const float* rstd, float slope, const float* dy, float* dw, float* dbias, int N,
+                                 int C, int D, int H, int W, int K, void* ws, size_t ws_bytes, void* stream);
 size_t nc_convT_k2s2_split_h2_ws_bytes(int N, int C, int D, int H, int W, int K);
 int nc_convT_k2s2_fwd_split_h2_debug(const float* x, const float* w, const float* bias, float* y, void* ys, int ys_ctot, int ys_c0, int N, int C,
                                      int D, int H, int W, int K, unsigned* out_cell, void* ws, size_t ws_bytes, void* stream);
diff --git a/neuroclear_amd/csrc/api.hip b/neuroclear_amd/csrc/api.hip
--- a/neuroclear_amd/csrc/api.hip
+++ b/neuroclear_amd/csrc/api.hip
@@ -509,6 +509,32 @@
   return make_dims(d, N, C, D, H, W, K, ks, ks, ks, 1, ks / 2) && fwd_path(d) == 9;
 }
 
+bool norm_1x1_taken(int N, int C, int D, int H, int W, int K) {
+  ConvDims d;
+  return make_dims(d, N, C, D, H, W, K, 1, 1, 1, 1, 0) && fwd_path(d) == 3 && wgrad_path(d) == 3 && norm_1x1_supported(d);
+}
+int conv_fwd_norm_1x1(const float* raw, const float* mean, const float* rstd, float slope, const float* w, const float* bias, float* y, int N, int C,
+                      int D, int H, int W, int K, void* ws, size_t ws_bytes, void* stream) {
+  ConvDims d;
+  if (int e = conv_args("conv_fwd_norm_1x1", d, raw, w, y, N, C, D, H, W, K, 1, 1, 1, 1, 0)) return e;
+  if (!mean || !rstd) { set_error("conv_fwd_norm_1x1: null pointer"); return NC_ERR_ARG; }
+  ProfScope ps(0, 3, d, 0, (hipStream_t)stream);
+  return conv_fwd_1x1_norm(raw, mean, rstd, slope, w, bias, y, d, ws, ws_bytes, (hipStream_t)stream);
+}
+int conv_wgrad_norm_1x1(const float* raw, const float* mean, const float* rstd, float slope, const float* dy, float* dw, float* dbias, int N, int C,
+                        int D, int H, int W, int K, void* ws, size_t ws_bytes, void* stream) {
+  ConvDims d;
+  if (int e = conv_args("conv_wgrad_norm_1x1", d, raw, dy, dw, N, C, D, H, W, K, 1, 1, 1, 1, 0)) return e;
+  if (!mean || !rstd) { set_error("conv_wgrad_norm_1x1: null pointer"); return NC_ERR_ARG; }
+  hipStream_t s = (hipStream_t)stream;
+  {
+    ProfScope ps(2, 3, d, 0, s);
+    if (int e = conv_wgrad_1x1_norm(raw, mean, rstd, slope, dy, dw, d, ws, ws_bytes, s)) return e;
+  }
+  if (dbias) return bias_grad(dy, dbias, d.N, d.K, (long)d.Do * d.Ho * d.Wo, ws, ws_bytes, s);
+  return NC_OK;
+}
+
 int conv_fwd_pre(const void* xs, const float* w, const float* bias, float* y, int N, int C, int D, int H, int W, int K, int ks, void* ws,
                  size_t ws_bytes, void* stream, float* stats_part, const S3xPrepared* prep) {
   ConvDims d;
@@ -561,3 +587,16 @@
   return nc_conv_bwd(x, dy, w, dx, dw, nullptr, N, C, D, H, W, K, ks, ks, ks, 1, ks / 2, ws, ws_bytes, stream);
 }
 }
+
+extern "C" {
+int nc_conv_fwd_norm_1x1_debug(const float* raw, const float* mean, const float* rstd, float slope, const float* w, const float* bias, float* y, int N,
+                               int C, int D, int H, int W, int K, void* ws, size_t ws_bytes, void* stream) {
+  if (!norm_1x1_taken(N, C, D, H, W, K)) { set_error("conv_fwd_norm_1x1_debug: the flat 1 x 1 kernels do not take this layer"); return NC_ERR_SHAPE; }
+  return conv_fwd_norm_1x1(raw, mean, rstd, slope, w, bias, y, N, C, D, H, W, K, ws, ws_bytes, stream);
+}
+int nc_conv_wgrad_norm_1x1_debug(const float* raw, const float* mean, const float* rstd, float slope, const float* dy, float* dw, float* dbias, int N,
+                                 int C, int D, int H, int W, int K, void* ws, size_t ws_bytes, void* stream) {
+  if (!norm_1x1_taken(N, C, D, H, W, K)) { set_error("conv_wgrad_norm_1x1_debug: the flat 1 x 1 kernels do not take this layer"); return NC_ERR_SHAPE; }
+  return conv_wgrad_norm_1x1(raw, mean, rstd, slope, dy, dw, dbias, N, C, D, H, W, K, ws, ws_bytes, stream);
+}
+}
diff --git a/neuroclear_amd/csrc/c8_api.hip b/neuroclear_amd/csrc/c8_api.hip
--- a/neuroclear_amd/csrc/c8_api.hip
+++ b/neuroclear_amd/csrc/c8_api.hip
@@ -215,8 +215,8 @@
 namespace nc {
 int convT_fwd_split_h2(const float* x, const float* w, const float* bias, float* y, void* ys, int ys_ctot, int ys_c0, int N, int C, int D, int H,
                        int W, int K, const unsigned* out_cell, void* ws, size_t ws_bytes, hipStream_t s) {
-  if (!x || !w || !ys || !out_cell || !ws) { set_error("convT_fwd_split_h2: null pointer"); return NC_ERR_ARG; }
-  if (!convT_s3x_supported(N, C, D, H, W, K)) { set_error("convT_fwd_split_h2: shape not covered"); return NC_ERR_SHAPE; }
+  if (!x || !w || (!y && !ys) || (ys && !out_cell) || !ws) { set_error("convT_fwd_split_h2: null pointer"); return NC_ERR_ARG; }
+  if (!convT_s3x_shape(N, C, D, H, W, K)) { set_error("convT_fwd_split_h2: shape not covered"); return NC_ERR_SHAPE; }
   const size_t wb = al256(convT_s3x_ws_bytes(C, K));
   const long S = (long)D * H * W;
   const size_t ex = (size_t)N * C * S;
diff --git a/neuroclear_amd/csrc/common.hpp b/neuroclear_amd/csrc/common.hpp
--- a/neuroclear_amd/csrc/common.hpp
+++ b/neuroclear_amd/csrc/common.hpp
@@ -152,6 +152,16 @@
                  hipStream_t s);
 int conv_dgrad_1x1(const float* dy, const float* w, float* dx, const ConvDims& d, void* ws, size_t wsb,
                    hipStream_t s);
+bool norm_1x1_supported(const ConvDims& d);
+int conv_fwd_1x1_norm(const float* raw, const float* mean, const float* rstd, float slope, const float* w, const float* b, float* y,
+                      const ConvDims& d, void* ws, size_t wsb, hipStream_t s);
+int conv_wgrad_1x1_norm(const float* raw, const float* mean, const float* rstd, float slope, const float* dy, float* dw, const ConvDims& d,
+                        void* ws, size_t wsb, hipStream_t s);
+bool norm_1x1_taken(int N, int C, int D, int H, int W, int K);
+int conv_fwd_norm_1x1(const float* raw, const float* mean, const float* rstd, float slope, const float* w, const float* bias, float* y, int N, int C,
+                      int D, int H, int W, int K, void* ws, size_t ws_bytes, void* stream);
+int conv_wgrad_norm_1x1(const float* raw, const float* mean, const float* rstd, float slope, const float* dy, float* dw, float* dbias, int N, int C,
+                        int D, int H, int W, int K, void* ws, size_t ws_bytes, void* stream);
 
 size_t conv_fwd_to1_k3_ws_bytes(int N, int D, int H, int W);
 int conv_fwd_to1_k3(const float* x, const float* w, float* y, int N, int C, int D, int H, int W, void* ws, size_t wsb, hipStream_t s);
@@ -248,6 +258,16 @@
 __device__ bool guard_skip(const unsigned* guard, int want);
 #endif
 #if defined(__HIPCC__)
+__device__ __forceinline__ float in_act(float x, float m, float r, float slope) {
+  const float v = (x - m) * r;
+  return v > 0.f ? v : v * slope;
+}
+__device__ __forceinline__ void pool_winner_step(float v, int idx, float& best, int& arg) {
+  if (v > best || v != v) {
+    best = v;
+    arg = idx;
+  }
+}
 __device__ __forceinline__ void h2_guard_decide_one(unsigned* ga, unsigned* gb, unsigned* prior, unsigned* flag, int can_flip,
                                                     unsigned long long* stats, unsigned long long total_a) {
   unsigned f = 0;
@@ -281,6 +301,8 @@
                 int c0, float bound, unsigned* cell, unsigned* cell2, hipStream_t s);
 int act_split2h_pool(const float* x, const float* mean, const float* rstd, float slope, void* ys, void* pooled, int N, int C, int D, int H, int W,
                      int ctot, int c0, float bound, unsigned* cell, hipStream_t s);
+int act_split2h_pool_arg(const float* x, const float* mean, const float* rstd, float slope, void* ys, float* pooled, unsigned char* arg, int N, int C,
+                         int D, int H, int W, int ctot, int c0, float bound, unsigned* cell, hipStream_t s);
 int conv_s3x(const void* xs, const float* w, const float* bias, float* y, int N, int Cin, int D, int H, int W, int Kout, int KS, long so,
              long si, int flip, void* wp_ws, hipStream_t s, const unsigned* guard = nullptr);
 bool conv_keep_supported(int N, int C, int D, int H, int W, int K, int ks);
@@ -304,6 +326,7 @@
 int conv_c8x(const void* xh, const float* w, const float* bias, float* y, void* yh, int ctot, int c0, int N, int Cin, int D, int H, int W,
              int Kout, int KS, long so, long si, int flip, int diffuse, int dt, void* wp_ws, hipStream_t s);
 bool convT_s3x_supported(int N, int C, int D, int H, int W, int K);
+bool convT_s3x_shape(int N, int C, int D, int H, int W, int K);
 size_t convT_s3x_ws_bytes(int C, int K);
 int convT_fwd_s3x(const void* xs, const float* w, const float* bias, float* y, void* ys, int ctot, int c0, int N, int C, int D, int H, int W,
                   int K, void* ws, size_t wsb, hipStream_t s, const unsigned* h2cell = nullptr, const unsigned* xcell = nullptr);
diff --git a/neuroclear_amd/csrc/conv_1x1.hip b/neuroclear_amd/csrc/conv_1x1.hip
--- a/neuroclear_amd/csrc/conv_1x1.hip
+++ b/neuroclear_amd/csrc/conv_1x1.hip
@@ -21,8 +21,12 @@
   int npd, npx;
   long nchunks;
   long cps;
+  const float* mean;
+  const float* rstd;
+  float slope;
 };
 
+template <bool NORM>
 __global__ __launch_bounds__(512) void k_wgrad_1x1(W1Params p) {
   extern __shared__ __attribute__((aligned(16))) float lds[];
   typedef const __attribute__((address_space(1))) void* gptr_t;
@@ -63,15 +67,18 @@
   };
 
   f32x4 acc[2] = {f32x4{0.f, 0.f, 0.f, 0.f}, f32x4{0.f, 0.f, 0.f, 0.f}};
-  int aoff[2], boff[2];
+  int aoff[2], boff[2], xch[2];
 #pragma unroll
   for (int t = 0; t < 2; ++t) {
     const int b = wave + 8 * t;
     const int mb = b < nblk ? b / NB : 0, nb = b < nblk ? b % NB : 0;
     aoff[t] = (mb * 16 + l15) * kPitch + 4 * kq;
     boff[t] = p.npd * 256 + (nb * 16 + l15) * kPitch + 4 * kq;
-  }
-
+    xch[t] = nb * 16 + l15;
+  }
+
+  float xm[2] = {0.f, 0.f}, xr[2] = {0.f, 0.f};
+  long ncur = -1;
   if (c0 < c1) issue(c0, lds);
   for (long c = c0; c < c1; ++c) {
     const int par = (int)((c - c0) & 1);
@@ -79,13 +86,22 @@
     __syncthreads();
     if (c + 1 < c1) issue(c + 1, lds + (par ^ 1) * bufsz);
     const float* buf = lds + par * bufsz;
+    if (NORM && c / p.cps != ncur) {
+      ncur = c / p.cps;
+#pragma unroll
+      for (int t = 0; t < 2; ++t) { xm[t] = p.mean[ncur * p.C + xch[t]]; xr[t] = p.rstd[ncur * p.C + xch[t]]; }
+    }
 #pragma unroll
     for (int t = 0; t < 2; ++t) {
       if (wave + 8 * t < nblk) {
 #pragma unroll
         for (int q = 0; q < kVC; q += 16) {
           const f32x4 a = *reinterpret_cast<const f32x4*>(__builtin_assume_aligned(buf + aoff[t] + q, 16));
-          const f32x4 b = *reinterpret_cast<const f32x4*>(__builtin_assume_aligned(buf + boff[t] + q, 16));
+          f32x4 b = *reinterpret_cast<const f32x4*>(__builtin_assume_aligned(buf + boff[t] + q, 16));
+          if (NORM) {
+#pragma unroll
+            for (int m = 0; m < 4; ++m) b[m] = in_act(b[m], xm[t], xr[t], p.slope);
+          }
 #pragma unroll
           for (int m = 0; m < 4; ++m) acc[t] = __builtin_amdgcn_mfma_f32_16x16x4f32(a[m], b[m], acc[t], 0, 0, 0);
         }
@@ -137,7 +153,8 @@
   return (size_t)wg1_nwg(d) * Kp * Cp * sizeof(float) + 256;
 }
 
-int conv_wgrad_1x1(const float* x, const float* dy, float* dw, const ConvDims& d, void* ws, size_t wsb, hipStream_t s) {
+static int launch_wgrad(const float* x, const float* mean, const float* rstd, float slope, const float* dy, float* dw, const ConvDims& d, void* ws,
+                        size_t wsb, hipStream_t s) {
   const size_t need = wgrad_1x1_ws_bytes(d);
   if (!need) {
     set_error("wgrad_1x1: unsupported shape");
@@ -159,12 +176,28 @@
   p.nchunks = (long)d.N * p.cps;
   const int nwg = wg1_nwg(d);
   const int lds_bytes = 2 * (p.npd + p.npx) * 256 * (int)sizeof(float);
-  if (int e = raise_dyn_lds(k_wgrad_1x1, 160 * 1024, "wgrad_1x1")) return e;
-  hipLaunchKernelGGL(k_wgrad_1x1, dim3(nwg), dim3(512), lds_bytes, s, p);
+  p.mean = mean; p.rstd = rstd; p.slope = slope;
+  if (mean) {
+    if (int e = raise_dyn_lds(k_wgrad_1x1<true>, 160 * 1024, "wgrad_1x1")) return e;
+    hipLaunchKernelGGL(k_wgrad_1x1<true>, dim3(nwg), dim3(512), lds_bytes, s, p);
+  } else {
+    if (int e = raise_dyn_lds(k_wgrad_1x1<false>, 160 * 1024, "wgrad_1x1")) return e;
+    hipLaunchKernelGGL(k_wgrad_1x1<false>, dim3(nwg), dim3(512), lds_bytes, s, p);
+  }
   if (int e = check_launch("wgrad_1x1")) return e;
   hipLaunchKernelGGL(k_wgrad_1x1_reduce, dim3((d.K * d.C + 3) / 4), dim3(256), 0, s, (const float*)ws, dw, nwg, d.K,
                      d.C, p.Kp, p.Cp);
   return check_launch("wgrad_1x1_reduce");
+}
+
+int conv_wgrad_1x1(const float* x, const float* dy, float* dw, const ConvDims& d, void* ws, size_t wsb, hipStream_t s) {
+  return launch_wgrad(x, nullptr, nullptr, 0.f, dy, dw, d, ws, wsb, s);
+}
+bool norm_1x1_supported(const ConvDims& d) { return wgrad_1x1_supported(d) && flat_1x1_supported(d) && d.C % 16 == 0; }
+int conv_wgrad_1x1_norm(const float* raw, const float* mean, const float* rstd, float slope, const float* dy, float* dw, const ConvDims& d,
+                        void* ws, size_t wsb, hipStream_t s) {
+  if (!mean || !rstd || !norm_1x1_supported(d)) { set_error("wgrad_1x1_norm: unsupported call"); return NC_ERR_SHAPE; }
+  return launch_wgrad(raw, mean, rstd, slope, dy, dw, d, ws, wsb, s);
 }
 
 static constexpr int kPitchF = 144;
@@ -181,8 +214,12 @@
   int Rp;
   int npi;
   long nchunks, cps;
+  const float* mean;
+  const float* rstd;
+  float slope;
 };
 
+template <bool NORM>
 __global__ __launch_bounds__(512) void k_flat_1x1(F1Params p) {
   extern __shared__ __attribute__((aligned(16))) float lds[];
   typedef const __attribute__((address_space(1))) void* gptr_t;
@@ -228,6 +265,8 @@
   }
   const int nks = p.Rp / 4;
   const int b_off = kq * kPitchF + l15;
+  float xm[16] = {}, xr[16] = {};
+  long ncur = -1;
 
   if (c0 < c1) issue(c0, lds);
   for (long c = c0; c < c1; ++c) {
@@ -237,11 +276,23 @@
     if (c + 1 < c1) issue(c + 1, lds + (par ^ 1) * bufsz);
     const float* buf = lds + par * bufsz + b_off;
     if (mb_on) {
+      if (NORM && c / p.cps != ncur) {
+        ncur = c / p.cps;
+#pragma unroll
+        for (int ks = 0; ks < 16; ++ks) {
+          xm[ks] = ks < nks ? p.mean[ncur * p.R + 4 * ks + kq] : 0.f;
+          xr[ks] = ks < nks ? p.rstd[ncur * p.R + 4 * ks + kq] : 0.f;
+        }
+      }
       for (int nb = wave % wpm; nb < 8; nb += wpm) {
         f32x4 acc = f32x4{0.f, 0.f, 0.f, 0.f};
 #pragma unroll
         for (int ks = 0; ks < 16; ++ks)
-          if (ks < nks) acc = __builtin_amdgcn_mfma_f32_16x16x4f32(aw[ks], buf[4 * ks * kPitchF + nb * 16], acc, 0, 0, 0);
+          if (ks < nks) {
+            float bv = buf[4 * ks * kPitchF + nb * 16];
+            if (NORM) bv = in_act(bv, xm[ks], xr[ks], p.slope);
+            acc = __builtin_amdgcn_mfma_f32_16x16x4f32(aw[ks], bv, acc, 0, 0, 0);
+          }
 #pragma unroll
         for (int rr = 0; rr < 4; ++rr) ost[(mb * 16 + 4 * kq + rr) * kPitchO + nb * 16 + l15] = acc[rr];
       }
@@ -273,7 +324,8 @@
 bool flat_1x1_supported(const ConvDims& d) { return flat_1x1_shape(d); }
 
 static int launch_flat(const float* in, const float* w, const float* bias, float* out, int M, int R, int sm, int sr,
-                       const ConvDims& d, void* ws, size_t wsb, hipStream_t s) {
+                       const ConvDims& d, void* ws, size_t wsb, hipStream_t s, const float* mean = nullptr, const float* rstd = nullptr,
+                       float slope = 0.f) {
   if (!ws || wsb < 256) {
     set_error("flat_1x1: workspace too small");
     return NC_ERR_WS;
@@ -290,8 +342,14 @@
   const int nwg = (int)(p.nchunks < 512 ? p.nchunks : 512);
   const int MB = (M + 15) / 16;
   const int lds_bytes = (2 * p.npi * 256 + MB * 16 * kPitchO) * (int)sizeof(float);
-  if (int e = raise_dyn_lds(k_flat_1x1, 160 * 1024, "flat_1x1")) return e;
-  hipLaunchKernelGGL(k_flat_1x1, dim3(nwg), dim3(512), lds_bytes, s, p);
+  p.mean = mean; p.rstd = rstd; p.slope = slope;
+  if (mean) {
+    if (int e = raise_dyn_lds(k_flat_1x1<true>, 160 * 1024, "flat_1x1")) return e;
+    hipLaunchKernelGGL(k_flat_1x1<true>, dim3(nwg), dim3(512), lds_bytes, s, p);
+  } else {
+    if (int e = raise_dyn_lds(k_flat_1x1<false>, 160 * 1024, "flat_1x1")) return e;
+    hipLaunchKernelGGL(k_flat_1x1<false>, dim3(nwg), dim3(512), lds_bytes, s, p);
+  }
   return check_launch("flat_1x1");
 }
 
@@ -299,6 +357,11 @@
                  hipStream_t s) {
   return launch_flat(x, w, b, y, d.K, d.C, d.C, 1, d, ws, wsb, s);
 }
+int conv_fwd_1x1_norm(const float* raw, const float* mean, const float* rstd, float slope, const float* w, const float* b, float* y,
+                      const ConvDims& d, void* ws, size_t wsb, hipStream_t s) {
+  if (!mean || !rstd || !norm_1x1_supported(d)) { set_error("flat_1x1_norm: unsupported call"); return NC_ERR_SHAPE; }
+  return launch_flat(raw, w, b, y, d.K, d.C, d.C, 1, d, ws, wsb, s, mean, rstd, slope);
+}
 int conv_dgrad_1x1(const float* dy, const float* w, float* dx, const ConvDims& d, void* ws, size_t wsb,
                    hipStream_t s) {
   return launch_flat(dy, w, nullptr, dx, d.C, d.K, 1, d.C, d, ws, wsb, s);
diff --git a/neuroclear_amd/csrc/convt_s3.hip b/neuroclear_amd/csrc/convt_s3.hip
--- a/neuroclear_amd/csrc/convt_s3.hip
+++ b/neuroclear_amd/csrc/convt_s3.hip
@@ -190,12 +190,14 @@
 
 }
 
-bool convT_s3x_supported(int N, int C, int D, int H, int W, int K) {
-  const bool on = sw::raw(sw::CONVT_S3X) != 0;
+bool convT_s3x_shape(int N, int C, int D, int H, int W, int K) {
   const long S = (long)D * H * W;
-  if (!on || C % 32 || K % 16 || C > 256 || N < 1) return false;
+  if (C % 32 || K % 16 || C > 256 || N < 1) return false;
   if ((C / 32) * qn_for(C) * 3 * 1024 > 128 * 1024) return false;
   return (long)N * K * 8 * S < (1L << 40) && S * 16 * 3 * (C / 8) < (1L << 40);
+}
+bool convT_s3x_supported(int N, int C, int D, int H, int W, int K) {
+  return sw::raw(sw::CONVT_S3X) != 0 && convT_s3x_shape(N, C, D, H, W, K);
 }
 size_t convT_s3x_ws_bytes(int C, int K) { return (size_t)C * K * 8 * 3 * 2 + 256; }
 
@@ -207,7 +209,7 @@
 int convT_fwd_s3x(const void* xs, const float* w, const float* bias, float* y, void* ys, int ctot, int c0, int N, int C, int D, int H, int W,
                   int K, void* ws, size_t wsb, hipStream_t s, const unsigned* h2cell, const unsigned* xcell) {
   if (!xs || !w || (!y && !ys) || !ws) { set_error("convT_fwd_s3x: null pointer"); return NC_ERR_ARG; }
-  if (!convT_s3x_supported(N, C, D, H, W, K) || ctot % 8 || c0 % 8) { set_error("convT_fwd_s3x: shape not covered"); return NC_ERR_SHAPE; }
+  if (!convT_s3x_shape(N, C, D, H, W, K) || ctot % 8 || c0 % 8) { set_error("convT_fwd_s3x: shape not covered"); return NC_ERR_SHAPE; }
   if (wsb < convT_s3x_ws_bytes(C, K)) { set_error("convT_fwd_s3x: workspace too small"); return NC_ERR_WS; }
   const int QN = qn_for(C);
   const int NT = xcell ? 2 : 3;
diff --git a/neuroclear_amd/csrc/gen_nets.hip b/neuroclear_amd/csrc/gen_nets.hip
--- a/neuroclear_amd/csrc/gen_nets.hip
+++ b/neuroclear_amd/csrc/gen_nets.hip
@@ -9,6 +9,9 @@
 
 size_t s3_floats(size_t elems) { return up64((elems * 6 + 3) / 4); }
 
+constexpr unsigned kLeanE1 = 1u << 27;
+constexpr unsigned kLeanUp1 = 1u << 28, kLeanUp2 = 1u << 29;
+constexpr unsigned kLeanLo1 = 1u << 30, kLeanLo2 = 1u << 31;
 constexpr int kLeanBit0 = 10;
 constexpr int kLeanBlocks[5] = {1, 3, 5, 6, 8};
 int lean_index(int consumer) {
@@ -184,6 +187,7 @@
   unsigned* cell7 = h2_cells_of(V + p.xs3[7], (size_t)N * 256 * Sh) + 1;
   unsigned* cell9 = h2_cells_of(V + p.xs3[9], (size_t)N * 128 * S) + 1;
   unsigned kept_mask = 0;
+  const bool pool_arg = sw::get(sw::IN_BWD_FOLD) != 0;
   S3xPrepared prep[18] = {};
   bool bound7 = false, bound9 = false;
   if (sw::raw(sw::UNET_WPREP)) {
@@ -216,7 +220,8 @@
     }
   }
   auto prep_of = [&](int seg) -> const S3xPrepared* { return prep[seg].wp ? &prep[seg] : nullptr; };
-  auto block = [&](int i, const float* in, float* out, size_t out_stride, int to, int to_ctot) -> int {
+  auto block = [&](int i, const float* in, float* out, size_t out_stride, int to, int to_ctot, float* pooled = nullptr,
+                   unsigned char* parg = nullptr) -> int {
     const UBlock& b = kUB[i];
     const int* d = p.d[b.lvl];
     const long S = p.S[b.lvl];
@@ -235,6 +240,11 @@
     }
     if (epi) NC_TRY(s3x_stats_finalize((const float*)iws, P + o.b[i], N, d[0], d[1], d[2], b.K, 3, 1e-5f, V + p.mean[i], V + p.rstd[i], hs));
     else NC_TRY(nc_instnorm_stats(V + p.raw[i], N * b.K, S, 1e-5f, V + p.mean[i], V + p.rstd[i], iws, p.in_ws, stream));
+    if (to >= 0 && lean && h2l[to] && to_ctot == 2 * b.K && pooled) kept_mask |= i == 1 ? kLeanLo1 : kLeanLo2;
+    if (pool_arg && (kept_mask & (i == 1 ? kLeanLo1 : kLeanLo2)) && pooled) {
+      return act_split2h_pool_arg(V + p.raw[i], V + p.mean[i], V + p.rstd[i], 0.f, V + p.xs3[to], pooled, parg, N, b.K, d[0], d[1], d[2], to_ctot, 0,
+                                  sqrtf((float)S), h2_cells_of(V + p.xs3[to], (size_t)N * to_ctot * S), hs);
+    }
     if (to >= 0 && use[to]) {
       const int lj = lean && h2l[to] && to_ctot == b.K ? lean_index(to) : -1;
       if (lj >= 0) { out = nullptr; kept_mask |= 1u << (kLeanBit0 + lj); }
@@ -242,6 +252,7 @@
       if (to_ctot == b.K) pre[to] = true;
       return NC_OK;
     }
+    if (to == -2) return NC_OK;
     if (out_stride == (size_t)b.K * S || N == 1)
       return nc_instnorm_act_fwd(V + p.raw[i], V + p.mean[i], V + p.rstd[i], 0.f, out, N * b.K, S, stream);
     for (int n = 0; n < N; ++n)
@@ -250,10 +261,9 @@
     return NC_OK;
   };
   NC_TRY(block(0, x, V + p.a1, (size_t)64 * S, 1, 64));
-  NC_TRY(block(1, V + p.a1, V + p.cat1, (size_t)128 * S, 9, 128));
-  const bool pool_arg = sw::get(sw::IN_BWD_FOLD) != 0;
+  NC_TRY(block(1, V + p.a1, V + p.cat1, (size_t)128 * S, 9, 128, V + p.p1, (unsigned char*)(V + p.parg[0])));
   if (pool_arg) kept_mask |= kKeptPoolArg;
-  for (int n = 0; n < N; ++n) {
+  for (int n = 0; n < N && !(pool_arg && (kept_mask & kLeanLo1)); ++n) {
     if (pool_arg)
       NC_TRY(maxpool2_fwd_arg(V + p.cat1 + (size_t)n * 128 * S, V + p.p1 + (size_t)n * 64 * Sh, (unsigned char*)(V + p.parg[0]) + (size_t)n * 64 * Sh, 64,
                               d0[0], d0[1], d0[2], hs));
@@ -261,8 +271,8 @@
       NC_TRY(nc_maxpool2_fwd(V + p.cat1 + (size_t)n * 128 * S, V + p.p1 + (size_t)n * 64 * Sh, 64, d0[0], d0[1], d0[2], stream));
   }
   NC_TRY(block(2, V + p.p1, V + p.a2, (size_t)128 * Sh, 3, 128));
-  NC_TRY(block(3, V + p.a2, V + p.cat2, (size_t)256 * Sh, 7, 256));
-  for (int n = 0; n < N; ++n) {
+  NC_TRY(block(3, V + p.a2, V + p.cat2, (size_t)256 * Sh, 7, 256, V + p.p2, (unsigned char*)(V + p.parg[1])));
+  for (int n = 0; n < N && !(pool_arg && (kept_mask & kLeanLo2)); ++n) {
     if (pool_arg)
       NC_TRY(maxpool2_fwd_arg(V + p.cat2 + (size_t)n * 256 * Sh, V + p.p2 + (size_t)n * 128 * Sq, (unsigned char*)(V + p.parg[1]) + (size_t)n * 128 * Sq,
                               128, d1[0], d1[1], d1[2], hs));
@@ -276,9 +286,11 @@
     NC_TRY(h2_zero_cells(cell7, 1, hs));
     NC_TRY(convT_h2_bound(P + o.w[10], P + o.b[10], 256, 128, sqrtf((float)Sq), cell7, hs));
   }
+  if (lean && ct2h) kept_mask |= kLeanUp2;
+  if (lean && ct1h) kept_mask |= kLeanUp1;
   for (int n = 0; n < N; ++n) {
     if (ct2h)
-      NC_TRY(convT_fwd_split_h2(V + p.b3 + (size_t)n * 256 * Sq, P + o.w[10], P + o.b[10], V + p.cat2 + ((size_t)n * 256 + 128) * Sh,
+      NC_TRY(convT_fwd_split_h2(V + p.b3 + (size_t)n * 256 * Sq, P + o.w[10], P + o.b[10], lean ? nullptr : V + p.cat2 + ((size_t)n * 256 + 128) * Sh,
                                 (char*)(V + p.xs3[7]) + (size_t)n * 256 * Sh * 4, 256, 128, 1, 256, d2[0], d2[1], d2[2], 128, cell7, cws, p.conv_ws, hs));
     else if (ct2)
       NC_TRY(nc_convT_k2s2_fwd_split(V + p.b3 + (size_t)n * 256 * Sq, nullptr, P + o.w[10], P + o.b[10], V + p.cat2 + ((size_t)n * 256 + 128) * Sh,
@@ -301,7 +313,7 @@
   }
   for (int n = 0; n < N; ++n) {
     if (ct1h)
-      NC_TRY(convT_fwd_split_h2(V + p.e2b + (size_t)n * 128 * Sh, P + o.w[11], P + o.b[11], V + p.cat1 + ((size_t)n * 128 + 64) * S,
+      NC_TRY(convT_fwd_split_h2(V + p.e2b + (size_t)n * 128 * Sh, P + o.w[11], P + o.b[11], lean ? nullptr : V + p.cat1 + ((size_t)n * 128 + 64) * S,
                                 (char*)(V + p.xs3[9]) + (size_t)n * 128 * S * 4, 128, 64, 1, 128, d1[0], d1[1], d1[2], 64, cell9, cws, p.conv_ws, hs));
     else if (ct1)
       NC_TRY(nc_convT_k2s2_fwd_split(V + p.e2b + (size_t)n * 128 * Sh, nullptr, P + o.w[11], P + o.b[11], V + p.cat1 + ((size_t)n * 128 + 64) * S,
@@ -318,8 +330,15 @@
     if (!ct_s3 && !ct1h) NC_TRY(operand_into(cd[9], V + p.cat1 + (size_t)64 * S, (long)128 * S, V + p.xs3[9], N, 64, S, 128, 64, hs));
     pre[9] = true;
   }
-  NC_TRY(block(9, V + p.cat1, V + p.e1, (size_t)64 * S, -1, 0));
-  NC_TRY(nc_conv_fwd(V + p.e1, P + o.w[12], P + o.b[12], V + p.t1, N, 64, d0[0], d0[1], d0[2], 1, 1, 1, 1, 1, 0, cws, p.conv_ws, stream));
+  if (lean && norm_1x1_taken(N, 64, d0[0], d0[1], d0[2], 1)) {
+    kept_mask |= kLeanE1;
+    NC_TRY(block(9, V + p.cat1, nullptr, (size_t)64 * S, -2, 0));
+    NC_TRY(conv_fwd_norm_1x1(V + p.raw[9], V + p.mean[9], V + p.rstd[9], 0.f, P + o.w[12], P + o.b[12], V + p.t1, N, 64, d0[0], d0[1], d0[2], 1, cws,
+                             p.conv_ws, stream));
+  } else {
+    NC_TRY(block(9, V + p.cat1, V + p.e1, (size_t)64 * S, -1, 0));
+    NC_TRY(nc_conv_fwd(V + p.e1, P + o.w[12], P + o.b[12], V + p.t1, N, 64, d0[0], d0[1], d0[2], 1, 1, 1, 1, 1, 0, cws, p.conv_ws, stream));
+  }
   NC_TRY(nc_conv_fwd(V + p.t1, P + o.w[13], P + o.b[13], y, N, 1, d0[0], d0[1], d0[2], 1, 1, 1, 1, 1, 0, cws, p.conv_ws, stream));
   if (kept) *kept = kept_mask;
   return nc_sigmoid_fwd(y, y, (long)N * S, stream);
@@ -357,6 +376,14 @@
       off += s3x_packed_bytes(sg[k].Cin, sg[k].Kout, 3, 2);
     }
   }
+  auto input_unread = [&](int i, bool want_dx) -> bool {
+    const UBlock& b = kUB[i];
+    const int* d = p.d[b.lvl];
+    ConvDims cdk;
+    const bool now_h2 = make_dims(cdk, N, b.C, d[0], d[1], d[2], b.K, 3, 3, 3, 1, 1) && conv_layer_h2(cdk);
+    const bool have = ((kept_mask >> i) & 1) && (((kept_mask >> (16 + i)) & 1) != 0) == now_h2;
+    return have && !h2_guard_can_flip() && conv_bwd_pre_supported(N, b.C, d[0], d[1], d[2], b.K, 3, want_dx, p.conv_ws);
+  };
   auto block_bwd = [&](int i, const float* g, const float* in, float* draw, float* gin, bool r1 = false, const float* pool = nullptr) -> int {
     const UBlock& b = kUB[i];
     const int* d = p.d[b.lvl];
@@ -366,8 +393,7 @@
     const void* xs = ((kept_mask >> i) & 1) && (((kept_mask >> (16 + i)) & 1) != 0) == now_h2 ? (const void*)(V + p.xs3[i]) : nullptr;
     const S3xPrepared* pd = i >= 1 && gin && now_h2 && (kept_mask & kKeptWPrep) && ((kept_mask >> (16 + i)) & 1) && wprep_now ? &prepd[i] : nullptr;
     const int lj = lean_index(i);
-    if (lj >= 0 && ((kept_mask >> (kLeanBit0 + lj)) & 1) &&
-        !(xs && !h2_guard_can_flip() && conv_bwd_pre_supported(N, b.C, d[0], d[1], d[2], b.K, 3, gin != nullptr, p.conv_ws))) {
+    if (lj >= 0 && ((kept_mask >> (kLeanBit0 + lj)) & 1) && !input_unread(i, gin != nullptr)) {
       NC_TRY(nc_instnorm_act_fwd(V + p.raw[i - 1], V + p.mean[i - 1], V + p.rstd[i - 1], 0.f, G + p.T, N * b.C, Sl, stream));
       in = G + p.T;
     }
@@ -409,6 +435,22 @@
     *out = G + p.T;
     return NC_OK;
   };
+  {
+    float* Vw = const_cast<float*>(saved);
+    auto rebuild = [&](int lo_blk, size_t cat, int C, long Sl, bool lower, bool upper, const float* tin, int tw, const int* td) -> int {
+      for (int n = 0; n < N && lower; ++n)
+        NC_TRY(nc_instnorm_act_fwd(V + p.raw[lo_blk] + (size_t)n * C * Sl, V + p.mean[lo_blk] + n * C, V + p.rstd[lo_blk] + n * C, 0.f,
+                                   Vw + cat + (size_t)n * 2 * C * Sl, C, Sl, stream));
+      for (int n = 0; n < N && upper; ++n)
+        NC_TRY(convT_fwd_split_h2(tin + (size_t)n * 2 * C * (Sl / 8), P + o.w[tw], P + o.b[tw], Vw + cat + ((size_t)n * 2 + 1) * C * Sl, nullptr, 2 * C, C, 1,
+                                  2 * C, td[0], td[1], td[2], C, nullptr, cws, p.conv_ws, hs));
+      return NC_OK;
+    };
+    const bool in9 = !input_unread(9, true), in7 = !input_unread(7, true);
+    const bool lo1 = (kept_mask & kLeanLo1) && (kept_mask & kKeptPoolArg), lo2 = (kept_mask & kLeanLo2) && (kept_mask & kKeptPoolArg);
+    NC_TRY(rebuild(1, p.cat1, 64, S, lo1 && (in9 || !pool_folds(1)), (kept_mask & kLeanUp1) && in9, V + p.e2b, 11, d1));
+    NC_TRY(rebuild(3, p.cat2, 128, Sh, lo2 && (in7 || !pool_folds(3)), (kept_mask & kLeanUp2) && in7, V + p.b3, 10, d2));
+  }
   NC_TRY(nc_sigmoid_bwd(dy, y, G + p.s1, (long)N * S, stream));
   NC_TRY(nc_conv_wgrad(V + p.t1, G + p.s1, DP + o.w[13], DP + o.b[13], N, 1, d0[0], d0[1], d0[2], 1, 1, 1, 1, 1, 0, cws, p.conv_ws, stream));
   NC_TRY(nc_conv_dgrad(G + p.s1, P + o.w[13], G + p.s2, N, 1, d0[0], d0[1], d0[2], 1, 1, 1, 1, 1, 0, cws, p.conv_ws, stream));
@@ -416,7 +458,17 @@
   const bool r1 = sw::raw(sw::UNET_LEAN) != 0 && N == 1 && fuse_bwd &&
                   make_dims(cd9, N, 128, d0[0], d0[1], d0[2], 64, 3, 3, 3, 1, 1) && conv_layer_h2(cd9) &&
                   conv_bwd_pre_supported(N, 128, d0[0], d0[1], d0[2], 64, 3, true, p.conv_ws) && instnorm_bwd_s3_supported(N, 64, S);
-  NC_TRY(nc_conv_wgrad(V + p.e1, G + p.s2, DP + o.w[12], DP + o.b[12], N, 64, d0[0], d0[1], d0[2], 1, 1, 1, 1, 1, 0, cws, p.conv_ws, stream));
+  if ((kept_mask & kLeanE1) && norm_1x1_taken(N, 64, d0[0], d0[1], d0[2], 1)) {
+    NC_TRY(conv_wgrad_norm_1x1(V + p.raw[9], V + p.mean[9], V + p.rstd[9], 0.f, G + p.s2, DP + o.w[12], DP + o.b[12], N, 64, d0[0], d0[1], d0[2], 1, cws,
+                               p.conv_ws, stream));
+  } else {
+    const float* e1 = V + p.e1;
+    if (kept_mask & kLeanE1) {
+      NC_TRY(nc_instnorm_act_fwd(V + p.raw[9], V + p.mean[9], V + p.rstd[9], 0.f, G + p.T, N * 64, S, stream));
+      e1 = G + p.T;
+    }
+    NC_TRY(nc_conv_wgrad(e1, G + p.s2, DP + o.w[12], DP + o.b[12], N, 64, d0[0], d0[1], d0[2], 1, 1, 1, 1, 1, 0, cws, p.conv_ws, stream));
+  }
   if (!r1) {
     NC_TRY(nc_conv_dgrad(G + p.s2, P + o.w[12], G + p.G1, N, 64, d0[0], d0[1], d0[2], 1, 1, 1, 1, 1, 0, cws, p.conv_ws, stream));
   }
diff --git a/neuroclear_amd/csrc/h2.hip b/neuroclear_amd/csrc/h2.hip
--- a/neuroclear_amd/csrc/h2.hip
+++ b/neuroclear_amd/csrc/h2.hip
@@ -157,9 +157,11 @@
   for (int t = 0; t < 2; ++t) out[(ob * 2 + t) * S + v] = s3_unit(e, t);
 }
 
+template <bool ARG>
 __global__ void __launch_bounds__(256) k_act_split2h_pool(const float* __restrict__ x, const float* __restrict__ mean, const float* __restrict__ rstd,
-                                                          float slope, uint4* __restrict__ out, uint4* __restrict__ pooled, int D, int H, int W,
-                                                          int cblocks, int oblocks, int ob0, unsigned bound_bits, unsigned* __restrict__ cell) {
+                                                          float slope, uint4* __restrict__ out, uint4* __restrict__ pooled, float* __restrict__ pf,
+                                                          unsigned char* __restrict__ parg, int D, int H, int W, int cblocks, int oblocks, int ob0,
+                                                          unsigned bound_bits, unsigned* __restrict__ cell) {
   if (blockIdx.x == 0 && blockIdx.y == 0 && threadIdx.x == 0 && cell) *cell = bound_bits;
   const int Do = D / 2, Ho = H / 2, Wo = W / 2;
   const long So = (long)Do * Ho * Wo, S = (long)D * H * W;
@@ -175,6 +177,11 @@
   for (int j = 0; j < 8; ++j) { m[j] = mean[c0 + j]; r[j] = rstd[c0 + j]; }
   float best[8];
   unsigned short w0[8], w1[8];
+  int win[8];
+  if (ARG) {
+#pragma unroll
+    for (int j = 0; j < 8; ++j) { best[j] = -INFINITY; win[j] = 0; }
+  }
 #pragma unroll
   for (int kp = 0; kp < 4; ++kp) {
     const long u = ((long)(2 * zo + (kp >> 1)) * H + (2 * yo + (kp & 1))) * W + 2 * xo;
@@ -186,6 +193,10 @@
       t0 = t0 > 0.f ? t0 : t0 * slope;
       t1 = t1 > 0.f ? t1 : t1 * slope;
       asm("" : "+v"(t0), "+v"(t1));
+      if (ARG) {
+        pool_winner_step(t0, kp * 2, best[j], win[j]);
+        pool_winner_step(t1, kp * 2 + 1, best[j], win[j]);
+      }
       h2_split(t0 * sc, e[0][j]);
       h2_split(t1 * sc, e[1][j]);
     }
@@ -193,6 +204,7 @@
     for (int h = 0; h < 2; ++h) {
 #pragma unroll
       for (int t = 0; t < 2; ++t) out[(ob * 2 + t) * S + u + h] = s3_unit(e[h], t);
+      if (ARG) continue;
       const int k = (kp >> 1) * 4 + (kp & 1) * 2 + h;
 #pragma unroll
       for (int j = 0; j < 8; ++j) {
@@ -200,6 +212,14 @@
         if (val > best[j] || k == 0) { best[j] = val; w0[j] = e[h][j][0]; w1[j] = e[h][j][1]; }
       }
     }
+  }
+  if (ARG) {
+#pragma unroll
+    for (int j = 0; j < 8; ++j) {
+      pf[(c0 + j) * So + v] = best[j];
+      parg[(c0 + j) * So + v] = (unsigned char)win[j];
+    }
+    return;
   }
   uint4 o0, o1;
   o0.x = w0[0] | ((unsigned)w0[1] << 16); o0.y = w0[2] | ((unsigned)w0[3] << 16); o0.z = w0[4] | ((unsigned)w0[5] << 16); o0.w = w0[6] | ((unsigned)w0[7] << 16);
@@ -339,9 +359,25 @@
   unsigned bits;
   __builtin_memcpy(&bits, &bound, 4);
   const long So = (long)(D / 2) * (H / 2) * (W / 2);
-  hipLaunchKernelGGL(k_act_split2h_pool, dim3((unsigned)cdiv(So, 256), (unsigned)(N * C / 8)), dim3(256), 0, s, x, mean, rstd, slope, (uint4*)ys,
-                     (uint4*)pooled, D, H, W, C / 8, ctot / 8, c0 / 8, bits, cell);
+  hipLaunchKernelGGL(k_act_split2h_pool<false>, dim3((unsigned)cdiv(So, 256), (unsigned)(N * C / 8)), dim3(256), 0, s, x, mean, rstd, slope, (uint4*)ys,
+                     (uint4*)pooled, (float*)nullptr, (unsigned char*)nullptr, D, H, W, C / 8, ctot / 8, c0 / 8, bits, cell);
   return check_launch("act_split2h_pool");
 }
 
-}
+int act_split2h_pool_arg(const float* x, const float* mean, const float* rstd, float slope, void* ys, float* pooled, unsigned char* arg, int N, int C,
+                         int D, int H, int W, int ctot, int c0, float bound, unsigned* cell, hipStream_t s) {
+  if (!x || !mean || !rstd || !ys || !pooled || !arg) { set_error("act_split2h_pool_arg: null pointer"); return NC_ERR_ARG; }
+  if (N < 1 || C < 8 || C % 8 || ctot % 8 || c0 % 8 || c0 < 0 || c0 + C > ctot || D < 2 || H < 2 || W < 2 || ((D | H | W) & 1) || (long)N * C / 8 > 65535) {
+    set_error("act_split2h_pool_arg: channels % 8, even extents");
+    return NC_ERR_SHAPE;
+  }
+  if ((((uintptr_t)x) & 7) != 0) { set_error("act_split2h_pool_arg: input not 8-byte aligned"); return NC_ERR_ARG; }
+  unsigned bits;
+  __builtin_memcpy(&bits, &bound, 4);
+  const long So = (long)(D / 2) * (H / 2) * (W / 2);
+  hipLaunchKernelGGL(k_act_split2h_pool<true>, dim3((unsigned)cdiv(So, 256), (unsigned)(N * C / 8)), dim3(256), 0, s, x, mean, rstd, slope, (uint4*)ys,
+                     (uint4*)nullptr, pooled, arg, D, H, W, C / 8, ctot / 8, c0 / 8, bits, cell);
+  return check_launch("act_split2h_pool_arg");
+}
+
+}
diff --git a/neuroclear_amd/csrc/h2_debug.hip b/neuroclear_amd/csrc/h2_debug.hip
--- a/neuroclear_amd/csrc/h2_debug.hip
+++ b/neuroclear_amd/csrc/h2_debug.hip
@@ -45,6 +45,12 @@
   if (!x || !mean || !rstd || !ys || !pooled) { set_error("act_split2h_pool_debug: null pointer"); return NC_ERR_ARG; }
   if (D < 2 || H < 2 || W < 2 || !h2_part_ok(N, C, (long)D * H * W, ctot, c0) || !(bound > 0.f)) { set_error("act_split2h_pool_debug: bad shape"); return NC_ERR_SHAPE; }
   return act_split2h_pool(x, mean, rstd, slope, ys, pooled, N, C, D, H, W, ctot, c0, bound, cell, (hipStream_t)stream);
+}
+
+int nc_act_split2h_pool_arg_debug(const float* x, const float* mean, const float* rstd, float slope, void* ys, float* pooled, unsigned char* arg, int N,
+                                  int C, int D, int H, int W, int ctot, int c0, float bound, unsigned* cell, void* stream) {
+  if (!(bound > 0.f)) { set_error("act_split2h_pool_arg_debug: bad shape"); return NC_ERR_SHAPE; }
+  return act_split2h_pool_arg(x, mean, rstd, slope, ys, pooled, arg, N, C, D, H, W, ctot, c0, bound, cell, (hipStream_t)stream);
 }
 
 int nc_maxpool2_h2_debug(const void* in, void* out, int N, int C, int ctot, int D, int H, int W, void* stream) {
diff --git a/neuroclear_amd/csrc/norm_act.hip b/neuroclear_amd/csrc/norm_act.hip
--- a/neuroclear_amd/csrc/norm_act.hip
+++ b/neuroclear_amd/csrc/norm_act.hip
@@ -95,16 +95,11 @@
     float4* o4 = reinterpret_cast<float4*>(o);
     for (long i = (long)blockIdx.x * 256 + threadIdx.x; i < S / 4; i += (long)gridDim.x * 256) {
       float4 v = p4[i];
-      v.x = (v.x - m) * r; v.y = (v.y - m) * r; v.z = (v.z - m) * r; v.w = (v.w - m) * r;
-      v.x = v.x > 0.f ? v.x : v.x * slope; v.y = v.y > 0.f ? v.y : v.y * slope;
-      v.z = v.z > 0.f ? v.z : v.z * slope; v.w = v.w > 0.f ? v.w : v.w * slope;
+      v.x = in_act(v.x, m, r, slope); v.y = in_act(v.y, m, r, slope); v.z = in_act(v.z, m, r, slope); v.w = in_act(v.w, m, r, slope);
       o4[i] = v;
     }
   } else {
-    for (long i = (long)blockIdx.x * 256 + threadIdx.x; i < S; i += (long)gridDim.x * 256) {
-      const float v = (p[i] - m) * r;
-      o[i] = v > 0.f ? v : v * slope;
-    }
+    for (long i = (long)blockIdx.x * 256 + threadIdx.x; i < S; i += (long)gridDim.x * 256) o[i] = in_act(p[i], m, r, slope);
   }
 }
 
@@ -789,13 +784,7 @@
   int arg = 0;
   for (int a = 0; a < wd; ++a)
     for (int b = 0; b < 2; ++b)
-      for (int c = 0; c < 2; ++c) {
-        const float v = p[((long)(od * wd + a) * H + (oh * 2 + b)) * W + ow * 2 + c];
-        if (v > best || v != v) {
-          best = v;
-          arg = (a * 2 + b) * 2 + c;
-        }
-      }
+      for (int c = 0; c < 2; ++c) pool_winner_step(p[((long)(od * wd + a) * H + (oh * 2 + b)) * W + ow * 2 + c], (a * 2 + b) * 2 + c, best, arg);
   return arg;
 }
 
```
